# neu-vi/Superpoints_Registration

Measured on AMD Instinct MI355X. Metric: point-cloud pairs/sec (16 384 pts/cloud), higher is better.
Workload: dtype f32 (matrix products: range-scaled split-f16x2 MFMA, f32 accumulate; attention weights below 2^-5 of their row sum carried in one f16 plane); 1 GPU; synthetic 16384-pt pairs, full KPConv backbone + superpoint attn + Sinkhorn-SVD pose (3dmatch config, BASELINE configs[1]); streams_per_gpu=1, points_per_cloud=16384, generator=box, point_order=reference, upsample_indices=True, cross_step_overlap=True, streams_inside_a_forward=3: main path, pyramid searches, ResNet shortcut branches

## Files before the change

include/spr.h:

```cpp
#ifndef SPR_H_
#define SPR_H_

#include <stddef.h>
#include <stdint.h>

#ifdef __cplusplus
extern "C" {
#endif

#define SPR_VERSION 6

#define SPR_ACT_NONE 0
#define SPR_ACT_RELU 1
#define SPR_ACT_SIGMOID 2

#define SPR_ORDER_REFERENCE 0
#define SPR_ORDER_CANONICAL 1

#define SPR_SELECT_NEAREST 0
#define SPR_SELECT_INDEX 1

int spr_version(void);
const char* spr_last_error(void);

// ... 13 lines not shown

#define SPR_PREPARE_RANGE (-1)
#define SPR_PREPARE_PROBE (-2)
#define SPR_PREPARE_BAD_LAYOUT (-3)
size_t spr_prepare_scans_scratch_len(int n, int nb);
int spr_prepare_scans(const float* pts, int stride, const int* cu, int n, int nb, double voxel_size,
                      double crop_radius, int remove_ground, int* scratch, size_t scratch_len,
                      float* out_xyz, int* out_idx, int* out_cu, int* status, void* stream);

size_t spr_radius_neighbors_workspace_bytes(int nq, int ns, int nb);
int spr_radius_neighbors(const float* q_xyz, const int* q_cu, int nq,
                         const float* s_xyz, const int* s_cu, int ns, int nb,
                         float radius, int limit, int algo, int select, int* out_idx,
                         int* max_count, void* ws, size_t ws_bytes, void* stream);

size_t spr_radius_table_bytes(int ns, int nb);
size_t spr_radius_table_build_workspace_bytes(int ns, int nb);
size_t spr_radius_table_query_workspace_bytes(int nq);
int spr_radius_table_slots(void);
int spr_radius_table_build(const float* s_xyz, const int* s_cu, int ns, int nb, float radius,
                           void* table, size_t table_bytes, void* ws, size_t ws_bytes, void* stream);
int spr_radius_table_query(const float* q_xyz, const int* q_cu, int nq, int self, int ns, int nb,
                           float radius, int limit, int slot, const void* table, int* out_idx,
                           int* max_count, int algo, int select, void* ws, size_t ws_bytes, void* stream);

int spr_radius_table_count(const float* q_xyz, const int* q_cu, int nq, int self, int ns, int nb,
                           float radius, const void* table, int* counts, int* hist, int hist_n,
                           int* status, void* stream);

size_t spr_kdtree_replay_size(int ns, int nb);
int spr_kdtree_replay_build(const float* s_xyz, const int* s_cu, int ns, int nb, void* tree, size_t tree_bytes,
                            void* stream);
size_t spr_tie_order_workspace_size(int nq, int max_count, int depth);
int spr_tie_order(const float* q_xyz, const int* q_cu, int nq, const float* s_xyz, const int* s_cu, int ns, int nb,
                  float radius, const void* tree, int depth, int* nbr, int stride, int width, int max_count,
                  int* status, void* ws, size_t ws_bytes, void* stream);
int spr_tie_order_host(const float* q_xyz_host, const int* q_cu_host, int nq, const float* s_xyz_host,
                       const int* s_cu_host, int ns, int nb, float radius, int* nbr_host, int stride, int width,
                       int max_count, int* status_host);
int spr_std_sort_replay_host(const float* keys_host, int n, int* perm_host, int* heap_ranges_host);

size_t spr_gt_overlap_workspace_bytes(int ns, int nt, int nb);
int spr_gt_overlap(const float* src_xyz, const int* src_cu, int ns, const float* tgt_xyz, const int* tgt_cu,
                   int nt, const float* pose, int nb, double radius, int* src_corr, int* tgt_corr,
                   unsigned char* src_mask, unsigned char* tgt_mask, int* corr, int* corr_count, void* ws,
                   size_t ws_bytes, void* stream);

#define SPR_AUG_NONE 0
#define SPR_AUG_SMALL 1
#define SPR_AUG_LARGE 2
int spr_philox4x32_host(const uint32_t* ctr_host, const uint32_t* key_host, uint32_t* out_host);
int spr_augment_draw(uint64_t seed, const uint64_t* pair_key_host, int nb, int mode, unsigned char* perturb_src_host,
                     unsigned char* swap_host, float* perturb_host, const uint64_t* pair_key, const int* src_cu,
                     int ns, const int* tgt_cu, int nt, float* noise, unsigned int* keys, void* stream);
size_t spr_augment_workspace_bytes(int ns, int nt, int nb, int corr_stride);
int spr_augment_pairs(const float* src_xyz, const int* src_cu, int ns, const float* tgt_xyz, const int* tgt_cu,
                      int nt, const float* pose, int nb, const unsigned char* src_mask,
                      const unsigned char* tgt_mask, const int* corr, int corr_stride, const int* corr_off,
                      const int* corr_count, const float* perturb, const unsigned char* flags, int mode, float scale,
                      int max_pts, uint64_t seed, const uint64_t* pair_key, const float* noise,
                      const unsigned int* keys, float* out_src_xyz, float* out_tgt_xyz, int* out_src_cu,
                      int* out_tgt_cu, float* out_pose, unsigned char* out_src_mask, unsigned char* out_tgt_mask,
                      int* out_src_perm, int* out_tgt_perm, int* out_corr, int* out_corr_count, int* status, void* ws,
                      size_t ws_bytes, void* stream);

int spr_modelnet_draw(uint64_t seed, const uint64_t* pair_key_host, int nb, double rot_mag, double trans_mag,
                      double* dirs_host, float* transform_host, const uint64_t* pair_key, const int* cu, int n_total,
                      int k, unsigned int* rkeys, unsigned int* extra, float* noise, unsigned int* skeys, void* stream);
size_t spr_modelnet_pairs_workspace_size(int n_total, int nb, int k);
int spr_modelnet_pairs(const float* xyz, const int* cu, int n_total, int nb, int max_len_host, float p_src, float p_tgt,
                       double q_src, double q_tgt, int k, float scale, float clip, const float* transform,
                       const double* dirs, uint64_t seed, const uint64_t* pair_key, const unsigned int* rkeys,
                       const unsigned int* extra, const float* noise, const unsigned int* skeys, float* src_xyz,
                       float* tgt_xyz, float* pose, unsigned char* src_overlap, unsigned char* tgt_overlap,
                       int* src_index, int* tgt_index, int* corr, int* corr_count, int* status, void* ws,
                       size_t ws_bytes, void* stream);

int spr_estimate_normals(const float* xyz, const int* cu, int n, int nb, const int* nbr, int nbr_stride, int kmax,
                         const float* viewpoint, float* normals, float* curvature, void* stream);
int spr_feats_gather_rotate(const float* feats, int n_in, int c, const int* rows, int n_out, const int* cu_out, int nb,
                            const float* rot, const int* dir_cols_host, int n_dir, float* out, void* stream);

size_t spr_kpconv_workspace_bytes(int nq, int ns, int cin, int cout);
size_t spr_kpconv_plan_bytes(int nq);
int spr_kpconv_plan(const int* nbr, int nq, int ns, int nbr_stride, int kmax, int rows_sorted,
                    const int* order, void* plan, size_t plan_bytes, void* stream);
size_t spr_kpconv_wplanes_bytes(int cin, int cout);
int spr_kpconv_prep_weights(const float* weights, int n_kp, int cin, int cout, const float* w_range,
                            int w_range_n, void* wplanes, size_t wplanes_bytes, void* stream);
int spr_kpconv_fwd(const float* q_xyz, int nq, const float* s_xyz, int ns, const int* nbr,
                   int nbr_stride, int kmax, int rows_sorted, const float* x, int cin,
                   const float* weights, int cout, const float* kernel_points, int n_kp,
                   float kp_extent, float* out, int impl, const float* x_range, int x_range_n,
                   const float* w_range, int w_range_n, const void* plan, const void* wplanes,
                   void* ws, size_t ws_bytes, void* stream);

#define SPR_KP_CONSTANT 0
#define SPR_KP_LINEAR 1
#define SPR_KP_GAUSSIAN 2
#define SPR_KP_SUM 0
#define SPR_KP_CLOSEST 1
size_t spr_kpconv_modes_workspace_size(int nq, int ns, int cin, int cout);
int spr_kpconv_modes_fwd(const float* q_xyz, int nq, const float* s_xyz, int ns, const int* nbr, int nbr_stride,
                         int kmax, const float* x, int cin, const float* weights, int cout,
                         const float* kernel_points, int n_kp, float kp_extent, int influence, int aggregation,
                         float* out, int impl, const float* x_range, int x_range_n, const float* w_range,
                         int w_range_n, const void* wplanes, void* ws, size_t ws_bytes, void* stream);
size_t spr_kpconv_modes_weighted_features_workspace_size(int ns);
int spr_kpconv_modes_weighted_features(const float* q_xyz, int nq, const float* s_xyz, int ns, const int* nbr,
                                       int nbr_stride, int kmax, const float* x, int cin, const float* kernel_points,
                                       int n_kp, float kp_extent, int influence, int aggregation, float* wf,
                                       float* cnt, void* ws, size_t ws_bytes, void* stream);
int spr_kpconv_modes_bwd_dx(const float* q_xyz, int nq, const float* s_xyz, int ns, const int* nbr, int nbr_stride,
                            int kmax, int cin, const float* kernel_points, int n_kp, float kp_extent, int influence,
                            int aggregation, const float* dwf, const float* dwf_range, int dwf_range_n, float* dx,
                            void* ws, size_t ws_bytes, void* stream);

size_t spr_kpconv_deform_workspace_size(int nq, int ns, int cin, int cout);
int spr_kpconv_deform_fwd(const float* q_xyz, int nq, const float* s_xyz, int ns, const int* nbr, int nbr_stride,
                          int kmax, const float* x, int cin, const float* weights, int cout,
                          const float* kernel_points, int n_kp, float kp_extent, const float* offset_features,
                          int of_stride, int modulated, float* out, float* min_d2, int impl, const float* x_range,
                          int x_range_n, const float* w_range, int w_range_n, const void* wplanes, void* ws,
                          size_t ws_bytes, void* stream);
size_t spr_kpconv_deform_weighted_features_workspace_size(int ns);
int spr_kpconv_deform_weighted_features(const float* q_xyz, int nq, const float* s_xyz, int ns, const int* nbr,
                                        int nbr_stride, int kmax, const float* x, int cin, const float* kernel_points,
                                        int n_kp, float kp_extent, const float* offset_features, int of_stride,
                                        float* wf, float* cnt, void* ws, size_t ws_bytes, void* stream);
int spr_kpconv_deform_bwd_dx(const float* q_xyz, int nq, const float* s_xyz, int ns, const int* nbr, int nbr_stride,
                             int kmax, int cin, const float* kernel_points, int n_kp, float kp_extent,
                             const float* offset_features, int of_stride, int modulated, const float* dwfm,
                             const float* dwfm_range, int dwfm_range_n, float* dx, void* ws, size_t ws_bytes,
                             void* stream);
int spr_kpconv_deform_bwd_offsets(const float* q_xyz, int nq, const float* s_xyz, int ns, const int* nbr,
                                  int nbr_stride, int kmax, const float* x, int cin, const float* kernel_points,
                                  int n_kp, float kp_extent, const float* offset_features, int of_stride,
                                  int modulated, const float* dwfm, float* d_offset_features, void* stream);

size_t spr_deform_reg_workspace_size(int nq);
int spr_deform_reg(const float* q_xyz, int nq, const float* s_xyz, int ns, const int* nbr, int nbr_stride, int kmax,
                   const float* kernel_points, int n_kp, float kp_extent, const float* offset_features, int of_stride,
                   int modulated, float repulse_extent, float* out, float* d_offset_features, void* ws,
                   size_t ws_bytes, void* stream);

size_t spr_icp_pairs_workspace_size(int ns, int nt, int nb);
int spr_icp_pairs(const float* src_xyz, const int* src_cu, int ns, const float* tgt_xyz, const int* tgt_cu, int nt,
                  const double* pose_init, int nb, double max_dist, int max_iter, double rel_fitness, double rel_rmse,
                  float* pose, double* pose64, double* fitness, double* inlier_rmse, int* iterations, int* count,
                  int* corr, int* status, void* ws, size_t ws_bytes, void* stream);

int spr_kpconv_few_supported(int cin, int cout, int n_kp);

int spr_kpconv_stem_supported(int cin, int cout, int n_kp);
size_t spr_kpconv_stem_workspace_size(int nq, int ns, int nb, int max_len_host, int cout);
int spr_kpconv_stem(const float* q_xyz, int nq, const float* s_xyz, int ns, const int* nbr, int nbr_stride,
                    int kmax, int rows_sorted, const float* x, const float* weights, int cout,
                    const float* kernel_points, int n_kp, float kp_extent, const int* cu, int nb,
                    int max_len_host, float eps, float slope, float* out, float* out_range, int out_range_n,
                    float* mean_out, float* rstd_out, void* ws, size_t ws_bytes, void* stream);

size_t spr_instnorm_workspace_bytes(int max_len_host, int nb, int c);
int spr_instnorm(const float* x, const int* cu, int n, int nb, int max_len_host, int c,
                 float eps, int norm, const float* add, float slope, float* out,
                 float* out_range, int out_range_n, void* ws, size_t ws_bytes, void* stream);
int spr_instnorm_stats(const float* x, const int* cu, int n, int nb, int max_len_host, int c, float eps,
                       float* mean, float* rstd, void* ws, size_t ws_bytes, void* stream);

int spr_block_tail_tile_rows(int ka, int kb, int n_out);
size_t spr_block_tail_tiles_len(int n, int nb, int tile_rows);
int spr_block_tail_tiles(const int* cu, int n, int nb, int tile_rows, int* tiles, void* stream);
size_t spr_block_tail_workspace_bytes(int n, int nb, int kb, int n_out, int tile_rows);
int spr_block_tail(const float* xa, int ka, const float* wa, const float* xb, int kb, const float* wb,
                   const float* add, const int* cu, const int* tiles, int n, int nb, int n_out, float eps,
                   float slope, float* out, const float* xa_range, int xa_range_n, const float* wa_range,
                   int wa_range_n, const float* xb_range, int xb_range_n, const float* wb_range,
                   int wb_range_n, float* out_range, int out_range_n, const float* xa_mean,
                   const float* xa_rstd, float xa_slope, void* ws, size_t ws_bytes, void* stream);

int spr_maxpool_gather(const float* x, int ns, int c, const int* idx, int nq, int idx_stride, int k,
                       const int* order, float* out, float* out_range, int out_range_n, void* stream);
size_t spr_cell_order_workspace_bytes(int n);
int spr_cell_order(const float* xyz, const int* cu, int n, int nb, float cell, int* order, void* ws, size_t ws_bytes,
                   void* stream);

size_t spr_linear_workspace_bytes(void);
int spr_linear(const float* x, int m, int k, const float* w, int n, const float* bias,
               const float* residual, int act, float* out, const float* x_range,
               int x_range_n, const float* w_range, int w_range_n, float* out_range,
               int out_range_cap, int* out_range_n_host, void* ws, size_t ws_bytes, void* stream);
int spr_range_parts(void);
int spr_absmax(const float* x, long rows, int cols, long stride, float* parts, void* stream);
int spr_absmax_multi(const void* jobs_dev, int njobs, int parts_per_job, float* parts_out, void* stream);

int spr_set_gemm_mode(int mode);

int spr_layernorm_range_count(int m);
int spr_layernorm(const float* x, int m, int c, const float* gamma, const float* beta,
                  float eps, const float* pos, float* out_norm, float* out_pos,
                  float* range_norm, float* range_pos, void* stream);

int spr_posemb_sine(const float* xyz, int n, int d_model, float scale,
                    float temperature, float* out, void* stream);

int spr_posemb_mlp(const float* xyz, const float* const* params_host, int t, int d_model, float* pe, void* stream);
size_t spr_posemb_mlp_bwd_workspace_bytes(int t);
int spr_posemb_mlp_bwd(const float* xyz, const float* const* params_host, const float* dpe, int t, int d_model,
                       float* const* grads_host, void* ws, size_t ws_bytes, void* stream);

size_t spr_attn_workspace_bytes(int t, int nseg, int nhead, int head_dim);
int spr_attn_varlen_fwd(const float* q, int q_stride, const float* k, int k_stride, const float* v,
                        int v_stride, const int* cu, const int* kv_seg, int t, int nseg, int max_len_host,
                        int nhead, int head_dim, float scale, float* out, int o_stride, float* lse,
                        int* lse_written, void* ws, size_t ws_bytes, void* stream);

size_t spr_attn_inproj_workspace_bytes(int t, int nseg, int nhead, int head_dim);
int spr_attn_inproj_prepare(const float* w_in, int d, float* out, void* stream);
int spr_attn_inproj_varlen_fwd(const float* x_qk, const float* x_v, int t, const float* w_in,
                               const float* b_in, const int* cu, const int* kv_seg, int nseg,
                               int max_len_host, int nhead, int head_dim, float scale,
                               float* out, int o_stride, const float* xqk_range,
                               int xqk_range_n, const float* xv_range, int xv_range_n,
                               float* out_range, const float* w_prep, void* ws, size_t ws_bytes, void* stream);

size_t spr_attn_probs_workspace_bytes(int t, int nhead, int head_dim);
int spr_attn_probs(const float* q, int q_stride, const float* k, int k_stride, const int* cu,
                   const int* kv_seg, int t, int nseg, int max_len_host, int nhead, int head_dim,
                   float scale, int per_head, float* out, const long long* place, int max_rows_host,
                   int max_cols_host, void* ws, size_t ws_bytes, void* stream);

#define SPR_XENC_PTRS_PER_LAYER 18
size_t spr_xenc_prepared_bytes(int n_layers, int d_ff);
size_t spr_xenc_plan_bytes(void);
int spr_xenc_prepare(const void* const* layer_ptrs_host, const float* eps_host, int n_layers,
                     int d_model, int nhead, int d_ff, const float* final_g, const float* final_b,
                     float final_eps, float pos_bound, void* prepared, size_t prepared_bytes,
                     void* plan_host, size_t plan_bytes, void* stream);
size_t spr_xenc_workspace_bytes(int t, int nseg);
int spr_xenc_forward(const void* plan_host, const float* x, const float* pos, const int* cu,
                     const int* kv_self, const int* kv_cross, int t, int nseg, int max_len_host,
                     float* out, void* ws, size_t ws_bytes, void* stream);

size_t spr_attn_bwd_workspace_bytes(int t, int nseg, int nhead);
size_t spr_attn_bwd_min_workspace_bytes(int t, int nhead);
int spr_attn_varlen_bwd(const float* q, int q_stride, const float* k, int k_stride, const float* v,
                        int v_stride, const float* out, int o_stride, const float* dout, int do_stride,
                        const float* lse, const int* cu, const int* kv_seg, const int* q_seg, int t, int nseg,
                        int max_len_host, int nhead, int head_dim, float scale, float* dq, float* dk,
                        float* dv, void* ws, size_t ws_bytes, void* stream);

int spr_set_attn_mode(int mode);

size_t spr_match_workspace_bytes(const int* cu_host, int npairs);
int spr_match_dualsoftmax(const float* feat, int d, const int* cu,
                          const int* cu_host, int npairs, float* match_val,
                          float* match_val2, int* match_ind, void* ws, size_t ws_bytes,
                          void* stream);

int spr_pose_residuals(const float* pose, const float* a, const float* b, const int* pair_cu,
                       int npairs, int total_host, float* res, void* stream);
int spr_pose_scores(const float* poses, int nh, const float* a, const float* b, int n,
// ... 164 lines not shown
```

superpoints_registration_amd/_lib.py:

```python
import ctypes
import os
import subprocess

_HERE = os.path.dirname(os.path.abspath(__file__))
LIB_PATH = os.environ.get("SPR_HIP_LIB") or os.path.join(_HERE, "libspr_hip.so")

_vp = ctypes.c_void_p
_i = ctypes.c_int
_f = ctypes.c_float
_sz = ctypes.c_size_t
_l = ctypes.c_long
_u64 = ctypes.c_uint64
_d = ctypes.c_double

SIGNATURES = {
    "spr_version": (_i, []),
    "spr_last_error": (ctypes.c_char_p, []),
    "spr_grid_subsample_workspace_bytes": (_sz, [_i, _i]),
    "spr_grid_subsample": (_i, [_vp, _vp, _i, _i, _f, _i, _i, _vp, _vp, _vp, _vp, _sz, _vp]),
    "spr_grid_subsample_attrs_workspace_size": (_sz, [_i, _i, _i, _i]),
    "spr_grid_subsample_attrs": (_i, [_vp, _vp, _i, _i, _f, _i, _i, _vp, _i, _vp, _i, _vp, _vp, _vp, _vp, _vp, _vp, _sz,
                                      _vp]),
    "spr_voxel_downsample_workspace_bytes": (_sz, [_i]),
    "spr_voxel_downsample": (_i, [_vp, _i, ctypes.c_double, _vp, _vp, _vp, _sz, _vp]),
    "spr_prepare_scans_scratch_len": (_sz, [_i, _i]),
    "spr_prepare_scans": (_i, [_vp, _i, _vp, _i, _i, ctypes.c_double, ctypes.c_double, _i, _vp, _sz, _vp, _vp, _vp, _vp,
                               _vp]),
    "spr_radius_neighbors_workspace_bytes": (_sz, [_i, _i, _i]),
    "spr_radius_neighbors": (_i, [_vp, _vp, _i, _vp, _vp, _i, _i, _f, _i, _i, _i, _vp, _vp, _vp, _sz, _vp]),
    "spr_radius_table_bytes": (_sz, [_i, _i]),
    "spr_radius_table_build_workspace_bytes": (_sz, [_i, _i]),
    "spr_radius_table_query_workspace_bytes": (_sz, [_i]),
    "spr_radius_table_slots": (_i, []),
    "spr_radius_table_build": (_i, [_vp, _vp, _i, _i, _f, _vp, _sz, _vp, _sz, _vp]),
    "spr_radius_table_query": (_i, [_vp, _vp, _i, _i, _i, _i, _f, _i, _i, _vp, _vp, _vp, _i, _i, _vp, _sz, _vp]),
    "spr_radius_table_count": (_i, [_vp, _vp, _i, _i, _i, _i, _f, _vp, _vp, _vp, _i, _vp, _vp]),
    "spr_kdtree_replay_size": (_sz, [_i, _i]),
    "spr_kdtree_replay_build": (_i, [_vp, _vp, _i, _i, _vp, _sz, _vp]),
    "spr_tie_order_workspace_size": (_sz, [_i, _i, _i]),
    "spr_tie_order": (_i, [_vp, _vp, _i, _vp, _vp, _i, _i, _f, _vp, _i, _vp, _i, _i, _i, _vp, _vp, _sz, _vp]),
    "spr_tie_order_host": (_i, [_vp, _vp, _i, _vp, _vp, _i, _i, _f, _vp, _i, _i, _i, _vp]),
    "spr_std_sort_replay_host": (_i, [_vp, _i, _vp, _vp]),
    "spr_gt_overlap_workspace_bytes": (_sz, [_i, _i, _i]),
    "spr_gt_overlap": (_i, [_vp, _vp, _i, _vp, _vp, _i, _vp, _i, ctypes.c_double, _vp, _vp, _vp, _vp, _vp, _vp, _vp,
                            _sz, _vp]),
    "spr_icp_pairs_workspace_size": (_sz, [_i, _i, _i]),
    "spr_icp_pairs": (_i, [_vp, _vp, _i, _vp, _vp, _i, _vp, _i, _d, _i, _d, _d, _vp, _vp, _vp, _vp, _vp, _vp, _vp, _vp,
                           _vp, _sz, _vp]),
    "spr_philox4x32_host": (_i, [_vp, _vp, _vp]),
    "spr_augment_draw": (_i, [_u64, _vp, _i, _i, _vp, _vp, _vp, _vp, _vp, _i, _vp, _i, _vp, _vp, _vp]),
    "spr_augment_workspace_bytes": (_sz, [_i, _i, _i, _i]),
    "spr_augment_pairs": (_i, [_vp, _vp, _i, _vp, _vp, _i, _vp, _i, _vp, _vp, _vp, _i, _vp, _vp, _vp, _vp, _i, _f, _i,
                               _u64, _vp, _vp, _vp, _vp, _vp, _vp, _vp, _vp, _vp, _vp, _vp, _vp, _vp, _vp, _vp, _vp,
                               _sz, _vp]),
    "spr_modelnet_draw": (_i, [_u64, _vp, _i, _d, _d, _vp, _vp, _vp, _vp, _i, _i, _vp, _vp, _vp, _vp, _vp]),
    "spr_modelnet_pairs_workspace_size": (_sz, [_i, _i, _i]),
    "spr_modelnet_pairs": (_i, [_vp, _vp, _i, _i, _i, _f, _f, _d, _d, _i, _f, _f, _vp, _vp, _u64, _vp, _vp, _vp, _vp,
                                _vp, _vp, _vp, _vp, _vp, _vp, _vp, _vp, _vp, _vp, _vp, _vp, _sz, _vp]),
    "spr_estimate_normals": (_i, [_vp, _vp, _i, _i, _vp, _i, _i, _vp, _vp, _vp, _vp]),
    "spr_feats_gather_rotate": (_i, [_vp, _i, _i, _vp, _i, _vp, _i, _vp, _vp, _i, _vp, _vp]),
    "spr_kpconv_workspace_bytes": (_sz, [_i, _i, _i, _i]),
    "spr_kpconv_fwd": (_i, [_vp, _i, _vp, _i, _vp, _i, _i, _i, _vp, _i, _vp, _i, _vp, _i, _f, _vp, _i, _vp, _i, _vp,
                            _i, _vp, _vp, _vp, _sz, _vp]),
    "spr_kpconv_modes_workspace_size": (_sz, [_i, _i, _i, _i]),
    "spr_kpconv_modes_fwd": (_i, [_vp, _i, _vp, _i, _vp, _i, _i, _vp, _i, _vp, _i, _vp, _i, _f, _i, _i, _vp, _i, _vp,
                                  _i, _vp, _i, _vp, _vp, _sz, _vp]),
    "spr_kpconv_modes_weighted_features_workspace_size": (_sz, [_i]),
    "spr_kpconv_modes_weighted_features": (_i, [_vp, _i, _vp, _i, _vp, _i, _i, _vp, _i, _vp, _i, _f, _i, _i, _vp, _vp,
                                                _vp, _sz, _vp]),
    "spr_kpconv_modes_bwd_dx": (_i, [_vp, _i, _vp, _i, _vp, _i, _i, _i, _vp, _i, _f, _i, _i, _vp, _vp, _i, _vp, _vp,
                                     _sz, _vp]),
    "spr_kpconv_deform_workspace_size": (_sz, [_i, _i, _i, _i]),
    "spr_kpconv_deform_fwd": (_i, [_vp, _i, _vp, _i, _vp, _i, _i, _vp, _i, _vp, _i, _vp, _i, _f, _vp, _i, _i, _vp, _vp,
                                   _i, _vp, _i, _vp, _i, _vp, _vp, _sz, _vp]),
    "spr_kpconv_deform_weighted_features_workspace_size": (_sz, [_i]),
    "spr_kpconv_deform_weighted_features": (_i, [_vp, _i, _vp, _i, _vp, _i, _i, _vp, _i, _vp, _i, _f, _vp, _i, _vp,
                                                 _vp, _vp, _sz, _vp]),
    "spr_kpconv_deform_bwd_dx": (_i, [_vp, _i, _vp, _i, _vp, _i, _i, _i, _vp, _i, _f, _vp, _i, _i, _vp, _vp, _i, _vp,
                                      _vp, _sz, _vp]),
    "spr_kpconv_deform_bwd_offsets": (_i, [_vp, _i, _vp, _i, _vp, _i, _i, _vp, _i, _vp, _i, _f, _vp, _i, _i, _vp, _vp,
                                           _vp]),
    "spr_deform_reg_workspace_size": (_sz, [_i]),
    "spr_deform_reg": (_i, [_vp, _i, _vp, _i, _vp, _i, _i, _vp, _i, _f, _vp, _i, _i, _f, _vp, _vp, _vp, _sz, _vp]),
    "spr_kpconv_few_supported": (_i, [_i, _i, _i]),
    "spr_kpconv_stem_supported": (_i, [_i, _i, _i]),
    "spr_kpconv_stem_workspace_size": (_sz, [_i, _i, _i, _i, _i]),
    "spr_kpconv_stem": (_i, [_vp, _i, _vp, _i, _vp, _i, _i, _i, _vp, _vp, _i, _vp, _i, _f, _vp, _i, _i, _f, _f, _vp,
                             _vp, _i, _vp, _vp, _vp, _sz, _vp]),
    "spr_instnorm_workspace_bytes": (_sz, [_i, _i, _i]),
    "spr_instnorm": (_i, [_vp, _vp, _i, _i, _i, _i, _f, _i, _vp, _f, _vp, _vp, _i, _vp, _sz, _vp]),
    "spr_maxpool_gather": (_i, [_vp, _i, _i, _vp, _i, _i, _i, _vp, _vp, _vp, _i, _vp]),
    "spr_linear_workspace_bytes": (_sz, []),
    "spr_linear": (_i, [_vp, _i, _i, _vp, _i, _vp, _vp, _i, _vp, _vp, _i, _vp, _i, _vp, _i, _vp, _vp, _sz, _vp]),
    "spr_range_parts": (_i, []),
    "spr_absmax_multi": (_i, [_vp, _i, _i, _vp, _vp]),
    "spr_absmax": (_i, [_vp, _l, _i, _l, _vp, _vp]),
    "spr_kpconv_plan_bytes": (_sz, [_i]),
    "spr_kpconv_plan": (_i, [_vp, _i, _i, _i, _i, _i, _vp, _vp, _sz, _vp]),
    "spr_kpconv_wplanes_bytes": (_sz, [_i, _i]),
    "spr_kpconv_prep_weights": (_i, [_vp, _i, _i, _i, _vp, _i, _vp, _sz, _vp]),
    "spr_block_tail_tile_rows": (_i, [_i, _i, _i]),
    "spr_block_tail_tiles_len": (_sz, [_i, _i, _i]),
    "spr_block_tail_tiles": (_i, [_vp, _i, _i, _i, _vp, _vp]),
    "spr_block_tail_workspace_bytes": (_sz, [_i, _i, _i, _i, _i]),
    "spr_block_tail": (_i, [_vp, _i, _vp, _vp, _i, _vp, _vp, _vp, _vp, _i, _i, _i, _f, _f, _vp, _vp, _i, _vp, _i,
                            _vp, _i, _vp, _i, _vp, _i, _vp, _vp, _f, _vp, _sz, _vp]),
    "spr_instnorm_stats": (_i, [_vp, _vp, _i, _i, _i, _i, _f, _vp, _vp, _vp, _sz, _vp]),
    "spr_cell_order_workspace_bytes": (_sz, [_i]),
    "spr_cell_order": (_i, [_vp, _vp, _i, _i, _f, _vp, _vp, _sz, _vp]),
    "spr_layernorm_range_count": (_i, [_i]),
    "spr_attn_inproj_prepare": (_i, [_vp, _i, _vp, _vp]),
    "spr_set_gemm_mode": (_i, [_i]),
    "spr_layernorm": (_i, [_vp, _i, _i, _vp, _vp, _f, _vp, _vp, _vp, _vp, _vp, _vp]),
    "spr_posemb_sine": (_i, [_vp, _i, _i, _f, _f, _vp, _vp]),
    "spr_posemb_mlp": (_i, [_vp, _vp, _i, _i, _vp, _vp]),
    "spr_posemb_mlp_bwd_workspace_bytes": (_sz, [_i]),
    "spr_posemb_mlp_bwd": (_i, [_vp, _vp, _vp, _i, _i, _vp, _vp, _sz, _vp]),
    "spr_attn_workspace_bytes": (_sz, [_i, _i, _i, _i]),
    "spr_attn_varlen_fwd": (_i, [_vp, _i, _vp, _i, _vp, _i, _vp, _vp, _i, _i, _i, _i, _i, _f, _vp, _i, _vp, _vp, _vp,
                                 _sz, _vp]),
    "spr_attn_probs_workspace_bytes": (_sz, [_i, _i, _i]),
    "spr_attn_probs": (_i, [_vp, _i, _vp, _i, _vp, _vp, _i, _i, _i, _i, _i, _f, _i, _vp, _vp, _i, _i, _vp, _sz,
                            _vp]),
    "spr_attn_bwd_workspace_bytes": (_sz, [_i, _i, _i]),
    "spr_attn_bwd_min_workspace_bytes": (_sz, [_i, _i]),
    "spr_attn_varlen_bwd": (_i, [_vp, _i, _vp, _i, _vp, _i, _vp, _i, _vp, _i, _vp, _vp, _vp, _vp, _i, _i, _i, _i, _i,
                                 _f, _vp, _vp, _vp, _vp, _sz, _vp]),
    "spr_attn_inproj_workspace_bytes": (_sz, [_i, _i, _i, _i]),
    "spr_attn_inproj_varlen_fwd": (_i, [_vp, _vp, _i, _vp, _vp, _vp, _vp, _i, _i, _i, _i, _f, _vp, _i, _vp, _i, _vp,
                                        _i, _vp, _vp, _vp, _sz, _vp]),
    "spr_set_attn_mode": (_i, [_i]),
    "spr_xenc_prepared_bytes": (_sz, [_i, _i]),
    "spr_xenc_plan_bytes": (_sz, []),
    "spr_xenc_prepare": (_i, [_vp, _vp, _i, _i, _i, _i, _vp, _vp, _f, _f, _vp, _sz, _vp, _sz, _vp]),
    "spr_xenc_workspace_bytes": (_sz, [_i, _i]),
    "spr_xenc_forward": (_i, [_vp, _vp, _vp, _vp, _vp, _vp, _i, _i, _i, _vp, _vp, _sz, _vp]),
    "spr_match_workspace_bytes": (_sz, [_vp, _i]),
    "spr_match_dualsoftmax": (_i, [_vp, _i, _vp, _vp, _i, _vp, _vp, _vp, _vp, _sz, _vp]),
    "spr_pose_residuals": (_i, [_vp, _vp, _vp, _vp, _i, _i, _vp, _vp]),
    "spr_pose_scores": (_i, [_vp, _i, _vp, _vp, _i, _vp, _vp]),
    "spr_weighted_procrustes": (_i, [_vp, _vp, _vp, _vp, _i, _vp, _vp]),
    "spr_refine_pairs_workspace_bytes": (_sz, [_i, _i]),
    "spr_refine_pairs": (_i, [_vp, _vp, _vp, _vp, _vp, _vp, _i, _i, _vp, _vp, _i, _f, _f, _i, _vp, _i, _vp, _vp, _vp, _vp,
                              _vp, _vp, _vp, _sz, _vp]),
    "spr_ransac_draw": (_i, [_u64, _vp, _vp, _i, _i, _i, _vp]),
    "spr_ransac_pairs": (_i, [_vp, _vp, _vp, _vp, _i, _i, _i, _u64, _vp, _vp, _vp, _vp, _vp, _vp, _vp, _vp]),
    "spr_sinkhorn_workspace_bytes": (_sz, [_vp, _i]),
    "spr_match_sinkhorn": (_i, [_vp, _i, _vp, _vp, _vp, _i, _vp, _vp, _i, _vp, _vp, _vp, _vp, _vp, _vp, _sz, _vp]),
    "spr_sinkhorn_correspondences": (_i, [_vp, _i, _vp, _vp, _vp, _i, _vp, _vp, _i, _i, _vp, _vp, _vp,
                                          _sz, _vp]),
    "spr_loss_workspace_bytes": (_sz, [_i, _i, _i]),
    "spr_overlap_pool": (_i, [_vp, _i, _vp, _i, _i, _i, _vp, _vp]),
    "spr_bce_logits_mean": (_i, [_vp, _vp, _i, _vp, _vp, _sz, _vp]),
    "spr_infonce_pair": (_i, [_vp, _i, _vp, _i, _i, _vp, _vp, _vp, _vp, _f, _f, _vp, _vp, _sz, _vp]),
    "spr_transform_l1_pair": (_i, [_vp, _vp, _vp, _i, _vp, _vp, _sz, _vp]),
    "spr_sum_scaled": (_i, [_vp, _i, _f, _vp, _vp]),
    "spr_gather_rows": (_i, [_vp, _i, _i, _vp, _i, _vp, _vp]),
    "spr_upsample_unary_supported": (_i, [_i, _i, _i]),
    "spr_upsample_unary_workspace_size": (_sz, []),
    "spr_upsample_unary": (_i, [_vp, _i, _i, _vp, _i, _i, _vp, _i, _vp, _i, _vp, _vp, _i, _vp, _i, _vp, _i, _vp, _i,
                                _vp, _vp, _sz, _vp]),
    "spr_pair_gather": (_i, [_vp, _i, _i, _vp, _i, _vp, _vp, _i, _vp, _i, _vp, _vp]),
    "spr_pair_gather_bwd": (_i, [_vp, _i, _i, _vp, _i, _vp, _vp, _i, _vp, _i, _vp, _vp]),
    "spr_overlap_pool_pairs": (_i, [_vp, _i, _vp, _i, _i, _i, _vp, _vp, _i, _vp, _i, _vp, _vp, _i, _vp, _vp]),
    "spr_bgemm": (_i, [_vp, _vp, _vp, _vp, _i, _i, _i, _l, _l, _l, _l, _l, _l, _f, _f, _vp]),
    "spr_tn_product_split_workspace_bytes": (_sz, []),
    "spr_tn_product_split": (_i, [_vp, _vp, _l, _i, _i, _i, _vp, _i, _vp, _i, _vp, _vp, _sz, _vp]),
    "spr_tn_product_f64_workspace_bytes": (_sz, [_l, _i, _i]),
    "spr_tn_product_f64": (_i, [_vp, _vp, _l, _i, _i, _vp, _vp, _sz, _vp]),
    "spr_reduce_parts": (_i, [_vp, _i, _l, _f, _vp, _i, _vp]),
    "spr_act_bwd": (_i, [_vp, _vp, _i, _l, _vp, _vp]),
    "spr_colsum_workspace_bytes": (_sz, [_i]),
    "spr_colsum": (_i, [_vp, _l, _i, _vp, _vp, _sz, _vp]),
    "spr_layernorm_bwd_workspace_bytes": (_sz, [_i]),
    "spr_layernorm_bwd": (_i, [_vp, _i, _i, _vp, _f, _vp, _vp, _vp, _vp, _vp, _vp, _sz, _vp]),
    "spr_instnorm_bwd_workspace_bytes": (_sz, [_i, _i, _i]),
    "spr_instnorm_bwd": (_i, [_vp, _vp, _vp, _vp, _i, _i, _i, _i, _f, _i, _f, _vp, _vp, _vp, _sz, _vp]),
    "spr_scatter_workspace_bytes": (_sz, [_l, _i]),
    "spr_maxpool_bwd": (_i, [_vp, _i, _i, _vp, _i, _i, _i, _vp, _vp, _vp, _sz, _vp]),
    "spr_scatter_rows_add": (_i, [_vp, _vp, _i, _i, _i, _vp, _vp, _sz, _vp]),
    "spr_kpconv_weighted_features_workspace_bytes": (_sz, [_i]),
    "spr_kpconv_weighted_features": (_i, [_vp, _i, _vp, _i, _vp, _i, _i, _vp, _i, _vp, _i, _f, _vp, _vp, _vp, _sz,
                                          _vp]),
    "spr_kpconv_bwd_dx": (_i, [_vp, _i, _vp, _i, _vp, _i, _i, _i, _vp, _i, _f, _vp, _vp, _i, _vp, _vp, _sz, _vp]),
    "spr_softmax_rows": (_i, [_vp, _vp, _i, _i, _vp]),
    "spr_softmax_bwd_rows": (_i, [_vp, _vp, _vp, _i, _i, _vp]),
    "spr_bce_logits_mean_bwd": (_i, [_vp, _vp, _i, _vp, _vp, _vp]),
    "spr_infonce_pair_dlogits": (_i, [_vp, _i, _vp, _i, _i, _vp, _vp, _vp, _vp, _f, _f, _vp, _vp, _vp, _vp, _vp, _sz,
                                      _vp]),
# ... 46 lines not shown
```

superpoints_registration_amd/csrc/block_tail.hip:

```cpp
#include "spr_common.h"
#include "split_mma.h"

namespace spr {
int gemm_mode();
namespace {

constexpr int kTailThreads = 512;
constexpr int kTailWaves = 8;

struct TailArgs {
  const float* xa;
  const float* xb;
  const float* wa;
  const float* wb;
  const float* add;
  const int* cu;
  const int* tile_cu;
  const int4* tile_desc;
  int nb, n, n_total;
  const float* xa_parts;
  const float* xb_parts;
  const float* wa_parts;
  const float* wb_parts;
  int xa_np, xb_np, wa_np, wb_np;
// ... 304 lines not shown
  }
  const int len = cu[cloud + 1] - cu[cloud];
  const double n = len > 0 ? (double)len : 1.0;
  const double m = s / n;
  double var = ss / n - m * m;
  if (var < 0.0) var = 0.0;
  float* o = stats + ((size_t)cloud * nbr + br) * 2 * n_total + col;
  o[0] = (float)m;
  o[n_total] = (float)(1.0 / sqrt(var + (double)eps));
}

__global__ __launch_bounds__(1024) void k_tile_cu(const int* __restrict__ cu, int nb, int tr, int* __restrict__ tile_cu) {
  __shared__ int sh[1024];
  int carry = 0;
  for (int base = 0; base < nb; base += 1024) {
    const int c = base + threadIdx.x;
    int v = c < nb ? (cu[c + 1] - cu[c] + tr - 1) / tr : 0;
    sh[threadIdx.x] = v;
    __syncthreads();
    for (int o = 1; o < 1024; o <<= 1) {
      const int add = threadIdx.x >= o ? sh[threadIdx.x - o] : 0;
      __syncthreads();
      sh[threadIdx.x] += add;
      __syncthreads();
    }
    if (c < nb) tile_cu[c + 1] = carry + sh[threadIdx.x];
    carry += sh[1023];
    __syncthreads();
  }
  if (threadIdx.x == 0) tile_cu[0] = 0;
}

__global__ void k_tile_desc(const int* __restrict__ cu, const int* __restrict__ tile_cu, int tr, int4* __restrict__ desc) {
  const int c = blockIdx.x;
  const int t0 = tile_cu[c], nt = tile_cu[c + 1] - t0, r0 = cu[c], len = cu[c + 1] - r0;
  for (int i = threadIdx.x; i < nt; i += blockDim.x) desc[t0 + i] = make_int4(r0 + i * tr, min(tr, len - i * tr), c, 0);
}

struct TailShape {
  int nc, tr;
};
TailShape tail_shape(int ka, int kb, int n_total) {
  if (ka == 32 && kb == 64 && n_total == 128) return {128, 64};
  if (ka == 32 && kb == 0 && n_total == 128) return {128, 64};
  if (ka == 64 && kb == 128 && n_total == 256) return {256, 64};
  if (ka == 64 && kb == 0 && n_total == 256) return {256, 64};
  if (ka == 128 && kb == 256 && n_total == 512) return {128, 32};
  if (ka == 128 && kb == 0 && n_total == 512) return {256, 64};
  return {0, 0};
}

template <int KA, int KB, int NC, int TR>
int launch_tail(const TailArgs& a, float eps, hipStream_t stream) {
  constexpr int KS = (KA + KB) / 32, NBR = KB > 0 ? 2 : 1;
  constexpr int lds = 4 * (TR / 16) * KS * 1024 + 2 * NBR * 2 * NC * (int)sizeof(float);
  const void* k1 = (const void*)k_block_tail<KA, KB, NC, TR, 1>;
  const void* k2 = (const void*)k_block_tail<KA, KB, NC, TR, 2>;
  if (int rc = ensure_dyn_lds(k1, lds)) return rc;
  if (int rc = ensure_dyn_lds(k2, lds)) return rc;
  static int per_cu[2] = {0, 0};
  if (per_cu[0] == 0) {
    int n1 = 0, n2 = 0;
    if (hipOccupancyMaxActiveBlocksPerMultiprocessor(&n1, k1, kTailThreads, lds) != hipSuccess || n1 < 1) n1 = 1;
    if (hipOccupancyMaxActiveBlocksPerMultiprocessor(&n2, k2, kTailThreads, lds) != hipSuccess || n2 < 1) n2 = 1;
    per_cu[1] = n2 > 2 ? 2 : n2;
    per_cu[0] = n1 > 2 ? 2 : n1;
  }
  const int ncg = a.n_total / NC;
  const int max_tiles = cdiv(a.n, TR) + a.nb;
  auto grid_x = [&](int occ) {
    int g = device_cu_count() * occ / ncg;
    if (g > max_tiles) g = max_tiles;
    return g < 1 ? 1 : g;
  };
  hipLaunchKernelGGL((k_block_tail<KA, KB, NC, TR, 1>), dim3(grid_x(per_cu[0]), ncg), dim3(kTailThreads), lds, stream, a);
  hipLaunchKernelGGL(k_tail_final, dim3(cdiv((long)a.nb * NBR * a.n_total, 256)), dim3(256), 0, stream, a.part, a.cu,
                     a.tile_cu, a.nb, NBR, a.n_total, eps, a.stats);
  hipLaunchKernelGGL((k_block_tail<KA, KB, NC, TR, 2>), dim3(grid_x(per_cu[1]), ncg), dim3(kTailThreads), lds, stream, a);
  SPR_LAUNCH_CHECK();
  return 0;
}

}
}

using namespace spr;

extern "C" int spr_block_tail_tile_rows(int ka, int kb, int n_out) { return tail_shape(ka, kb, n_out).tr; }

static size_t tiles_desc_offset(int nb) { return align_up((size_t)(nb > 0 ? nb : 0) + 1, 4); }
extern "C" size_t spr_block_tail_tiles_len(int n, int nb, int tile_rows) {
  return tiles_desc_offset(nb) + 4 * ((size_t)cdiv(n > 0 ? n : 1, tile_rows > 0 ? tile_rows : 64) + (size_t)(nb > 0 ? nb : 1));
}

extern "C" int spr_block_tail_tiles(const int* cu, int n, int nb, int tile_rows, int* tiles, void* stream_) {
  hipStream_t stream = (hipStream_t)stream_;
  SPR_REQUIRE(cu != nullptr && tiles != nullptr && n >= 1 && nb >= 1 && tile_rows >= 16 && ((uintptr_t)tiles & 15) == 0,
              "block_tail_tiles: bad arguments");
  hipLaunchKernelGGL(k_tile_cu, dim3(1), dim3(1024), 0, stream, cu, nb, tile_rows, tiles);
  hipLaunchKernelGGL(k_tile_desc, dim3(nb), dim3(256), 0, stream, cu, tiles, tile_rows,
                     reinterpret_cast<int4*>(tiles + tiles_desc_offset(nb)));
  SPR_LAUNCH_CHECK();
  return 0;
}

namespace {
struct TailWs {
  double* part;
  float* stats;
  float* mp[4];
};
TailWs tail_layout(Workspace& w, int n, int nb, int kb, int n_out, int tile_rows) {
  const size_t nbr = kb > 0 ? 2 : 1, B = (size_t)(nb > 0 ? nb : 1), no = (size_t)(n_out > 0 ? n_out : 0);
  const size_t tiles = (size_t)cdiv(n > 0 ? n : 1, tile_rows > 0 ? tile_rows : 64) + B;
  TailWs l;
  l.part = w.take<double>(tiles * nbr * 2 * no);
  l.stats = w.take<float>(B * nbr * 2 * no);
  for (float*& p : l.mp) p = w.take<float>(kAmaxParts);
  return l;
}
}

extern "C" size_t spr_block_tail_workspace_bytes(int n, int nb, int kb, int n_out, int tile_rows) {
  return measure(tail_layout, n, nb, kb, n_out, tile_rows);
}

extern "C" int spr_block_tail(const float* xa, int ka, const float* wa, const float* xb, int kb, const float* wb,
                              const float* add, const int* cu, const int* tiles, int n, int nb, int n_out, float eps,
                              float slope, float* out, const float* xa_range, int xa_range_n, const float* wa_range,
                              int wa_range_n, const float* xb_range, int xb_range_n, const float* wb_range,
                              int wb_range_n, float* out_range, int out_range_n, const float* xa_mean,
                              const float* xa_rstd, float xa_slope, void* ws, size_t ws_bytes, void* stream_) {
  hipStream_t stream = (hipStream_t)stream_;
  SPR_REQUIRE(spr::gemm_mode() == 1, "block_tail: only in the split-fp16 product mode (spr_set_gemm_mode(1))");
  const TailShape sh = tail_shape(ka, kb, n_out);
  SPR_REQUIRE(sh.tr > 0, "block_tail: unsupported shape ka=%d kb=%d n_out=%d (spr_block_tail_tile_rows)", ka, kb, n_out);
  SPR_REQUIRE(xa && wa && cu && tiles && out && n > 0 && nb >= 1, "block_tail: null operand or empty input");
  SPR_REQUIRE((kb > 0) == (xb != nullptr) && (kb > 0) == (wb != nullptr), "block_tail: xb / wb must come with kb > 0");
  SPR_REQUIRE(!(kb > 0 && add != nullptr), "block_tail: either a projected shortcut (xb, wb) or a plain one (add)");
  SPR_REQUIRE(out_range == nullptr || (out_range_n >= 1 && (out_range_n & (out_range_n - 1)) == 0),
              "block_tail: out_range_n must be a power of two");
  Workspace w(ws, ws_bytes);
  const TailWs l = tail_layout(w, n, nb, kb, n_out, sh.tr);
  SPR_REQUIRE(ws != nullptr && w.ok(), "block_tail: workspace too small");
  TailArgs a;
  a.part = l.part;
  a.stats = l.stats;
  float* const* mp = l.mp;
  a.xa = xa; a.xb = xb; a.wa = wa; a.wb = wb; a.add = add; a.cu = cu; a.tile_cu = tiles;
  a.tile_desc = reinterpret_cast<const int4*>(tiles + tiles_desc_offset(nb));
  a.nb = nb; a.n = n; a.n_total = n_out; a.slope = slope; a.out = out; a.out_range = out_range; a.nslots = out_range_n;
  a.xa_mean = xa_mean; a.xa_rstd = xa_rstd; a.xa_slope = xa_slope;
  SPR_REQUIRE((xa_mean == nullptr) == (xa_rstd == nullptr), "block_tail: xa_mean and xa_rstd come together");
  SPR_REQUIRE(xa_mean == nullptr || xa_range != nullptr,
              "block_tail: a normalised-on-load xa needs the bound of the NORMALISED values as xa_range");
  auto range = [&](const float* x, long rows, int cols, const float* given, int given_n, float* scratch,
                   const float*& parts, int& np) -> int {
    if (given != nullptr) {
      SPR_REQUIRE(given_n >= 1, "block_tail: a range needs a count");
      parts = given;
      np = given_n;
      return 0;
    }
    parts = scratch;
    np = kAmaxParts;
    return launch_absmax(x, rows, cols, cols, scratch, stream);
  };
  if (int rc = range(xa, n, ka, xa_range, xa_range_n, mp[0], a.xa_parts, a.xa_np)) return rc;
  if (int rc = range(wa, n_out, ka, wa_range, wa_range_n, mp[1], a.wa_parts, a.wa_np)) return rc;
  a.xb_parts = a.wb_parts = nullptr;
  a.xb_np = a.wb_np = 0;
  if (kb > 0) {
    if (int rc = range(xb, n, kb, xb_range, xb_range_n, mp[2], a.xb_parts, a.xb_np)) return rc;
// ... 15 lines not shown
```

superpoints_registration_amd/csrc/kpconv.hip:

```cpp
#include "lds_dma.h"
#include "spr_common.h"
#include "split_mma.h"

namespace spr {
namespace {

constexpr int kKP = 15;

__global__ __launch_bounds__(256) void k_rowflag(const float* __restrict__ x, const float* __restrict__ s_xyz,
                                                 int ns, int cin, unsigned char* __restrict__ flag,
                                                 float4* __restrict__ sxf, int* __restrict__ tile_ctr) {
  const int wid = (blockIdx.x * blockDim.x + threadIdx.x) >> 6;
  const int lane = threadIdx.x & 63;
  const int c4 = cin >> 2;
  if (blockIdx.x == 0 && threadIdx.x == 0) {
    sxf[ns] = make_float4(-1.0e17f, -1.0e17f, -1.0e17f, __int_as_float(0));
    tile_ctr[0] = 0;
  }
  if ((cin & 3) == 0 && c4 <= 64 && (c4 & (c4 - 1)) == 0) {
    constexpr int kRfSteps = 4;
    const int rpl = 64 / c4;
    const int sub = lane / c4, chunk = lane % c4;
    const int row0 = wid * rpl * kRfSteps + sub;
    float4 v[kRfSteps];
#pragma unroll
    for (int r = 0; r < kRfSteps; ++r) {
      const int row = row0 + r * rpl;
      v[r] = make_float4(0.f, 0.f, 0.f, 0.f);
      if (row < ns) v[r] = reinterpret_cast<const float4*>(x + (size_t)row * cin)[chunk];
    }
#pragma unroll
    for (int r = 0; r < kRfSteps; ++r) {
      const int row = row0 + r * rpl;
      float c[4] = {v[r].x, v[r].y, v[r].z, v[r].w};
#pragma unroll
      for (int e = 0; e < 4; ++e) {
        float t = c[e];
        if (c4 == 64) {
          const int b = lane & 15;
          const float a0 = __shfl(t, b, 64), a1 = __shfl(t, b | 16, 64), a2 = __shfl(t, b | 32, 64),
                      a3 = __shfl(t, b | 48, 64);
          t = ((a0 + a1) + a2) + a3;
        } else if (c4 == 32) {
          t += __shfl_xor(t, 16, 64);
        }
        for (int o = (c4 < 16 ? c4 : 16) >> 1; o > 0; o >>= 1) t += __shfl_xor(t, o, 64);
        c[e] = t;
      }
      const float t = (c[0] + c[2]) + (c[1] + c[3]);
      if (chunk == 0 && row < ns) {
        const int f = t > 0.f ? 1 : 0;
        flag[row] = (unsigned char)f;
        sxf[row] = make_float4(s_xyz[3 * (size_t)row], s_xyz[3 * (size_t)row + 1],
                               s_xyz[3 * (size_t)row + 2], __int_as_float(f));
      }
    }
    return;
  }
  const int row = wid;
  if (row >= ns) return;
  float s = 0.f;
  for (int c = lane; c < cin; c += 64) s += x[(size_t)row * cin + c];
  s = wave_sum(s);
  if (lane == 0) {
    const int f = s > 0.f ? 1 : 0;
    flag[row] = (unsigned char)f;
    sxf[row] = make_float4(s_xyz[3 * (size_t)row], s_xyz[3 * (size_t)row + 1],
                           s_xyz[3 * (size_t)row + 2], __int_as_float(f));
  }
}

__global__ void k_kpconv_simple(const float* __restrict__ q_xyz, int nq,
                                const float* __restrict__ s_xyz, int ns,
                                const int* __restrict__ nbr, int nbr_stride, int kmax,
                                const float* __restrict__ x, int cin,
                                const float* __restrict__ W, int cout,
                                const float* __restrict__ kpts, int n_kp, float inv_extent,
                                const unsigned char* __restrict__ flag,
                                float* __restrict__ out) {
  const long gid = (long)blockIdx.x * blockDim.x + threadIdx.x;
  if (gid >= (long)nq * cout) return;
  const int n = (int)(gid / cout), o = (int)(gid % cout);
  const float qx = q_xyz[3 * (size_t)n], qy = q_xyz[3 * (size_t)n + 1], qz = q_xyz[3 * (size_t)n + 2];
  float acc = 0.f;
  int cnt = 0;
  for (int k = 0; k < kmax; ++k) {
    const int idx = nbr[(size_t)n * nbr_stride + k];
    if (idx < 0 || idx >= ns) continue;
    cnt += flag[idx];
    const float rx = s_xyz[3 * (size_t)idx] - qx, ry = s_xyz[3 * (size_t)idx + 1] - qy,
                rz = s_xyz[3 * (size_t)idx + 2] - qz;
    for (int p = 0; p < n_kp; ++p) {
      const float dx = rx - kpts[3 * p], dy = ry - kpts[3 * p + 1], dz = rz - kpts[3 * p + 2];
      const float w = fmaxf(0.f, 1.f - sqrtf(dx * dx + dy * dy + dz * dz) * inv_extent);
      if (w > 0.f) {
        float d = 0.f;
        for (int c = 0; c < cin; ++c)
          d += x[(size_t)idx * cin + c] * W[((size_t)p * cin + c) * cout + o];
        acc += w * d;
      }
    }
  }
  out[(size_t)n * cout + o] = acc / (float)max(cnt, 1);
}

__global__ __launch_bounds__(256) void k_records_cin1(const float* __restrict__ x, const float* __restrict__ s_xyz,
                                                      int ns, float4* __restrict__ sxf) {
  const int i = blockIdx.x * blockDim.x + threadIdx.x;
  if (i < ns) sxf[i] = make_float4(s_xyz[3 * (size_t)i], s_xyz[3 * (size_t)i + 1], s_xyz[3 * (size_t)i + 2], x[i]);
}

constexpr int kCin1Chunk = 64;
constexpr int kCin1RowStride = kCin1Chunk + 1;
constexpr int kCin1Batch = 8;
constexpr int kCin1LdsInts = 4 * 16 * kCin1RowStride + 32;

template <int B>
__device__ __forceinline__ void cin1_gather(const float* __restrict__ q_xyz, int nq, int ns,
                                            const int* __restrict__ nbr, int nbr_stride, int kmax, int rows_sorted,
                                            const float4* __restrict__ sxf, const float* __restrict__ kpts, int n_kp,
                                            float inv_extent, int* __restrict__ lrows, float (&wf)[4]) {
  static_assert(B >= 1 && B <= 32, "the last batch's reads past the last staged row stay inside the slack");
  const int lane = threadIdx.x & 63, wave = threadIdx.x >> 6;
  const int qv = lane & 15, g = lane >> 4;
  const int q0 = blockIdx.x * 64 + wave * 16;
  const int n = min(q0 + qv, nq - 1);
  const float qx = q_xyz[3 * (size_t)n], qy = q_xyz[3 * (size_t)n + 1], qz = q_xyz[3 * (size_t)n + 2];
  float kx[4], ky[4], kz[4];
  bool kok[4];
#pragma unroll
  for (int s = 0; s < 4; ++s) {
    const int p = 4 * s + g;
    kok[s] = p < n_kp;
    kx[s] = kok[s] ? kpts[3 * p] : 0.f;
    ky[s] = kok[s] ? kpts[3 * p + 1] : 0.f;
    kz[s] = kok[s] ? kpts[3 * p + 2] : 0.f;
  }
#pragma unroll
  for (int s = 0; s < 4; ++s) wf[s] = 0.f;
  int cnt = 0;
  int* lrow = lrows + wave * 16 * kCin1RowStride;
  bool done = q0 >= nq;
  for (int c0 = 0; c0 < kmax; c0 += kCin1Chunk) {
    const int kc = min(kCin1Chunk, kmax - c0);
    if (c0 > 0) __syncthreads();
    {
      int v[4][kCin1Chunk / 16];
#pragma unroll
      for (int i = 0; i < 4; ++i) {
        const int* src = nbr + (size_t)min(q0 + g + 4 * i, nq - 1) * nbr_stride + c0;
#pragma unroll
        for (int j = 0; j < kCin1Chunk / 16; ++j) {
// ... 1032 lines not shown

    f32x4 acc2 = {0.f, 0.f, 0.f, 0.f};
    {
      const _Float16* ah_row = wfh + p16 * SH + 8 * j4;
      const _Float16* al_row = wfl + p16 * SH + 8 * j4;
#pragma unroll
      for (int k = 0; k < KSW; ++k) {
        const int ks = min(ks0 + k, KS - 1);
        const f16x8 ah = *reinterpret_cast<const f16x8*>(ah_row + 32 * ks);
        const f16x8 al = *reinterpret_cast<const f16x8*>(al_row + 32 * ks);
        acc2 = mma3_16(ah, al, bh[k], bl[k], acc2);
      }
    }
    if (sp > 0) {
#pragma unroll
      for (int r = 0; r < 4; ++r) red[((ng * (SPLIT - 1) + sp - 1) * 4 + r) * 64 + lane] = acc2[r];
    }
    KP_STAMP(6);
    asm volatile("s_waitcnt lgkmcnt(0)" ::: "memory");
    __builtin_amdgcn_s_barrier();
    KP_STAMP(7);
    if (sp == 0) {
#pragma unroll
      for (int s2 = 1; s2 < SPLIT; ++s2)
#pragma unroll
        for (int r = 0; r < 4; ++r) acc2[r] += red[((ng * (SPLIT - 1) + s2 - 1) * 4 + r) * 64 + lane];
#pragma unroll
      for (int r = 0; r < 4; ++r) {
        const int ql = acc_row16(r, j4);
        pend_n[r] = lqid[par * kRingTQ + ql];
        const float inv = unscale / (float)max(lcnt[par * kRingTQ + ql], 1);
        pend_v[r] = acc2[r] * inv;
      }
    }
    KP_STAMP(8);
    d_cur = d_nxt;
    d_nxt = d_nn;
    tile = tile_nxt;
    tile_nxt = tile_nn;
    tile_nn = __builtin_amdgcn_readfirstlane(ltile[1 + par]);
  }
  if (sp == 0) flush_pending();
  wait_vm<0>();
#ifdef SPR_KP_RING_PROF
  if (blockIdx.x == 0) {
    asm volatile("s_waitcnt lgkmcnt(0)" ::: "memory");
    for (int k = lane; k < kTraceN; k += 64) g_kp_trace[wave * kTraceN + k] = k < trace_n ? trace_lds[wave * kTraceN + k] : 0ull;
  }
#endif
}

template <int CC, int COUT, int NS>
int launch_ring(const float* q_xyz, int nq, int ns, const int* nbr, int nbr_stride, int kmax, const float* x,
                const _Float16* Wh, const _Float16* Wl, const float* kpts, float inv_extent, const float4* sxf,
                const int4* desc, const int* pad_word, const float* x_parts, const float* w_parts, int n_xparts,
                int n_wparts, int* tile_ctr, float* out, hipStream_t stream) {
  typedef RingShape<CC, COUT, NS> S;
  const int idxw = kmax <= 64 ? 64 : 128;
#ifdef SPR_KP_RING_PROF
  const size_t lds = S::lds_bytes(idxw) + 8 * kTraceN * 8;
#else
  const size_t lds = S::lds_bytes(idxw);
#endif
  auto kern = k_kpconv_ring<CC, COUT, NS>;
  ProfScope prof(stream, CC * 100000 + COUT, nq);
  if (lds > 64 * 1024)
    if (int rc = ensure_dyn_lds((const void*)kern, 160 * 1024)) return rc;
  const int ntiles = cdiv(nq, kRingTQ);
  const int n_cu = device_cu_count();
  int per_cu = (int)((160 * 1024) / lds);
  per_cu = per_cu < 1 ? 1 : (per_cu > S::MINW / 2 ? S::MINW / 2 : per_cu);
  const int grid = ntiles < n_cu * per_cu ? ntiles : n_cu * per_cu;
  hipLaunchKernelGGL(kern, dim3(grid), dim3(512), lds, stream, q_xyz, ns, nbr, nbr_stride, kmax, x, Wh, Wl, kpts,
                     inv_extent, sxf, desc, ntiles, pad_word, idxw, x_parts, w_parts, n_xparts, n_wparts, tile_ctr, out);
  SPR_LAUNCH_CHECK();
  return 0;
}

}

void launch_rowflag(const float* x, const float* s_xyz, int ns, int cin, unsigned char* flag, float4* sxf,
                    int* tile_ctr, hipStream_t stream) {
  const int c4 = cin >> 2;
  const bool wide = (cin & 3) == 0 && c4 <= 64 && (c4 & (c4 - 1)) == 0;
  const long waves = wide ? cdiv(ns, (64 / c4) * 4) : (long)ns;
  hipLaunchKernelGGL(k_rowflag, dim3(cdiv(waves * 64, 256)), dim3(256), 0, stream, x, s_xyz, ns, cin, flag, sxf, tile_ctr);
}
}

using namespace spr;

#ifdef SPR_KP_RING_PROF
extern "C" int spr_debug_kp_trace(unsigned long long* out, int n) {
  if (hipDeviceSynchronize() != hipSuccess) return 1;
  if (hipMemcpyFromSymbol(out, HIP_SYMBOL(g_kp_trace), sizeof(unsigned long long) * n) != hipSuccess) return 1;
  return 0;
}
#endif

struct KpPlan {
  int4* desc;
  int* pad_word;
};
static KpPlan plan_view(Workspace& w, int nq) {
  KpPlan p;
  p.desc = w.take<int4>((size_t)cdiv(nq > 0 ? nq : 1, kRingTQ) * 8);
  p.pad_word = w.take<int>(64);
  return p;
}
struct KpWPlanes {
  _Float16 *hi, *lo;
};
static KpWPlanes wplanes_view(Workspace& w, int cin, int cout) {
  const size_t n = (size_t)32 * (size_t)(cin > 0 ? cin : 0) * (size_t)(cout > 0 ? cout : 0);
  KpWPlanes p;
  p.hi = w.take<_Float16>(n);
  p.lo = w.take<_Float16>(n);
  return p;
}
struct KpWs {
  unsigned char* flag;
  float4* sxf;
  KpWPlanes wplanes;
  float *x_parts, *w_parts;
  KpPlan plan;
  int* tile_ctr;
  float4* few_rec;
};
static inline bool few_cin(int cin) { return cin >= 2 && cin <= 8; }
static KpWs kpconv_layout(Workspace& w, int nq, int ns, int cin, int cout) {
  const size_t n = (size_t)(ns > 0 ? ns : 1);
  KpWs l;
  l.flag = w.take<unsigned char>(n);
  l.sxf = w.take<float4>(n + 1);
  l.wplanes = wplanes_view(w, cin, cout);
  l.x_parts = w.take<float>(kAmaxParts);
  l.w_parts = w.take<float>(kAmaxParts);
  l.plan = plan_view(w, nq);
  l.tile_ctr = w.take<int>(64);
  l.few_rec = w.take<float4>(cin >= 2 ? n * (cin <= 4 ? 2 : 3) : 0);
  return l;
}
static inline int w_chunk(int cin) { return cin % 64 == 0 ? 64 : 32; }
static inline bool ring_shape(int cin, int cout) {
  return (cin == 32 || cin == 64) && cin * cout <= 4096 && cout % 32 == 0 && 8 % (cout / 16) == 0;
}

extern "C" size_t spr_kpconv_plan_bytes(int nq) {
  return measure(plan_view, nq);
}

static int launch_plan(const int* nbr, int nq, int ns, int nbr_stride, int kmax, int rows_sorted, const int* order,
                       const KpPlan& p, hipStream_t stream) {
  const int ntiles = cdiv(nq, kRingTQ);
  hipLaunchKernelGGL(k_kp_tiles, dim3(cdiv((long)ntiles * 64, 256)), dim3(256), 0, stream, nbr, nq, ns, nbr_stride,
                     kmax, rows_sorted, order, ntiles, p.desc, p.pad_word);
  SPR_LAUNCH_CHECK();
  return 0;
}

extern "C" int spr_kpconv_plan(const int* nbr, int nq, int ns, int nbr_stride, int kmax, int rows_sorted,
                               const int* order, void* plan, size_t plan_bytes, void* stream_) {
  hipStream_t stream = (hipStream_t)stream_;
  SPR_REQUIRE(nq > 0 && ns > 0 && kmax >= 1 && kmax <= nbr_stride, "kpconv plan: bad sizes");
  Workspace w(plan, plan_bytes);
  const KpPlan p = plan_view(w, nq);
  SPR_REQUIRE(plan != nullptr && w.ok(), "kpconv plan: buffer too small");
  return launch_plan(nbr, nq, ns, nbr_stride, kmax, rows_sorted, order, p, stream);
}

extern "C" size_t spr_kpconv_wplanes_bytes(int cin, int cout) {
  return measure(wplanes_view, cin, cout);
}

extern "C" int spr_kpconv_prep_weights(const float* weights, int n_kp, int cin, int cout, const float* w_range,
                                       int w_range_n, void* wplanes, size_t bytes, void* stream_) {
  hipStream_t stream = (hipStream_t)stream_;
  SPR_REQUIRE(n_kp == kKP && cin % 32 == 0 && cout % 32 == 0 && cout <= 256,
              "kpconv weight planes exist for the MFMA shapes only (15 kernel points, channels in multiples of 32)");
  SPR_REQUIRE(w_range != nullptr && w_range_n >= 1, "kpconv weight planes: the weight range is required");
  Workspace w(wplanes, bytes);
  const auto [wh, wl] = wplanes_view(w, cin, cout);
  SPR_REQUIRE(wplanes != nullptr && w.ok(), "kpconv weight planes: buffer too small");
  hipLaunchKernelGGL(k_w_prep, dim3(cdiv((long)n_kp * cin * cout, 256)), dim3(256), 0, stream, weights, cin, cout,
                     w_chunk(cin), w_range, w_range_n, wh, wl);
  SPR_LAUNCH_CHECK();
  return 0;
}

extern "C" size_t spr_kpconv_workspace_bytes(int nq, int ns, int cin, int cout) {
  return measure(kpconv_layout, nq, ns, cin, cout);
}

namespace {
struct StemWs {
  float4* sxf;
  float* S;
  double* part;
  float *mean, *rstd;
};
StemWs stem_layout(Workspace& w, int nq, int ns, int nb, int max_len, int cout) {
  const size_t Q = (size_t)(nq > 0 ? nq : 1), N = (size_t)(ns > 0 ? ns : 1), B = (size_t)(nb > 0 ? nb : 1),
               C = (size_t)(cout > 0 ? cout : 1);
  StemWs l{};
  l.sxf = w.take<float4>(N);
  l.S = w.take<float>(Q * 16);
  l.part = w.take<double>(B * instnorm_nsplit(max_len) * 2 * C);
  l.mean = w.take<float>(B * C);
  l.rstd = w.take<float>(B * C);
  return l;
}
}

extern "C" int spr_kpconv_few_supported(int cin, int cout, int n_kp) {
  return few_cin(cin) && cout >= 1 && n_kp >= 1 && n_kp <= 16;
}

extern "C" int spr_kpconv_stem_supported(int cin, int cout, int n_kp) {
  return cin == 1 && cout >= 16 && cout % 16 == 0 && n_kp >= 1 && n_kp <= 16;
}

extern "C" size_t spr_kpconv_stem_workspace_size(int nq, int ns, int nb, int max_len, int cout) {
  return measure(stem_layout, nq, ns, nb, max_len, cout);
}

extern "C" int spr_kpconv_stem(const float* q_xyz, int nq, const float* s_xyz, int ns, const int* nbr, int nbr_stride,
                               int kmax, int rows_sorted, const float* x, const float* weights, int cout,
                               const float* kernel_points, int n_kp, float kp_extent, const int* cu, int nb,
                               int max_len_host, float eps, float slope, float* out, float* out_range,
                               int out_range_n, float* mean_out, float* rstd_out, void* ws, size_t ws_bytes,
                               void* stream_) {
  hipStream_t stream = (hipStream_t)stream_;
  SPR_REQUIRE(nq > 0 && ns > 0 && nb >= 1, "kpconv_stem: empty input");
  SPR_REQUIRE(kmax >= 1 && kmax <= nbr_stride, "kpconv_stem: bad kmax=%d stride=%d", kmax, nbr_stride);
  SPR_REQUIRE(spr_kpconv_stem_supported(1, cout, n_kp), "kpconv_stem: no kernel for cout=%d, %d kernel points", cout,
              n_kp);
  SPR_REQUIRE(kp_extent > 0.f, "kpconv_stem: KP_extent must be > 0");
  SPR_REQUIRE(max_len_host >= 1 && max_len_host <= nq, "kpconv_stem: bad max_len_host=%d", max_len_host);
  SPR_REQUIRE(out_range == nullptr || (out_range_n >= 1 && (out_range_n & (out_range_n - 1)) == 0),
              "kpconv_stem: out_range_n must be a power of two");
  SPR_REQUIRE(instnorm_slice_rows() == kStemSliceRows, "kpconv_stem: statistics slices differ from the InstanceNorm's");
  Workspace w(ws, ws_bytes);
  const StemWs l = stem_layout(w, nq, ns, nb, max_len_host, cout);
  SPR_REQUIRE(ws != nullptr && w.ok(), "kpconv_stem: workspace too small");
  const int nsplit = instnorm_nsplit(max_len_host);
  float* mean = mean_out != nullptr ? mean_out : l.mean;
  float* rstd = rstd_out != nullptr ? rstd_out : l.rstd;
  hipLaunchKernelGGL(k_records_cin1, dim3(cdiv(ns, 256)), dim3(256), 0, stream, x, s_xyz, ns, l.sxf);
  {
    ProfScope prof(stream, 100000 + cout, nq);
    hipLaunchKernelGGL(k_stem_sums, dim3(cdiv(nq, 64)), dim3(256), 0, stream, q_xyz, nq, ns, nbr, nbr_stride, kmax,
                       rows_sorted, l.sxf, kernel_points, n_kp, 1.0f / kp_extent, l.S);
  }
  hipLaunchKernelGGL(k_stem_stats, dim3(nb, nsplit), dim3(256), 0, stream, l.S, cu, weights, cout, n_kp, nsplit,
                     l.part);
  launch_in_final(l.part, cu, nb, cout, nsplit, eps, mean, rstd, stream);
  hipLaunchKernelGGL(k_stem_apply, dim3(cdiv(nq, 64)), dim3(256), 0, stream, l.S, nq, cu, nb, weights, cout, n_kp,
                     mean, rstd, slope, out, out_range, out_range_n);
  SPR_LAUNCH_CHECK();
  return 0;
}

extern "C" int spr_kpconv_fwd(const float* q_xyz, int nq, const float* s_xyz, int ns,
                              const int* nbr, int nbr_stride, int kmax, int rows_sorted,
                              const float* x, int cin, const float* weights, int cout,
                              const float* kernel_points, int n_kp, float kp_extent,
                              float* out, int impl, const float* x_range, int x_range_n, const float* w_range,
                              int w_range_n, const void* plan, const void* wplanes, void* ws, size_t ws_bytes,
                              void* stream_) {
  hipStream_t stream = (hipStream_t)stream_;
  SPR_REQUIRE((x_range == nullptr || x_range_n >= 1) && (w_range == nullptr || w_range_n >= 1),
              "kpconv: a range needs a count");
  SPR_REQUIRE(nq > 0 && ns > 0, "kpconv: empty input");
  SPR_REQUIRE(kmax >= 1 && kmax <= nbr_stride, "kpconv: bad kmax=%d stride=%d", kmax, nbr_stride);
  SPR_REQUIRE(cin >= 1 && cout >= 1 && n_kp >= 1 && n_kp <= 32, "kpconv: bad dims");
  SPR_REQUIRE(kp_extent > 0.f, "kpconv: KP_extent must be > 0");
  Workspace w(ws, ws_bytes);
  const auto [flag, sxf, own_wplanes, x_parts, w_parts, own_plan, tile_ctr, few_rec] = kpconv_layout(w, nq, ns, cin, cout);
  SPR_REQUIRE(ws != nullptr && w.ok(), "kpconv: workspace too small");
  SPR_REQUIRE(wplanes == nullptr || w_range != nullptr, "kpconv: prepared weight planes come with the range they were scaled by");
  Workspace given_w(const_cast<void*>(wplanes), SIZE_MAX), given_p(const_cast<void*>(plan), SIZE_MAX);
  const auto [wh, wl] = wplanes != nullptr ? wplanes_view(given_w, cin, cout) : own_wplanes;
  const float inv_extent = 1.0f / kp_extent;

  if (cin == 1 && (impl == 0 || impl == 2) && n_kp <= 16) {
    hipLaunchKernelGGL(k_records_cin1, dim3(cdiv(ns, 256)), dim3(256), 0, stream, x, s_xyz, ns, sxf);
    ProfScope prof(stream, cin * 100000 + cout, nq);
    hipLaunchKernelGGL(k_kpconv_cin1, dim3(cdiv(nq, 64)), dim3(256), 0, stream, q_xyz, nq, s_xyz, ns, nbr,
                       nbr_stride, kmax, rows_sorted, sxf, weights, cout, kernel_points, n_kp, inv_extent, out);
    SPR_LAUNCH_CHECK();
    return 0;
  }

  if ((impl == 0 || impl == 2) && spr_kpconv_few_supported(cin, cout, n_kp)) {
    switch (cin) {
#define SPR_FEW_CASE(C)                                                                                              \
  case C: {                                                                                                          \
    hipLaunchKernelGGL(k_records_few<C>, dim3(cdiv(ns, 256)), dim3(256), 0, stream, x, s_xyz, ns, few_rec);          \
    ProfScope prof(stream, cin * 100000 + cout, nq);                                                                 \
    hipLaunchKernelGGL(k_kpconv_few<C>, dim3(cdiv(nq, 64)), dim3(256), 0, stream, q_xyz, nq, ns, nbr, nbr_stride,    \
                       kmax, rows_sorted, few_rec, weights, cout, kernel_points, n_kp, inv_extent, out);             \
  } break;
      SPR_FEW_CASE(2) SPR_FEW_CASE(3) SPR_FEW_CASE(4) SPR_FEW_CASE(5) SPR_FEW_CASE(6) SPR_FEW_CASE(7) SPR_FEW_CASE(8)
#undef SPR_FEW_CASE
    }
    SPR_LAUNCH_CHECK();
    return 0;
  }

  launch_rowflag(x, s_xyz, ns, cin, flag, sxf, tile_ctr, stream);
  SPR_LAUNCH_CHECK();

  const bool tile_fits = cin % 64 == 0 ? mfma_lds_bytes(64, kTile64TQ, kTileWaves, kmax) <= kMfmaLdsMax
                                       : mfma_lds_bytes(32, kTile32TQ, kTileWaves, kmax) <= kMfmaLdsMax;
  if ((impl == 0 || impl == 2) && n_kp == kKP && cin % 32 == 0 && cout % 32 == 0 && cout <= 256 && tile_fits) {
    const int ktot = n_kp * cin;
    const float* xp = x_range != nullptr ? x_range : x_parts;
    const float* wp = w_range != nullptr ? w_range : w_parts;
    const int n_xp = x_range != nullptr ? x_range_n : kAmaxParts, n_wp = w_range != nullptr ? w_range_n : kAmaxParts;
    if (x_range == nullptr && w_range == nullptr) {
      if (int rc = launch_absmax2(x, ns, cin, cin, x_parts, weights, ktot, cout, cout, w_parts, stream)) return rc;
    } else if (x_range == nullptr) {
      if (int rc = launch_absmax(x, ns, cin, cin, x_parts, stream)) return rc;
    } else if (w_range == nullptr) {
      if (int rc = launch_absmax(weights, ktot, cout, cout, w_parts, stream)) return rc;
    }
    if (wplanes == nullptr)
      hipLaunchKernelGGL(k_w_prep, dim3(cdiv((long)ktot * cout, 256)), dim3(256), 0, stream, weights, cin, cout,
                         w_chunk(cin), wp, n_wp, wh, wl);
    const bool ring_ok = impl == 0 && ring_shape(cin, cout) && kmax <= 128 && (size_t)ns * cin * 4 < (1ull << 32) &&
                         (size_t)nq * nbr_stride * 4 < (1ull << 32);
    if (ring_ok) {
      if (plan == nullptr)
        if (int rc = launch_plan(nbr, nq, ns, nbr_stride, kmax, rows_sorted, nullptr, own_plan, stream)) return rc;
      const auto [desc, pad_word] = plan != nullptr ? plan_view(given_p, nq) : own_plan;
#define SPR_RING_ARGS                                                                                       \
  q_xyz, nq, ns, nbr, nbr_stride, kmax, x, wh, wl, kernel_points, inv_extent, sxf, desc, pad_word, xp, wp, \
      n_xp, n_wp, tile_ctr, out, stream
      if (cin == 64 && cout == 64) return launch_ring<64, 64, 4>(SPR_RING_ARGS);
      if (cin == 64 && cout == 32) return launch_ring<64, 32, 4>(SPR_RING_ARGS);
      if (cin == 32 && cout == 32) return launch_ring<32, 32, 3>(SPR_RING_ARGS);
      if (cin == 32 && cout == 64) return launch_ring<32, 64, 8>(SPR_RING_ARGS);
      if (cin == 32 && cout == 128) return launch_ring<32, 128, 8>(SPR_RING_ARGS);
#undef SPR_RING_ARGS
    }
#define SPR_KP_ARGS                                                                         \
  q_xyz, nq, s_xyz, ns, nbr, nbr_stride, kmax, rows_sorted, x, cin, wh, wl, cout,           \
      kernel_points, inv_extent, sxf, xp, wp, n_xp, n_wp, out, stream
    if (cin % 64 == 0) {
      if (cout == 64) return launch_mfma<64, kTile64TQ, 1, kTileWaves, 2>(SPR_KP_ARGS);
      if (cout == 128) return launch_mfma<64, kTile64TQ, 2, kTileWaves, 2>(SPR_KP_ARGS);
      if (cout == 256) return launch_mfma<64, kTile64TQ, 4, kTileWaves, 2>(SPR_KP_ARGS);
    } else {
      if (cout == 32) return launch_mfma<32, kTile32TQ, 1, kTileWaves, 1>(SPR_KP_ARGS);
      if (cout == 64) return launch_mfma<32, kTile32TQ, 2, kTileWaves, 1>(SPR_KP_ARGS);
      if (cout == 128) return launch_mfma<32, kTile32TQ, 4, kTileWaves, 1>(SPR_KP_ARGS);
    }
#undef SPR_KP_ARGS
  }
  const long total = (long)nq * cout;
  hipLaunchKernelGGL(k_kpconv_simple, dim3(cdiv(total, 256)), dim3(256), 0, stream, q_xyz, nq,
                     s_xyz, ns, nbr, nbr_stride, kmax, x, cin, weights, cout, kernel_points, n_kp,
                     inv_extent, flag, out);
  SPR_LAUNCH_CHECK();
  return 0;
}
```

superpoints_registration_amd/csrc/linear.hip:

```cpp
#include <atomic>

#include "attn_planes.h"
#include "lds_dma.h"
#include "spr_common.h"
#include "split_mma.h"

namespace spr {
namespace {

constexpr int BK = 32;
static_assert(BK == kPlaneK, "the split kernels stage split_mma.h's slabs");
constexpr int LDSK = BK + 1;

template <int ACT, bool RES>
__device__ __forceinline__ float store_tile(const f32x16& acc, int row0, int col, int M, int N,
                                            float bv, const float* __restrict__ residual,
                                            float* __restrict__ out, int lh, float unscale = 1.0f,
                                            const float* __restrict__ epi = nullptr) {
  if (col >= N) return 0.f;
  float vmax = 0.f;
  float res[16];
  if (RES) {
#pragma unroll
    for (int r = 0; r < 16; ++r) {
// ... 37 lines not shown
  f32x16 acc;
#pragma unroll
  for (int i = 0; i < 16; ++i) acc[i] = 0.f;

  f32x4 ra[A_PT], rb[B_PT];
  auto load_slab = [&](int k0) {
#pragma unroll
    for (int i = 0; i < A_PT; ++i) {
      const int f = tid + i * NT;
      if (f < A_F4) {
        const int r = f / (BK / 4), c4 = f % (BK / 4);
        const float* p = X + (size_t)min(m0 + r, M - 1) * K + k0 + c4 * 4;
        asm volatile("global_load_dwordx4 %0, %1, off" : "=v"(ra[i]) : "v"(p));
      }
    }
#pragma unroll
    for (int i = 0; i < B_PT; ++i) {
      const int f = tid + i * NT;
      if (f < B_F4) {
        const int r = f / (BK / 4), c4 = f % (BK / 4);
        const float* p = Wt + (size_t)min(n0 + r, N - 1) * K + k0 + c4 * 4;
        asm volatile("global_load_dwordx4 %0, %1, off" : "=v"(rb[i]) : "v"(p));
      }
    }
  };
  auto store_slab = [&]() {
    wait_vm<0>();
    __builtin_amdgcn_sched_barrier(0);
#pragma unroll
    for (int i = 0; i < A_PT; ++i) {
      const int f = tid + i * NT;
      if (f < A_F4) {
        const int r = f / (BK / 4), c4 = f % (BK / 4);
        const bool in = m0 + r < M;
        float* d = As + r * LDSK + c4 * 4;
        d[0] = in ? ra[i][0] : 0.f;
        d[1] = in ? ra[i][1] : 0.f;
        d[2] = in ? ra[i][2] : 0.f;
        d[3] = in ? ra[i][3] : 0.f;
      }
    }
#pragma unroll
    for (int i = 0; i < B_PT; ++i) {
      const int f = tid + i * NT;
      if (f < B_F4) {
        const int r = f / (BK / 4), c4 = f % (BK / 4);
        const bool in = n0 + r < N;
        float* d = Bs + r * LDSK + c4 * 4;
        d[0] = in ? rb[i][0] : 0.f;
        d[1] = in ? rb[i][1] : 0.f;
        d[2] = in ? rb[i][2] : 0.f;
        d[3] = in ? rb[i][3] : 0.f;
      }
    }
  };

  load_slab(0);
  for (int k0 = 0; k0 < K; k0 += BK) {
    store_slab();
    __syncthreads();
    if (k0 + BK < K) load_slab(k0 + BK);
    __builtin_amdgcn_sched_barrier(0);
    const float* ap = As + (wm * 32 + l31) * LDSK + lh;
    const float* bp = Bs + (wn * 32 + l31) * LDSK + lh;
    float fa[BK / 2], fb[BK / 2];
#pragma unroll
    for (int s = 0; s < BK / 2; ++s) {
      fa[s] = ap[2 * s];
      fb[s] = bp[2 * s];
    }
    __builtin_amdgcn_sched_barrier(0);
#pragma unroll
    for (int s = 0; s < BK / 2; ++s)
      acc = __builtin_amdgcn_mfma_f32_32x32x2f32(fa[s], fb[s], acc, 0, 0, 0);
    __builtin_amdgcn_sched_barrier(0);
    __syncthreads();
  }
  wait_vm<0>();
  const int col = n0 + wn * 32 + l31;
  const float bv = (bias && col < N) ? bias[col] : 0.f;
  store_tile<ACT, RES>(acc, m0 + wm * 32, col, M, N, bv, residual, out, lh);
}

template <int BM, int BN, int WM, int WN, int ACT, bool RES, bool PLANES = false>
__global__ __launch_bounds__(WM* WN * 64) void k_gemm_nt_h3(
    const float* __restrict__ Xp, int Mp, int K, const float* __restrict__ Wp, int Np,
    const float* __restrict__ bias, const float* __restrict__ residual,
    float* __restrict__ outp, AttnPlanes pl, int f0, const float* __restrict__ a_parts, int n_aparts,
    const float* __restrict__ w_parts, float* __restrict__ out_parts,
    const GemmGroup* __restrict__ groups, int n_wparts) {
  constexpr int NT = WM * WN * 64;
  const float* __restrict__ X = Xp;
  const float* __restrict__ Wt = Wp;
  float* __restrict__ out = outp;
  int M = Mp, N = Np, bid = blockIdx.x, nblk = gridDim.x;
  if (groups != nullptr) {
    int g = 0, beg = 0;
    while (bid >= groups[g].tile_end) beg = groups[g++].tile_end;
    X += groups[g].a_off;
    Wt += groups[g].b_off;
    out += groups[g].c_off;
    M = groups[g].m;
    N = groups[g].n;
    nblk = groups[g].tile_end - beg;
    bid -= beg;
  }
  constexpr int TM = BM / (WM * 32), TN = BN / (WN * 32);
  extern __shared__ __align__(16) unsigned char gemm_smem[];
  _Float16* Ah = reinterpret_cast<_Float16*>(gemm_smem);
  _Float16* Al = Ah + BM * kPlaneStride;
  _Float16* Bh = Al + BM * kPlaneStride;
  _Float16* Bl = Bh + BN * kPlaneStride;
  const int tid = threadIdx.x, wave = tid >> 6, lane = tid & 63;
  const int wm = wave / WN, wn = wave % WN;
  const int gx = (N + BN - 1) / BN;
  const int lid = groups != nullptr ? bid : xcd_swizzle(bid, nblk);
  const int m0 = (lid / gx) * BM, n0 = (lid % gx) * BN;
  const int l31 = lane & 31, lh = lane >> 5;

  float sa, sb, unscale;
  {
    float* shf = reinterpret_cast<float*>(gemm_smem);
    const int ka = pow2_exp_for(block_absmax(a_parts, shf, n_aparts));
    const int kb = pow2_exp_for(block_absmax(w_parts, shf, n_wparts));
    __syncthreads();
    sa = pow2f(ka);
    sb = pow2f(kb);
    unscale = pow2f(-ka - kb);
  }

  f32x16 acc[TM][TN];
#pragma unroll
  for (int i = 0; i < TM; ++i)
#pragma unroll
    for (int j = 0; j < TN; ++j)
#pragma unroll
      for (int r = 0; r < 16; ++r) acc[i][j][r] = 0.f;

  f32x4 ra[BM * BK / 4 / NT], rb[BN * BK / 4 / NT];
  auto load_slab = [&](int k0) {
    slab_load<BM, NT>(ra, X, M, K, tid, m0, k0);
    slab_load<BN, NT>(rb, Wt, N, K, tid, n0, k0);
  };
  auto store_slab = [&]() {
    wait_vm<0>();
    __builtin_amdgcn_sched_barrier(0);
    slab_store<BM, NT>(ra, sa, Ah, Al, tid);
    slab_store<BN, NT>(rb, sb, Bh, Bl, tid);
  };

  load_slab(0);
  for (int k0 = 0; k0 < K; k0 += BK) {
    store_slab();
    __syncthreads();
    if (k0 + BK < K) load_slab(k0 + BK);
    __builtin_amdgcn_sched_barrier(0);
#pragma unroll
    for (int s = 0; s < BK / 16; ++s) {
      const int ko = 16 * s + 8 * lh;
      f16x8 ah[TM], al[TM], bh[TN], bl[TN];
#pragma unroll
      for (int i = 0; i < TM; ++i) frag_ld40(Ah, Al, (wm * TM + i) * 32 + l31, ko, ah[i], al[i]);
#pragma unroll
      for (int j = 0; j < TN; ++j) frag_ld40(Bh, Bl, (wn * TN + j) * 32 + l31, ko, bh[j], bl[j]);
#pragma unroll
      for (int i = 0; i < TM; ++i)
#pragma unroll
        for (int j = 0; j < TN; ++j) {
          if (PLANES) acc[i][j] = mma3_32<true>(bh[j], bl[j], ah[i], al[i], acc[i][j]);
          else acc[i][j] = mma3_32(ah[i], al[i], bh[j], bl[j], acc[i][j]);
        }
    }
    __builtin_amdgcn_sched_barrier(0);
    __syncthreads();
  }
  wait_vm<0>();
  if (PLANES) {
#pragma unroll
    for (int i = 0; i < TM; ++i) {
      const int tok = m0 + (wm * TM + i) * 32 + l31;
      if (tok >= M) continue;
      const int which = (f0 + n0) >> 8;
      const float pmul = pl.scales[which];
      int vcol = 0;
      if (which == 2) {
        const int sg = find_segment(pl.cu, pl.nseg, tok);
        vcol = attn_vperm(attn_vstart_of(pl.cu[sg], sg) + tok - pl.cu[sg]);
      }
#pragma unroll
      for (int j = 0; j < TN; ++j) {
        const int fl = n0 + (wn * TN + j) * 32;
        const int fg = (f0 + fl) & 255;
        if (which == 2) {
#pragma unroll
          for (int r = 0; r < 16; r += 2) {
            const int d = acc_row32(r, lh);
            const float a = acc[i][j][r] * unscale + bias[fl + d];
            const float b = acc[i][j][r + 1] * unscale + bias[fl + d + 1];
            unsigned int hu, lu;
            split_pk_s(a, b, pmul, hu, lu);
            const f16x2 hh = __builtin_bit_cast(f16x2, hu), ll = __builtin_bit_cast(f16x2, lu);
            const size_t o = attn_v_off(fg + d, (size_t)vcol, 256);
            pl.vth[o] = hh[0];
            pl.vth[o + 16] = hh[1];
            pl.vtl[o] = ll[0];
            pl.vtl[o + 16] = ll[1];
          }
        } else {
          _Float16* ph = which == 0 ? pl.qh : pl.kh;
          _Float16* pw = which == 0 ? pl.ql : pl.kl;
          const size_t row = ((size_t)(fg >> 5) * pl.t_total + tok) * 32;
#pragma unroll
          for (int g = 0; g < 4; ++g) {
            const int d0 = 8 * g + 4 * lh;
            f32x4 v;
#pragma unroll
            for (int e = 0; e < 4; ++e) v[e] = acc[i][j][4 * g + e] * unscale + bias[fl + d0 + e];
            split_store4(v, pmul, ph + row + d0, pw + row + d0);
          }
        }
      }
    }
    return;
  }
  float omax = 0.f;
#pragma unroll
  for (int j = 0; j < TN; ++j) {
    const int col = n0 + (wn * TN + j) * 32 + l31;
    const float bv = (ACT < kEpiScale && bias && col < N) ? bias[col] : 0.f;
#pragma unroll
    for (int i = 0; i < TM; ++i)
      omax = fmaxf(omax, store_tile<ACT, RES>(acc[i][j], m0 + (wm * TM + i) * 32, col, M, N, bv, residual, out, lh,
                                              unscale, ACT >= kEpiScale ? bias : nullptr));
  }
  if (out_parts != nullptr) {
    float* shf = reinterpret_cast<float*>(gemm_smem);
    omax = wave_max(omax);
    __syncthreads();
    if (lane == 0) shf[wave] = omax;
    __syncthreads();
    if (tid == 0) {
      float t = shf[0];
      for (int w_ = 1; w_ < WM * WN; ++w_) t = fmaxf(t, shf[w_]);
      out_parts[blockIdx.x] = t;
    }
  }
}

template <int ACT>
__global__ __launch_bounds__(512) void k_gemm_nt_h3p(
    const float* __restrict__ X, int M, const float* __restrict__ Wt, int N,
    const float* __restrict__ bias, float* __restrict__ out,
    const float* __restrict__ a_parts, int n_aparts, const float* __restrict__ w_parts, int n_wparts,
    float* __restrict__ out_parts, int ntiles) {
  constexpr int K = 256, NSLAB = K / BK;
  constexpr int BM = 128, BN = 256, WN = 4, NT = 512, TM = 2, TN = 2;
  constexpr int QPS = 16 / NSLAB;
  extern __shared__ __align__(16) unsigned char gemm_smem[];
  _Float16* Ah = reinterpret_cast<_Float16*>(gemm_smem);
  _Float16* Al = Ah + BM * kPlaneStride;
  _Float16* Bh = Al + BM * kPlaneStride;
  _Float16* Bl = Bh + BN * kPlaneStride;
  const int tid = threadIdx.x, wave = tid >> 6, lane = tid & 63;
  const int wm = wave / WN, wn = wave % WN;
  const int l31 = lane & 31, lh = lane >> 5;
  const int gx = (N + BN - 1) / BN;

  float sa, sb, unscale;
  {
    float* shf = reinterpret_cast<float*>(gemm_smem);
    const int ka = pow2_exp_for(block_absmax(a_parts, shf, n_aparts));
    const int kb = pow2_exp_for(block_absmax(w_parts, shf, n_wparts));
    __syncthreads();
    sa = pow2f(ka);
    sb = pow2f(kb);
    unscale = pow2f(-ka - kb);
  }

  f32x16 acc[TM][TN], prev[TM][TN];
  f32x4 ra[BM * BK / 4 / NT], rb[BN * BK / 4 / NT];
  auto load_slab = [&](int m0, int n0, int k0) {
    slab_load<BM, NT>(ra, X, M, K, tid, m0, k0);
    slab_load<BN, NT>(rb, Wt, N, K, tid, n0, k0);
  };
  auto store_slab = [&]() {
    slab_store<BM, NT>(ra, sa, Ah, Al, tid);
    slab_store<BN, NT>(rb, sb, Bh, Bl, tid);
  };

  bool have_prev = false;
  int pm0 = 0, pn0 = 0, ptile = 0;
  float pbias[TN] = {0.f, 0.f};
  float pmax = 0.f;
  auto emit = [&](auto qtag) {
    constexpr int Q = decltype(qtag)::value;
    constexpr int b = Q >> 2, g = Q & 3, bi = b >> 1, bj = b & 1;
    const int row0 = pm0 + (wm * TM + bi) * 32 + 8 * g + 4 * lh;
    const int col = pn0 + (wn * TN + bj) * 32 + l31;
    if (col < N) {
      float* p = out + (size_t)row0 * N + col;
#pragma unroll
      for (int e = 0; e < 4; ++e) {
        float y = prev[bi][bj][4 * g + e] * unscale + pbias[bj];
        if (ACT == SPR_ACT_RELU) y = fmaxf(y, 0.f);
        if (ACT == SPR_ACT_SIGMOID) y = 1.f / (1.f + expf(-y));
        if (row0 + e < M) {
          asm volatile("global_store_dword %0, %1, off" ::"v"(p + (size_t)e * N), "v"(y) : "memory");
          pmax = fmaxf(pmax, fabsf(y));
        }
      }
    }
  };
  auto publish_prev_max = [&]() {
    if (out_parts == nullptr) return;
    float* shf = reinterpret_cast<float*>(gemm_smem);
    const float t_ = wave_max(pmax);
// ... 246 lines not shown
    if (threadIdx.x == 0) {
      const int slot = blockIdx.x & (kLnRangeSlots - 1);
      if (range_norm)
        atomicMax(reinterpret_cast<unsigned int*>(range_norm) + slot,
                  __float_as_uint(fmaxf(fmaxf(shr[0], shr[1]), fmaxf(shr[2], shr[3]))));
      if (range_pos)
        atomicMax(reinterpret_cast<unsigned int*>(range_pos) + slot,
                  __float_as_uint(fmaxf(fmaxf(shr[4], shr[5]), fmaxf(shr[6], shr[7]))));
    }
  }
}

constexpr int kPosembTokens = 16;
constexpr int kPosembMaxFreq = 1024;

__global__ __launch_bounds__(256) void k_posemb(const float* __restrict__ xyz, int n, int d_model, int npf,
                                                float scale, float temperature, float* __restrict__ out) {
  __shared__ float dim_t[kPosembMaxFreq];
  for (int f = threadIdx.x; f < npf / 2; f += 256) dim_t[f] = powf(temperature, (float)(2 * f) / (float)npf);
  __syncthreads();
  const int slots = (d_model + 1) >> 1;
  const bool vec = (d_model & 1) == 0;
  const int row0 = blockIdx.x * kPosembTokens;
  const int rows = min(kPosembTokens, n - row0);
  const int dr = 256 / slots, ds = 256 % slots;
  int r = (int)threadIdx.x / slots, s = (int)threadIdx.x % slots;
  while (r < rows) {
    const int row = row0 + r, ch = 2 * s;
    float v0 = 0.f, v1 = 0.f;
    if (ch < 3 * npf) {
      const int axis = (ch >= npf ? 1 : 0) + (ch >= 2 * npf ? 1 : 0), i = ch - axis * npf;
      const float a = (xyz[3 * (size_t)row + axis] * scale) / dim_t[i >> 1];
      v0 = sinf(a);
      v1 = cosf(a);
    }
    float* o = out + (size_t)row * d_model + ch;
    if (vec) {
      *reinterpret_cast<float2*>(o) = make_float2(v0, v1);
    } else {
      o[0] = v0;
      if (ch + 1 < d_model) o[1] = v1;
    }
    s += ds;
    r += dr;
    if (s >= slots) {
      s -= slots;
      ++r;
    }
  }
}

}
}

using namespace spr;

namespace {
template <int ACT, bool RES>
int launch_gemm(const float* x, int m, int k, const float* w, int n, const float* bias,
                const float* residual, float* out, const float* a_parts, int n_aparts, const float* w_parts,
                int n_wparts, float* out_parts, int out_cap, int* out_n, hipStream_t stream) {
  if (out_n) *out_n = 0;
  if (spr::g_gemm_mode.load(std::memory_order_relaxed) == 1) {
    SPR_REQUIRE(a_parts != nullptr && w_parts != nullptr, "linear: split-fp16 mode needs the absmax partials");
    auto lds = [](int bm, int bn) { return (size_t)(bm + bn) * spr::kPlaneStride * 2 * sizeof(_Float16); };
    if (!RES && ACT <= SPR_ACT_SIGMOID && n >= 256 && k == 256 && m >= 1024 && m < 32768) {
      auto kern = spr::k_gemm_nt_h3p<ACT>;
      if (int rc = ensure_dyn_lds((const void*)kern, (int)lds(128, 256))) return rc;
      const int ntiles = cdiv(n, 256) * cdiv(m, 128);
      int grid = device_cu_count();
      grid = grid < ntiles ? grid : ntiles;
      if (grid >= 8) grid &= ~7;
      float* op = (out_parts && ntiles <= out_cap) ? out_parts : nullptr;
      if (op && out_n) *out_n = ntiles;
      hipLaunchKernelGGL(kern, dim3(grid), dim3(512), lds(128, 256), stream, x, m, w, n, bias, out,
                         a_parts, n_aparts, w_parts, n_wparts, op, ntiles);
    } else if (n >= 256 && m >= 256 && cdiv(n, 256) * cdiv(m, 256) >= 128) {
      auto kern = spr::k_gemm_nt_h3<256, 256, 4, 2, ACT, RES>;
      if (int rc = ensure_dyn_lds((const void*)kern, (int)lds(256, 256))) return rc;
      const int grid = cdiv(n, 256) * cdiv(m, 256);
      float* op = (out_parts && grid <= out_cap) ? out_parts : nullptr;
      if (op && out_n) *out_n = grid;
      hipLaunchKernelGGL(kern, dim3(grid), dim3(512), lds(256, 256), stream, x, m, k,
                         w, n, bias, residual, out, spr::AttnPlanes(), 0, a_parts, n_aparts, w_parts, op, (const spr::GemmGroup*)nullptr, n_wparts);
    } else if (n > 32) {
      const int grid = cdiv(n, 64) * cdiv(m, 128);
      float* op = (out_parts && grid <= out_cap) ? out_parts : nullptr;
      if (op && out_n) *out_n = grid;
      hipLaunchKernelGGL((spr::k_gemm_nt_h3<128, 64, 4, 1, ACT, RES>), dim3(grid),
                         dim3(256), lds(128, 64), stream, x, m, k, w, n, bias, residual, out, spr::AttnPlanes(), 0,
                         a_parts, n_aparts, w_parts, op, (const spr::GemmGroup*)nullptr, n_wparts);
    } else {
      hipLaunchKernelGGL((spr::k_gemm_nt_h3<128, 32, 4, 1, ACT, RES>), dim3(cdiv(n, 32) * cdiv(m, 128)),
                         dim3(256), lds(128, 32), stream, x, m, k, w, n, bias, residual, out, spr::AttnPlanes(), 0,
                         a_parts, n_aparts, w_parts, (float*)nullptr, (const spr::GemmGroup*)nullptr, n_wparts);
    }
  } else if (n % 64 == 0) {
    hipLaunchKernelGGL((spr::k_gemm_nt<2, 2, ACT, RES>), dim3((n / 64) * cdiv(m, 64)), dim3(256), 0, stream,
                       x, m, k, w, n, bias, residual, out);
  } else {
    hipLaunchKernelGGL((spr::k_gemm_nt<4, 1, ACT, RES>), dim3(cdiv(n, 32) * cdiv(m, 128)), dim3(256), 0,
                       stream, x, m, k, w, n, bias, residual, out);
  }
  SPR_LAUNCH_CHECK();
  return 0;
}
}

int spr::gemm_mode() { return spr::g_gemm_mode.load(std::memory_order_relaxed); }

int spr::launch_inproj_planes(const float* x, int m, int k, const float* w, int n, const float* bias, int f0,
                              const AttnPlanes& planes, const float* a_parts, int n_aparts, const float* w_parts,
                              hipStream_t stream) {
  SPR_REQUIRE(n % 256 == 0 && f0 % 256 == 0 && k % BK == 0 && m >= 1 && bias != nullptr,
              "in-projection planes: bad shape (m=%d k=%d n=%d)", m, k, n);
  SPR_REQUIRE(a_parts && w_parts && planes.scales, "in-projection planes: missing scale inputs");
  auto kern = spr::k_gemm_nt_h3<256, 256, 4, 2, SPR_ACT_NONE, false, true>;
  const size_t lds = (size_t)(256 + 256) * spr::kPlaneStride * 2 * sizeof(_Float16);
  if (int rc = ensure_dyn_lds((const void*)kern, (int)lds)) return rc;
  hipLaunchKernelGGL(kern, dim3(cdiv(n, 256) * cdiv(m, 256)), dim3(512), lds, stream, x, m, k, w, n, bias,
                     (const float*)nullptr, (float*)nullptr, planes, f0, a_parts, n_aparts, w_parts, (float*)nullptr,
                     (const spr::GemmGroup*)nullptr, kAmaxParts);
  SPR_LAUNCH_CHECK();
  return 0;
}

int spr::launch_linear_ranged(const float* x, int m, int k, const float* w, int n, const float* bias,
                              float* out, const float* a_parts, const float* w_parts, hipStream_t stream) {
  return launch_gemm<SPR_ACT_NONE, false>(x, m, k, w, n, bias, nullptr, out, a_parts, kAmaxParts, w_parts, kAmaxParts,
                                          nullptr, 0, nullptr, stream);
}

void spr::gemm_group_tile(int max_n, int* bm, int* bn) {
  if (max_n >= 256) { *bm = 256; *bn = 256; }
  else if (max_n > 32) { *bm = 128; *bn = 64; }
  else { *bm = 128; *bn = 32; }
}

namespace {
template <int ACT>
int launch_grouped_act(const float* a, int k, const float* b, float* c, const spr::GemmGroup* groups_dev,
                       int total_tiles, int max_n, const float* a_parts, const float* w_parts, const float* epi,
                       hipStream_t stream) {
  auto lds = [](int bm, int bn) { return (size_t)(bm + bn) * spr::kPlaneStride * 2 * sizeof(_Float16); };
  int bm, bn;
  spr::gemm_group_tile(max_n, &bm, &bn);
  if (bn == 256) {
    auto kern = spr::k_gemm_nt_h3<256, 256, 4, 2, ACT, false>;
    if (int rc = ensure_dyn_lds((const void*)kern, (int)lds(256, 256))) return rc;
    hipLaunchKernelGGL(kern, dim3(total_tiles), dim3(512), lds(256, 256), stream, a, 0, k, b, 0, epi,
                       (const float*)nullptr, c, spr::AttnPlanes(), 0, a_parts, kAmaxParts, w_parts,
                       (float*)nullptr, groups_dev, kAmaxParts);
  } else if (bn == 64) {
    hipLaunchKernelGGL((spr::k_gemm_nt_h3<128, 64, 4, 1, ACT, false>), dim3(total_tiles), dim3(256),
                       lds(128, 64), stream, a, 0, k, b, 0, epi, (const float*)nullptr, c, spr::AttnPlanes(), 0,
                       a_parts, kAmaxParts, w_parts, (float*)nullptr, groups_dev, kAmaxParts);
  } else {
    hipLaunchKernelGGL((spr::k_gemm_nt_h3<128, 32, 4, 1, ACT, false>), dim3(total_tiles), dim3(256),
                       lds(128, 32), stream, a, 0, k, b, 0, epi, (const float*)nullptr, c, spr::AttnPlanes(), 0,
                       a_parts, kAmaxParts, w_parts, (float*)nullptr, groups_dev, kAmaxParts);
  }
  SPR_LAUNCH_CHECK();
  return 0;
}
}

int spr::launch_gemm_grouped(const float* a, int k, const float* b, float* c, const GemmGroup* groups_dev,
                             int total_tiles, int max_n, const float* a_parts, const float* w_parts,
                             int epi_mode, const float* epi, hipStream_t stream) {
  SPR_REQUIRE(spr::gemm_mode() == 1 && a_parts && w_parts && groups_dev && total_tiles >= 1 && k % BK == 0,
              "grouped gemm: bad arguments");
  SPR_REQUIRE(epi_mode == 0 || epi != nullptr, "grouped gemm: epilogue parameters missing");
  switch (epi_mode) {
    case 0: return launch_grouped_act<SPR_ACT_NONE>(a, k, b, c, groups_dev, total_tiles, max_n, a_parts, w_parts,
                                                    nullptr, stream);
    case kEpiScale: return launch_grouped_act<kEpiScale>(a, k, b, c, groups_dev, total_tiles, max_n, a_parts,
                                                         w_parts, epi, stream);
  }
  SPR_REQUIRE(false, "grouped gemm: unknown epilogue %d", epi_mode);
  return 1;
}

namespace {
struct LinearWs {
  float *ap, *wp;
};
LinearWs linear_layout(Workspace& w) {
  LinearWs l;
  l.ap = w.take<float>(kAmaxParts);
  l.wp = w.take<float>(kAmaxParts);
  return l;
}
}

extern "C" size_t spr_linear_workspace_bytes(void) {
  return measure(linear_layout);
}

extern "C" int spr_linear(const float* x, int m, int k, const float* w, int n, const float* bias,
                          const float* residual, int act, float* out, const float* x_range, int x_range_n,
                          const float* w_range, int w_range_n, float* out_range, int out_range_cap,
                          int* out_range_n_host, void* ws, size_t ws_bytes, void* stream_) {
  hipStream_t stream = (hipStream_t)stream_;
  if (out_range_n_host) *out_range_n_host = 0;
  SPR_REQUIRE(m > 0 && k > 0 && n > 0, "linear: bad sizes m=%d k=%d n=%d", m, k, n);
  SPR_REQUIRE(act >= 0 && act <= 2, "linear: unknown activation %d", act);
  SPR_REQUIRE(x_range == nullptr || x_range_n >= 1, "linear: x_range needs a count");
  SPR_REQUIRE(w_range == nullptr || w_range_n >= 1, "linear: w_range needs a count");
  if (n < 16 || k % BK != 0) {
    SPR_REQUIRE(n <= 64 || k % BK == 0, "linear: k must be a multiple of %d for n > 64 (k=%d n=%d)", BK, k, n);
    const long waves = (long)m * n;
    hipLaunchKernelGGL(k_gemv_rows, dim3(cdiv(waves * 64, 256)), dim3(256), 0, stream, x, m, k, w, n,
                       bias, residual, act, out);
    SPR_LAUNCH_CHECK();
    return 0;
  }
  const float *a_parts = nullptr, *w_parts = nullptr;
  int n_ap = kAmaxParts, n_wp = kAmaxParts;
  if (spr::gemm_mode() == 1) {
    Workspace wk(ws, ws_bytes);
    const auto [ap, wp] = linear_layout(wk);
    SPR_REQUIRE(ws != nullptr && wk.ok(),
                "linear: workspace too small (%zu bytes given, spr_linear_workspace_bytes() needed)", ws_bytes);
    a_parts = x_range != nullptr ? x_range : ap;
    w_parts = w_range != nullptr ? w_range : wp;
    if (x_range != nullptr) n_ap = x_range_n;
    if (w_range != nullptr) n_wp = w_range_n;
    if (x_range == nullptr && w_range == nullptr) {
      if (int rc = launch_absmax2(x, m, k, k, ap, w, n, k, k, wp, stream)) return rc;
    } else if (x_range == nullptr) {
      if (int rc = launch_absmax(x, m, k, k, ap, stream)) return rc;
    } else if (w_range == nullptr) {
      if (int rc = launch_absmax(w, n, k, k, wp, stream)) return rc;
    }
  }
  const bool res = residual != nullptr;
#define SPR_LG(A, R) launch_gemm<A, R>(x, m, k, w, n, bias, residual, out, a_parts, n_ap, w_parts, n_wp, out_range, \
                                       out_range_cap, out_range_n_host, stream)
  switch (act * 2 + (res ? 1 : 0)) {
    case 0: return SPR_LG(SPR_ACT_NONE, false);
    case 1: return SPR_LG(SPR_ACT_NONE, true);
    case 2: return SPR_LG(SPR_ACT_RELU, false);
    case 3: return SPR_LG(SPR_ACT_RELU, true);
// ... 49 lines not shown
```

superpoints_registration_amd/csrc/norm_pool.hip:

```cpp
#include "spr_common.h"

namespace spr {
namespace {

constexpr int kSliceRows = 512;
int in_nsplit(int max_len) {
  int s = cdiv(max_len > 0 ? max_len : 1, kSliceRows);
  return s < 1 ? 1 : s;
}

__global__ __launch_bounds__(256) void k_in_stats(const float* __restrict__ x,
                                                  const int* __restrict__ cu, int c, int nsplit,
                                                  double* __restrict__ part ) {
  const int cloud = blockIdx.x, split = blockIdx.y, cb = blockIdx.z * 64;
  const int beg = cu[cloud], end = cu[cloud + 1];
  const int r0 = beg + split * kSliceRows;
  const int r1 = min(r0 + kSliceRows, end);
  const int cw = min(c - cb, 64);
  const int cw4 = cw >> 2;
  const int rl = 256 / cw4;
  const int tc = threadIdx.x % cw4, tr = threadIdx.x / cw4;
  __shared__ double sh[8][256];
  double s[4] = {0, 0, 0, 0}, ss[4] = {0, 0, 0, 0};
  if (tr < rl) {
    const float* base = x + cb + 4 * tc;
    int r = r0 + tr;
    for (; r + 3 * rl < r1; r += 4 * rl) {
      float4 v[4];
#pragma unroll
      for (int u = 0; u < 4; ++u)
        v[u] = *reinterpret_cast<const float4*>(base + (size_t)(r + u * rl) * c);
#pragma unroll
      for (int u = 0; u < 4; ++u) {
        const double a = v[u].x, b = v[u].y, cc = v[u].z, d = v[u].w;
        s[0] += a; ss[0] += a * a;
        s[1] += b; ss[1] += b * b;
        s[2] += cc; ss[2] += cc * cc;
        s[3] += d; ss[3] += d * d;
      }
    }
    for (; r < r1; r += rl) {
      const float4 v = *reinterpret_cast<const float4*>(base + (size_t)r * c);
      const double a = v.x, b = v.y, cc = v.z, d = v.w;
      s[0] += a; ss[0] += a * a;
      s[1] += b; ss[1] += b * b;
      s[2] += cc; ss[2] += cc * cc;
      s[3] += d; ss[3] += d * d;
    }
  }
#pragma unroll
  for (int k = 0; k < 4; ++k) {
    sh[k][threadIdx.x] = s[k];
    sh[4 + k][threadIdx.x] = ss[k];
  }
  __syncthreads();
  if (tr == 0) {
    double* p = part + (((size_t)cloud * nsplit + split) * 2) * c;
#pragma unroll
    for (int k = 0; k < 4; ++k) {
      double a = s[k], b = ss[k];
      for (int q = 1; q < rl; ++q) {
        a += sh[k][q * cw4 + tc];
        b += sh[4 + k][q * cw4 + tc];
      }
      p[cb + 4 * tc + k] = a;
      p[c + cb + 4 * tc + k] = b;
    }
  }
}

__global__ void k_in_final(const double* __restrict__ part, const int* __restrict__ cu, int nb,
                           int c, int nsplit, float eps, float* __restrict__ mean,
                           float* __restrict__ rstd) {
  const int i = blockIdx.x * blockDim.x + threadIdx.x;
  if (i >= nb * c) return;
  const int cloud = i / c, ch = i % c;
  double s = 0.0, ss = 0.0;
  for (int k = 0; k < nsplit; ++k) {
    const double* p = part + (((size_t)cloud * nsplit + k) * 2) * c;
    s += p[ch];
    ss += p[c + ch];
  }
  const int len = cu[cloud + 1] - cu[cloud];
  const double n = len > 0 ? (double)len : 1.0;
  const double m = s / n;
  double var = ss / n - m * m;
  if (var < 0.0) var = 0.0;
  mean[i] = (float)m;
  rstd[i] = (float)(1.0 / sqrt(var + (double)eps));
}

constexpr int kInApplyUnroll = 4;
__global__ __launch_bounds__(256) void k_in_apply(const float* __restrict__ x, const int* __restrict__ cu, int n,
                                                  int nb, int c, int norm, const float* __restrict__ mean,
                                                  const float* __restrict__ rstd, const float* __restrict__ add,
                                                  float slope, float* __restrict__ out,
                                                  float* __restrict__ out_range, int nslots) {
  const int c4 = c >> 2;
  const long total = (long)n * c4;
  const long stride = (long)gridDim.x * blockDim.x;
  const long g0 = (long)blockIdx.x * blockDim.x + threadIdx.x;
  float4 v[kInApplyUnroll], a[kInApplyUnroll];
#pragma unroll
  for (int u = 0; u < kInApplyUnroll; ++u) {
    const long gid = g0 + u * stride;
    if (gid < total) {
      v[u] = reinterpret_cast<const float4*>(x)[gid];
      if (add) a[u] = reinterpret_cast<const float4*>(add)[gid];
    }
  }
  float mx = 0.f;
#pragma unroll
  for (int u = 0; u < kInApplyUnroll; ++u) {
    const long gid = g0 + u * stride;
    if (gid >= total) continue;
    float4 w = v[u];
    if (norm) {
      const int row = (int)(gid / c4), q = (int)(gid % c4);
      const int cloud = find_segment(cu, nb, row);
      const float4 m = reinterpret_cast<const float4*>(mean + (size_t)cloud * c)[q];
      const float4 r = reinterpret_cast<const float4*>(rstd + (size_t)cloud * c)[q];
      w.x = (w.x - m.x) * r.x;
      w.y = (w.y - m.y) * r.y;
      w.z = (w.z - m.z) * r.z;
      w.w = (w.w - m.w) * r.w;
    }
    if (add) {
      w.x += a[u].x;
      w.y += a[u].y;
      w.z += a[u].z;
      w.w += a[u].w;
    }
    w.x = w.x >= 0.f ? w.x : w.x * slope;
    w.y = w.y >= 0.f ? w.y : w.y * slope;
    w.z = w.z >= 0.f ? w.z : w.z * slope;
    w.w = w.w >= 0.f ? w.w : w.w * slope;
    reinterpret_cast<float4*>(out)[gid] = w;
    mx = fmaxf(mx, fmaxf(fmaxf(fabsf(w.x), fabsf(w.y)), fmaxf(fabsf(w.z), fabsf(w.w))));
  }
  if (out_range != nullptr) publish_range(mx, out_range, nslots);
}

__global__ __launch_bounds__(256) void k_in_bwd_stats(const float* __restrict__ x, const float* __restrict__ out,
                                                      const float* __restrict__ dout, const int* __restrict__ cu,
                                                      int c, int nsplit, float slope,
                                                      const float* __restrict__ mean, const float* __restrict__ rstd,
                                                      double* __restrict__ part ) {
  const int cloud = blockIdx.x, split = blockIdx.y, cb = blockIdx.z * 64;
  const int beg = cu[cloud], end = cu[cloud + 1];
  const int r0 = beg + split * kSliceRows;
  const int r1 = min(r0 + kSliceRows, end);
  const int cw = min(c - cb, 64);
  const int cw4 = cw >> 2;
  const int rl = 256 / cw4;
  const int tc = threadIdx.x % cw4, tr = threadIdx.x / cw4;
  __shared__ double sh[8][256];
  double s1[4] = {0, 0, 0, 0}, s2[4] = {0, 0, 0, 0};
  if (tr < rl) {
    const int col = cb + 4 * tc;
    const float4 mu = *reinterpret_cast<const float4*>(mean + (size_t)cloud * c + col);
    const float4 rs = *reinterpret_cast<const float4*>(rstd + (size_t)cloud * c + col);
    for (int r = r0 + tr; r < r1; r += rl) {
      const size_t o = (size_t)r * c + col;
      const float4 xv = *reinterpret_cast<const float4*>(x + o);
      const float4 ov = *reinterpret_cast<const float4*>(out + o);
      const float4 dv = *reinterpret_cast<const float4*>(dout + o);
      const float g0 = dv.x * (ov.x > 0.f ? 1.f : slope), g1 = dv.y * (ov.y > 0.f ? 1.f : slope);
      const float g2 = dv.z * (ov.z > 0.f ? 1.f : slope), g3 = dv.w * (ov.w > 0.f ? 1.f : slope);
      s1[0] += (double)g0; s2[0] += (double)g0 * (double)((xv.x - mu.x) * rs.x);
      s1[1] += (double)g1; s2[1] += (double)g1 * (double)((xv.y - mu.y) * rs.y);
      s1[2] += (double)g2; s2[2] += (double)g2 * (double)((xv.z - mu.z) * rs.z);
      s1[3] += (double)g3; s2[3] += (double)g3 * (double)((xv.w - mu.w) * rs.w);
    }
  }
#pragma unroll
  for (int k = 0; k < 4; ++k) {
    sh[k][threadIdx.x] = s1[k];
    sh[4 + k][threadIdx.x] = s2[k];
  }
  __syncthreads();
  if (tr == 0) {
    double* p = part + (((size_t)cloud * nsplit + split) * 2) * c;
#pragma unroll
    for (int k = 0; k < 4; ++k) {
      double a = s1[k], b = s2[k];
      for (int q = 1; q < rl; ++q) {
        a += sh[k][q * cw4 + tc];
        b += sh[4 + k][q * cw4 + tc];
      }
      p[cb + 4 * tc + k] = a;
      p[c + cb + 4 * tc + k] = b;
    }
  }
}

__global__ void k_in_bwd_final(const double* __restrict__ part, const int* __restrict__ cu, int nb, int c,
                               int nsplit, double* __restrict__ m1, double* __restrict__ m2) {
  const int i = blockIdx.x * blockDim.x + threadIdx.x;
  if (i >= nb * c) return;
  const int cloud = i / c, ch = i % c;
  double s1 = 0.0, s2 = 0.0;
  for (int k = 0; k < nsplit; ++k) {
    const double* p = part + (((size_t)cloud * nsplit + k) * 2) * c;
    s1 += p[ch];
    s2 += p[c + ch];
  }
  const int len = cu[cloud + 1] - cu[cloud];
  const double n = len > 0 ? (double)len : 1.0;
  m1[i] = s1 / n;
  m2[i] = s2 / n;
}

__global__ void k_in_bwd_apply(const float* __restrict__ x, const float* __restrict__ out,
                               const float* __restrict__ dout, const int* __restrict__ cu, int n, int nb, int c,
                               int norm, float slope, const float* __restrict__ mean,
                               const float* __restrict__ rstd, const double* __restrict__ m1,
                               const double* __restrict__ m2, float* __restrict__ dx, float* __restrict__ dadd) {
  const long gid = (long)blockIdx.x * blockDim.x + threadIdx.x;
  if (gid >= (long)n * c) return;
  const int row = (int)(gid / c), ch = (int)(gid % c);
  const float g = dout[gid] * (out[gid] > 0.f ? 1.f : slope);
// ... 75 lines not shown
    float4 v = make_float4(0.f, 0.f, 0.f, 0.f);
    if (id >= 0 && id < ns) v = reinterpret_cast<const float4*>(x + (size_t)id * c)[q];
    m.x = fmaxf(m.x, v.x);
    m.y = fmaxf(m.y, v.y);
    m.z = fmaxf(m.z, v.z);
    m.w = fmaxf(m.w, v.w);
  }
  reinterpret_cast<float4*>(out)[gid] = m;
  mx = fmaxf(fmaxf(fabsf(m.x), fabsf(m.y)), fmaxf(fabsf(m.z), fabsf(m.w)));
  }
  if (out_range != nullptr) publish_range(mx, out_range, nslots);
}

__global__ void k_gather_rows(const float* __restrict__ x, int n_src, int c,
                              const int* __restrict__ idx, int n, float* __restrict__ out) {
  const long gid = (long)blockIdx.x * blockDim.x + threadIdx.x;
  if (gid >= (long)n * c) return;
  const int row = (int)(gid / c), ch = (int)(gid % c);
  const int id = idx[row];
  out[gid] = (id >= 0 && id < n_src) ? x[(size_t)id * c + ch] : 0.f;
}

}

int instnorm_slice_rows() { return kSliceRows; }
int instnorm_nsplit(int max_len) { return in_nsplit(max_len); }
void launch_in_final(const double* part, const int* cu, int nb, int c, int nsplit, float eps, float* mean,
                     float* rstd, hipStream_t stream) {
  hipLaunchKernelGGL(k_in_final, dim3(cdiv((long)nb * c, 256)), dim3(256), 0, stream, part, cu, nb, c, nsplit, eps,
                     mean, rstd);
}
}

using namespace spr;

namespace {
struct InstnormWs {
  double* part;
  float *mean, *rstd;
  double *m1, *m2;
};
InstnormWs instnorm_layout(Workspace& w, int max_len, int nb, int c, bool backward) {
  const size_t B = (size_t)(nb > 0 ? nb : 1), C = (size_t)(c > 0 ? c : 1);
  InstnormWs l{};
  l.part = w.take<double>(B * in_nsplit(max_len) * 2 * C);
  l.mean = w.take<float>(B * C);
  l.rstd = w.take<float>(B * C);
  if (backward) {
    l.m1 = w.take<double>(B * C);
    l.m2 = w.take<double>(B * C);
  }
  return l;
}
}

extern "C" size_t spr_instnorm_workspace_bytes(int max_len, int nb, int c) {
  return measure(instnorm_layout, max_len, nb, c, false);
}

extern "C" int spr_instnorm(const float* x, const int* cu, int n, int nb, int max_len_host, int c,
                            float eps, int norm, const float* add, float slope, float* out, float* out_range,
                            int out_range_n, void* ws, size_t ws_bytes, void* stream_) {
  hipStream_t stream = (hipStream_t)stream_;
  SPR_REQUIRE(out_range == nullptr || (out_range_n >= 1 && (out_range_n & (out_range_n - 1)) == 0),
              "instnorm: out_range_n must be a power of two");
  SPR_REQUIRE(n > 0 && nb >= 1 && c >= 4 && c % 4 == 0, "instnorm: need n>0 and c %% 4 == 0 (c=%d)", c);
  float* mean = nullptr;
  float* rstd = nullptr;
  if (norm) {
    SPR_REQUIRE(max_len_host >= 1 && max_len_host <= n, "instnorm: bad max_len_host=%d", max_len_host);
    Workspace w(ws, ws_bytes);
    const InstnormWs l = instnorm_layout(w, max_len_host, nb, c, false);
    SPR_REQUIRE(ws != nullptr && w.ok(), "instnorm: workspace too small");
    const int nsplit = in_nsplit(max_len_host);
    double* part = l.part;
    mean = l.mean;
    rstd = l.rstd;
    hipLaunchKernelGGL(k_in_stats, dim3(nb, nsplit, cdiv(c, 64)), dim3(256), 0, stream, x, cu, c, nsplit, part);
    hipLaunchKernelGGL(k_in_final, dim3(cdiv((long)nb * c, 256)), dim3(256), 0, stream, part, cu,
                       nb, c, nsplit, eps, mean, rstd);
    SPR_LAUNCH_CHECK();
  }
  const long total = (long)n * (c / 4);
  hipLaunchKernelGGL(k_in_apply, dim3(cdiv(total, 256 * kInApplyUnroll)), dim3(256), 0, stream, x, cu, n, nb, c,
                     norm, mean, rstd, add, slope, out, out_range, out_range_n);
  SPR_LAUNCH_CHECK();
  return 0;
}

extern "C" int spr_instnorm_stats(const float* x, const int* cu, int n, int nb, int max_len_host, int c, float eps,
                                  float* mean, float* rstd, void* ws, size_t ws_bytes, void* stream_) {
  hipStream_t stream = (hipStream_t)stream_;
  SPR_REQUIRE(x && cu && mean && rstd && n > 0 && nb >= 1 && c >= 4 && c % 4 == 0, "instnorm_stats: bad arguments (c=%d)", c);
  SPR_REQUIRE(max_len_host >= 1 && max_len_host <= n, "instnorm_stats: bad max_len_host=%d", max_len_host);
  Workspace w(ws, ws_bytes);
  double* part = instnorm_layout(w, max_len_host, nb, c, false).part;
  SPR_REQUIRE(ws != nullptr && w.ok(), "instnorm_stats: workspace too small");
  const int nsplit = in_nsplit(max_len_host);
  hipLaunchKernelGGL(k_in_stats, dim3(nb, nsplit, cdiv(c, 64)), dim3(256), 0, stream, x, cu, c, nsplit, part);
  hipLaunchKernelGGL(k_in_final, dim3(cdiv((long)nb * c, 256)), dim3(256), 0, stream, part, cu, nb, c, nsplit, eps, mean,
                     rstd);
  SPR_LAUNCH_CHECK();
  return 0;
}

extern "C" size_t spr_instnorm_bwd_workspace_bytes(int max_len, int nb, int c) {
  return measure(instnorm_layout, max_len, nb, c, true);
}

extern "C" int spr_instnorm_bwd(const float* x, const float* out, const float* dout, const int* cu, int n, int nb,
                                int max_len_host, int c, float eps, int norm, float slope, float* dx, float* dadd,
                                void* ws, size_t ws_bytes, void* stream_) {
  hipStream_t stream = (hipStream_t)stream_;
  SPR_REQUIRE(n > 0 && nb >= 1 && c >= 4 && c % 4 == 0, "instnorm_bwd: need n>0 and c %% 4 == 0 (c=%d)", c);
  SPR_REQUIRE(x && out && dout && dx, "instnorm_bwd: null operand");
  float *mean = nullptr, *rstd = nullptr;
  double *m1 = nullptr, *m2 = nullptr;
  if (norm) {
    SPR_REQUIRE(max_len_host >= 1 && max_len_host <= n, "instnorm_bwd: bad max_len_host=%d", max_len_host);
    Workspace w(ws, ws_bytes);
    const InstnormWs l = instnorm_layout(w, max_len_host, nb, c, true);
    SPR_REQUIRE(ws != nullptr && w.ok(), "instnorm_bwd: workspace too small");
    const int nsplit = in_nsplit(max_len_host);
    double* part = l.part;
    mean = l.mean; rstd = l.rstd; m1 = l.m1; m2 = l.m2;
    hipLaunchKernelGGL(k_in_stats, dim3(nb, nsplit, cdiv(c, 64)), dim3(256), 0, stream, x, cu, c, nsplit, part);
    hipLaunchKernelGGL(k_in_final, dim3(cdiv((long)nb * c, 256)), dim3(256), 0, stream, part, cu, nb, c, nsplit,
                       eps, mean, rstd);
    hipLaunchKernelGGL(k_in_bwd_stats, dim3(nb, nsplit, cdiv(c, 64)), dim3(256), 0, stream, x, out, dout, cu, c, nsplit, slope,
                       mean, rstd, part);
    hipLaunchKernelGGL(k_in_bwd_final, dim3(cdiv((long)nb * c, 256)), dim3(256), 0, stream, part, cu, nb, c, nsplit,
                       m1, m2);
    SPR_LAUNCH_CHECK();
  }
  if (c % 4 == 0 && (((uintptr_t)x | (uintptr_t)out | (uintptr_t)dout | (uintptr_t)dx | (uintptr_t)dadd) & 15) == 0)
    hipLaunchKernelGGL(k_in_bwd_apply4, dim3(cdiv((long)n * (c / 4), 256)), dim3(256), 0, stream, x, out, dout, cu, n, nb,
                       c, norm, slope, mean, rstd, m1, m2, dx, dadd);
  else
    hipLaunchKernelGGL(k_in_bwd_apply, dim3(cdiv((long)n * c, 256)), dim3(256), 0, stream, x, out, dout, cu, n, nb, c,
                       norm, slope, mean, rstd, m1, m2, dx, dadd);
  SPR_LAUNCH_CHECK();
  return 0;
}

extern "C" int spr_maxpool_gather(const float* x, int ns, int c, const int* idx, int nq, int idx_stride, int k,
                                  const int* order, float* out, float* out_range, int out_range_n, void* stream_) {
  hipStream_t stream = (hipStream_t)stream_;
  SPR_REQUIRE(out_range == nullptr || (out_range_n >= 1 && (out_range_n & (out_range_n - 1)) == 0),
              "maxpool: out_range_n must be a power of two");
  SPR_REQUIRE(nq > 0 && ns > 0 && c % 4 == 0 && k >= 1 && k <= idx_stride, "maxpool: bad arguments");
  const long total = (long)nq * (c / 4);
  const long nblk = order != nullptr ? align_up((size_t)cdiv(total, 256), 8) : cdiv(total, 256);
  hipLaunchKernelGGL(k_maxpool, dim3((unsigned)nblk), dim3(256), 0, stream, x, ns, c, idx, nq, idx_stride, k, out,
                     out_range, out_range_n, order);
  SPR_LAUNCH_CHECK();
  return 0;
}

extern "C" int spr_gather_rows(const float* x, int n_src, int c, const int* idx, int n, float* out,
                               void* stream_) {
  hipStream_t stream = (hipStream_t)stream_;
  SPR_REQUIRE(n > 0 && c >= 1, "gather_rows: bad arguments");
  const long total = (long)n * c;
  hipLaunchKernelGGL(k_gather_rows, dim3(cdiv(total, 256)), dim3(256), 0, stream, x, n_src, c, idx,
                     n, out);
  SPR_LAUNCH_CHECK();
  return 0;
}
// ... 1 lines not shown
```

superpoints_registration_amd/csrc/spr_common.h:

```cpp
#pragma once
#include <hip/hip_runtime.h>

#include <cstdarg>
#include <cstdio>
#include <cstdint>
#include <cstring>

#include "../../include/spr.h"

namespace spr {

constexpr int kWave = 64;

void set_error(const char* fmt, ...);

#define SPR_HIP_CHECK(expr)                                                   \
  do {                                                                        \
    hipError_t _e = (expr);                                                   \
    if (_e != hipSuccess) {                                                   \
      ::spr::set_error("%s failed: %s (%s:%d)", #expr, hipGetErrorString(_e), \
                       __FILE__, __LINE__);                                   \
      return 1;                                                               \
    }                                                                         \
  } while (0)
// ... 8 lines not shown
    }                                                                       \
  } while (0)

#define SPR_REQUIRE(cond, ...)        \
  do {                                \
    if (!(cond)) {                    \
      ::spr::set_error(__VA_ARGS__);  \
      return 2;                       \
    }                                 \
  } while (0)

static inline size_t align_up(size_t x, size_t a) { return (x + a - 1) / a * a; }
static inline int cdiv(long a, long b) { return (int)((a + b - 1) / b); }

struct Workspace {
  char* base;
  size_t size;
  size_t off;
  bool failed;
  Workspace() : base(nullptr), size(SIZE_MAX), off(0), failed(false) {}
  Workspace(void* p, size_t n) : base((char*)p), size(n), off(0), failed(false) {}
  bool ok() const { return !failed; }
  size_t used() const { return failed ? SIZE_MAX : off; }
  template <typename T>
  T* take(size_t count) {
    if (count > (SIZE_MAX - 255) / sizeof(T)) {
      failed = true;
      return nullptr;
    }
    size_t bytes = align_up(count * sizeof(T), 256);
    if (bytes > size - off) {
      failed = true;
      return nullptr;
    }
    T* r = base ? (T*)(base + off) : nullptr;
    off += bytes;
    return r;
  }
};
template <typename Layout, typename... Args>
size_t measure(Layout layout, Args... args) {
  Workspace w;
  layout(w, args...);
  return w.used();
}

bool prof_enabled();
void prof_push(hipEvent_t beg, hipEvent_t end, int code, int n);
struct ProfScope {
  hipStream_t stream;
  bool on;
  hipEvent_t beg, end;
  int code, n;
  ProfScope(hipStream_t s, int code_, int n_) : stream(s), on(prof_enabled()), code(code_), n(n_) {
    if (!on) return;
    if (hipEventCreate(&beg) != hipSuccess || hipEventCreate(&end) != hipSuccess) {
      on = false;
      return;
    }
    (void)hipEventRecord(beg, stream);
  }
  ~ProfScope() {
    if (!on) return;
    (void)hipEventRecord(end, stream);
    prof_push(beg, end, code, n);
  }
};

int ensure_dyn_lds(const void* kernel, int bytes);
int device_cu_count();

int launch_absmax(const float* x, long rows, int cols, long stride, float* parts, hipStream_t stream);
int launch_absmax2(const float* x0, long rows0, int cols0, long stride0, float* parts0, const float* x1,
                   long rows1, int cols1, long stride1, float* parts1, hipStream_t stream);

void launch_rowflag(const float* x, const float* s_xyz, int ns, int cin, unsigned char* flag, float4* sxf,
                    int* tile_ctr, hipStream_t stream);

int instnorm_slice_rows();
int instnorm_nsplit(int max_len);
void launch_in_final(const double* part, const int* cu, int nb, int c, int nsplit, float eps, float* mean,
                     float* rstd, hipStream_t stream);

#ifdef __HIPCC__
typedef float f32x2 __attribute__((ext_vector_type(2)));
typedef float f32x4 __attribute__((ext_vector_type(4)));
typedef float f32x16 __attribute__((ext_vector_type(16)));
typedef _Float16 f16x2 __attribute__((ext_vector_type(2)));

__device__ __forceinline__ int find_segment(const int* __restrict__ cu, int nseg,
                                            int i) {
  int lo = 0, hi = nseg;
  while (hi - lo > 1) {
    int mid = (lo + hi) >> 1;
    if (cu[mid] <= i)
      lo = mid;
    else
      hi = mid;
  }
  return lo;
}

__device__ __forceinline__ int xcd_swizzle(int b, int nwg) {
  const int q = nwg >> 3, r = nwg & 7;
  const int xcd = b & 7, idx = b >> 3;
  const int base = (xcd < r) ? xcd * (q + 1) : r * (q + 1) + (xcd - r) * q;
  return base + idx;
}

__device__ __forceinline__ void split_pk(float a, float b, unsigned int& hi_u, unsigned int& lo_u) {
  const f16x2 hi = {(_Float16)a, (_Float16)b};
  hi_u = __builtin_bit_cast(unsigned int, hi);
  asm("v_fma_mixlo_f16 %0, %1, -1.0, %2 op_sel_hi:[1,0,0]\n\t"
      "v_fma_mixhi_f16 %0, %1, -1.0, %3 op_sel:[1,0,0] op_sel_hi:[1,0,0]"
      : "=&v"(lo_u)
      : "v"(hi_u), "v"(a), "v"(b));
}

__device__ __forceinline__ void split_pk_s(float a, float b, float s, unsigned int& hi_u,
                                           unsigned int& lo_u) {
  asm("v_fma_mixlo_f16 %0, %1, %3, 0 op_sel_hi:[0,0,0]\n\t"
      "v_fma_mixhi_f16 %0, %2, %3, 0 op_sel_hi:[0,0,0]"
      : "=&v"(hi_u)
      : "v"(a), "v"(b), "v"(s));
  asm("v_fma_mixlo_f16 %0, %2, %4, -%1 op_sel_hi:[0,0,1]\n\t"
      "v_fma_mixhi_f16 %0, %3, %4, -%1 op_sel:[0,0,1] op_sel_hi:[0,0,1]"
      : "=&v"(lo_u)
      : "v"(hi_u), "v"(a), "v"(b), "v"(s));
}

__device__ __forceinline__ void split_pk_s_hi(float a, float b, float s, unsigned int& hi_u) {
  asm("v_fma_mixlo_f16 %0, %1, %3, 0 op_sel_hi:[0,0,0]\n\t"
      "v_fma_mixhi_f16 %0, %2, %3, 0 op_sel_hi:[0,0,0]"
      : "=&v"(hi_u)
      : "v"(a), "v"(b), "v"(s));
}
__device__ __forceinline__ void split_pk_s_lo(float a, float b, float s, unsigned int hi_u, unsigned int& lo_u) {
  asm("v_fma_mixlo_f16 %0, %2, %4, -%1 op_sel_hi:[0,0,1]\n\t"
      "v_fma_mixhi_f16 %0, %3, %4, -%1 op_sel:[0,0,1] op_sel_hi:[0,0,1]"
      : "=&v"(lo_u)
      : "v"(hi_u), "v"(a), "v"(b), "v"(s));
}

__host__ __device__ __forceinline__ int pow2_exp_for(float amax) {
  if (!(amax > 0.f) || !(amax < 3.0e38f)) return 0;
  unsigned int u;
#ifdef __HIP_DEVICE_COMPILE__
  u = __float_as_uint(amax);
#else
  memcpy(&u, &amax, 4);
#endif
  const int e = (int)((u >> 23) & 0xff) - 127;
  int k = 14 - e;
  if (k > 60) k = 60;
  if (k < -60) k = -60;
  return k;
}
__host__ __device__ __forceinline__ float pow2f(int k) {
  const unsigned int u = (unsigned int)(127 + k) << 23;
  float f;
#ifdef __HIP_DEVICE_COMPILE__
  f = __uint_as_float(u);
#else
  memcpy(&f, &u, 4);
#endif
  return f;
// ... 57 lines not shown
```

superpoints_registration_amd/kpconv_blocks.py:

```python
import math

import torch
import torch.nn as nn
from torch.nn.init import kaiming_uniform_
from torch.nn.parameter import Parameter

from . import _concurrency, kpconv_modes, ops, stem
from .kernel_points import load_kernels


def _cu_of(batch, layer_ind):
    cache = batch.setdefault('_cu', {})
    cu = cache.get(layer_ind)
    if cu is None:
        cu = ops.lengths_to_cu(batch['stack_lengths'][layer_ind],
                               batch['points'][layer_ind].device)
        cache[layer_ind] = cu
    return cu


def _maxlen_of(batch, layer_ind):
    lens = batch.get('_lens_host')
    return max(lens[layer_ind]) if lens is not None else None


def _idx_of(batch, key, layer_ind):
    cache = batch.setdefault('_i32', {})
    t = cache.get((key, layer_ind))
    if t is None:
        t = batch[key][layer_ind].to(torch.int32)
        cache[(key, layer_ind)] = t
    return t


def gather(x, idx, method=2):
    if idx.dim() == 1:
        return ops.gather_rows(x, idx.to(torch.int32))
    flat = ops.gather_rows(x, idx.reshape(-1).to(torch.int32))
    return flat.view(*idx.shape, x.shape[1])


def _pool_order_of(batch, level):
    po = batch.get('pool_order') if isinstance(batch, dict) else None
    return po[level] if po is not None and level < len(po) else None


def max_pool(x, inds, order=None):
    return ops.maxpool(x, inds, order)


def closest_pool(x, inds):
    return ops.gather_rows(x, inds[:, 0].contiguous().to(torch.int32))


class KPConv(nn.Module):

    def __init__(self, kernel_size, p_dim, in_channels, out_channels, KP_extent, radius,
                 fixed_kernel_points='center', KP_influence='linear', aggregation_mode='sum',
                 deformable=False, modulated=False):
        super().__init__()
        if deformable or modulated:
            raise NotImplementedError("deformable / modulated KPConv is outside the hot-path scope")
        kpconv_modes.mode_codes(KP_influence, aggregation_mode)
        self.K = kernel_size
        self.p_dim = p_dim
        self.in_channels = in_channels
        self.out_channels = out_channels
        self.radius = radius
        self.KP_extent = KP_extent
        self.fixed_kernel_points = fixed_kernel_points
        self.KP_influence = KP_influence
        self.aggregation_mode = aggregation_mode
        self.deformable = deformable
        self.modulated = modulated
        self.rows_sorted = False
        self.impl = 0

        self.weights = Parameter(torch.zeros((self.K, in_channels, out_channels), dtype=torch.float32),
                                 requires_grad=True)
        self.reset_parameters()
        self.kernel_points = self.init_KP()

    def reset_parameters(self):
        kaiming_uniform_(self.weights, a=math.sqrt(5))

    def init_KP(self):
        K_points_numpy = load_kernels(self.radius, self.K, dimension=self.p_dim,
                                      fixed=self.fixed_kernel_points)
        return Parameter(torch.tensor(K_points_numpy, dtype=torch.float32), requires_grad=False)

    def forward(self, q_pts, s_pts, neighb_inds, x):
        if kpconv_modes.is_default_mode(self.KP_influence, self.aggregation_mode):
            return ops.kpconv(q_pts, s_pts, neighb_inds, x, self.weights,
                              self.kernel_points.detach(), self.KP_extent,
                              rows_sorted=self.rows_sorted, impl=self.impl)
        return kpconv_modes.kpconv(q_pts, s_pts, neighb_inds, x, self.weights, self.kernel_points.detach(),
                                   self.KP_extent, self.KP_influence, self.aggregation_mode)

    def __repr__(self):
        return 'KPConv(radius: {:.2f}, extent: {:.2f}, in_feat: {:d}, out_feat: {:d})'.format(
            self.radius, self.KP_extent, self.in_channels, self.out_channels)


DEFORMABLE_SIMPLE = ('simple_deformable', 'simple_deformable_strided')
DEFORMABLE_RESNET = ('resnetb_deformable', 'resnetb_deformable_strided')


def deformable_enabled(config) -> bool:
    return bool(getattr(config, 'deformable_kpconv', False))


def _block_kpconv(block_name, config, in_dim, out_dim, extent, radius):
    kw = dict(fixed_kernel_points=config.fixed_kernel_points, KP_influence=config.KP_influence,
              aggregation_mode=config.aggregation_mode)
    optin = deformable_enabled(config)
    if optin and 'deform' in block_name:
        from . import deformable
        return deformable.KPConvDeformable(config.num_kernel_points, config.in_points_dim, in_dim, out_dim, extent,
                                           radius, deformable=True, modulated=config.modulated, **kw)
    return KPConv(config.num_kernel_points, config.in_points_dim, in_dim, out_dim, extent, radius,
                  deformable='deform' in block_name, modulated=False if optin else config.modulated, **kw)


def block_decider(block_name, radius, in_dim, out_dim, layer_ind, config):
    if block_name in DEFORMABLE_SIMPLE and deformable_enabled(config):
        return SimpleBlock(block_name, in_dim, out_dim, radius, layer_ind, config)
    elif block_name in DEFORMABLE_RESNET and deformable_enabled(config):
        return ResnetBottleneckBlock(block_name, in_dim, out_dim, radius, layer_ind, config)
    elif block_name == 'unary':
        return UnaryBlock(in_dim, out_dim, config.use_batch_norm, config.batch_norm_momentum)
    elif block_name in ['simple', 'simple_strided']:
        return SimpleBlock(block_name, in_dim, out_dim, radius, layer_ind, config)
    elif block_name in ['resnetb', 'resnetb_strided']:
        return ResnetBottleneckBlock(block_name, in_dim, out_dim, radius, layer_ind, config)
    elif block_name == 'nearest_upsample':
        return NearestUpsampleBlock(layer_ind)
    else:
        raise ValueError('Unknown / unsupported block name in the architecture definition : ' + block_name)


class BatchNormBlock(nn.Module):

    def __init__(self, in_dim, use_bn, bn_momentum):
        super().__init__()
        self.bn_momentum = bn_momentum
        self.use_bn = use_bn
        self.in_dim = in_dim
        self.eps = 1e-5
        if not self.use_bn:
            self.bias = Parameter(torch.zeros(in_dim, dtype=torch.float32), requires_grad=True)

    def forward(self, x, stack_lengths, cu=None, add=None, slope=1.0, max_len=None):
        if cu is None:
            cu = ops.lengths_to_cu(stack_lengths, x.device)
        if self.use_bn:
            return ops.instnorm(x, cu, eps=self.eps, norm=True, add=add, slope=slope, max_len=max_len)
        y = x + self.bias
        return ops.instnorm(y, cu, norm=False, add=add, slope=slope, max_len=max_len)

    def __repr__(self):
        return 'BatchNormBlock(in_feat: {:d}, momentum: {:.3f}, only_bias: {:s})'.format(
            self.in_dim, self.bn_momentum, str(not self.use_bn))


class UnaryBlock(nn.Module):

    def __init__(self, in_dim, out_dim, use_bn, bn_momentum, no_relu=False):
        super().__init__()
        self.bn_momentum = bn_momentum
        self.use_bn = use_bn
        self.no_relu = no_relu
        self.in_dim = in_dim
        self.out_dim = out_dim
        self.mlp = nn.Linear(in_dim, out_dim, bias=False)
        self.batch_norm = BatchNormBlock(out_dim, self.use_bn, self.bn_momentum)
        if not no_relu:
            self.leaky_relu = nn.LeakyReLU(0.1)

# ... 34 lines not shown
        if 'strided' in self.block_name:
            q_pts, s_pts = batch['points'][li + 1], batch['points'][li]
            neighb_inds = _idx_of(batch, 'pools', li)
            stack_lengths, cu, ml = batch['stack_lengths'][li + 1], _cu_of(batch, li + 1), _maxlen_of(batch, li + 1)
        else:
            q_pts = s_pts = batch['points'][li]
            neighb_inds = _idx_of(batch, 'neighbors', li)
            stack_lengths, cu, ml = batch['stack_lengths'][li], _cu_of(batch, li), _maxlen_of(batch, li)
        self.KPConv.rows_sorted = bool(batch.get('_rows_sorted', False))
        if self.stem_route(x):
            return stem.kpconv_stem(q_pts, s_pts, neighb_inds, x, self.KPConv.weights,
                                    self.KPConv.kernel_points.detach(), self.KPConv.KP_extent, cu,
                                    eps=self.batch_norm.eps, slope=0.1, rows_sorted=self.KPConv.rows_sorted,
                                    max_len=ml)
        x = self.KPConv(q_pts, s_pts, neighb_inds, x)
        return self.batch_norm(x, stack_lengths, cu=cu, slope=0.1, max_len=ml)


class ResnetBottleneckBlock(nn.Module):

    def __init__(self, block_name, in_dim, out_dim, radius, layer_ind, config):
        super().__init__()
        current_extent = radius * config.KP_extent / config.conv_radius
        self.bn_momentum = config.batch_norm_momentum
        self.use_bn = config.use_batch_norm
        self.block_name = block_name
        self.layer_ind = layer_ind
        self.in_dim = in_dim
        self.out_dim = out_dim
        if in_dim != out_dim // 4:
            self.unary1 = UnaryBlock(in_dim, out_dim // 4, self.use_bn, self.bn_momentum)
        else:
            self.unary1 = nn.Identity()
        self.KPConv = _block_kpconv(block_name, config, out_dim // 4, out_dim // 4, current_extent, radius)
        self.batch_norm_conv = BatchNormBlock(out_dim // 4, self.use_bn, self.bn_momentum)
        self.unary2 = UnaryBlock(out_dim // 4, out_dim, self.use_bn, self.bn_momentum, no_relu=True)
        if in_dim != out_dim:
            self.unary_shortcut = UnaryBlock(in_dim, out_dim, self.use_bn, self.bn_momentum,
                                             no_relu=True)
        else:
            self.unary_shortcut = nn.Identity()
        self.leaky_relu = nn.LeakyReLU(0.1)

    def forward(self, features, batch):
        li = self.layer_ind
        stack_lengths_pre, cu_pre, ml_pre = batch['stack_lengths'][li], _cu_of(batch, li), _maxlen_of(batch, li)
        if 'strided' in self.block_name:
            q_pts, s_pts = batch['points'][li + 1], batch['points'][li]
            neighb_inds = _idx_of(batch, 'pools', li)
            stack_lengths_post, cu_post, ml_post = (batch['stack_lengths'][li + 1], _cu_of(batch, li + 1),
                                                    _maxlen_of(batch, li + 1))
        else:
            q_pts = s_pts = batch['points'][li]
            neighb_inds = _idx_of(batch, 'neighbors', li)
            stack_lengths_post, cu_post, ml_post = batch['stack_lengths'][li], _cu_of(batch, li), ml_pre

        strided = 'strided' in self.block_name
        projected = isinstance(self.unary_shortcut, UnaryBlock)
        mid = self.unary2.in_dim
        fused = (features.is_cuda and not torch.is_grad_enabled() and self.use_bn
                 and ops.block_tail_tile_rows(mid, self.in_dim if projected else 0, self.out_dim) > 0)

        def shortcut_branch():
            sc = max_pool(features, neighb_inds, _pool_order_of(batch, li)) if strided else features
            if projected and not fused:
                sc = self.unary_shortcut(sc, stack_lengths_post, cu=cu_post, max_len=ml_post)
            return sc

        has_work = strided or (projected and not fused)
        fork = (has_work and features.is_cuda and not torch.is_grad_enabled()
                and _concurrency.active(features.device))
        if fork:
            main = torch.cuda.current_stream(features.device)
            branch = _concurrency.aux_stream(main, features.device, 'shortcut')
            ready = torch.cuda.Event()
            ready.record(main)
            branch.wait_event(ready)
            with torch.cuda.stream(branch):
                shortcut = shortcut_branch()
                joined = torch.cuda.Event()
                joined.record(branch)
            features.record_stream(branch)

        x = self.unary1(features, stack_lengths_pre, cu=cu_pre, max_len=ml_pre) \
            if isinstance(self.unary1, UnaryBlock) else features
        self.KPConv.rows_sorted = bool(batch.get('_rows_sorted', False))
        x = self.KPConv(q_pts, s_pts, neighb_inds, x)
        fold = fused and self.use_bn
        conv_stats = None
        if fold:
            conv_stats = ops.instnorm_stats(x, cu_post, eps=self.batch_norm_conv.eps, max_len=ml_post)
        else:
            x = self.batch_norm_conv(x, stack_lengths_post, cu=cu_post, slope=0.1, max_len=ml_post)

        if fork:
            main.wait_event(joined)
            shortcut.record_stream(main)
        else:
            shortcut = shortcut_branch()
        if fused:
            if projected:
                return ops.block_tail(x, self.unary2.mlp.weight, cu_post, xb=shortcut,
                                      wb=self.unary_shortcut.mlp.weight, eps=self.unary2.batch_norm.eps, slope=0.1,
                                      xa_stats=conv_stats, xa_slope=0.1, xa_max_len=ml_post)
            return ops.block_tail(x, self.unary2.mlp.weight, cu_post, add=shortcut,
                                  eps=self.unary2.batch_norm.eps, slope=0.1,
                                  xa_stats=conv_stats, xa_slope=0.1, xa_max_len=ml_post)
        return self.unary2(x, stack_lengths_post, cu=cu_post, add=shortcut, final_slope=0.1,
                           max_len=ml_post)


class NearestUpsampleBlock(nn.Module):

    def __init__(self, layer_ind):
        super().__init__()
        self.layer_ind = layer_ind

    def forward(self, x, batch):
        return closest_pool(x, _idx_of(batch, 'upsamples', self.layer_ind - 1))

    def __repr__(self):
        return 'NearestUpsampleBlock(layer: {:d} -> {:d})'.format(self.layer_ind, self.layer_ind - 1)
```

superpoints_registration_amd/ops.py:

```python
import ctypes
import math
import threading
from typing import Optional, Sequence, Tuple

import numpy as np
import torch

from . import _lib

ACT_NONE, ACT_RELU, ACT_SIGMOID = 0, 1, 2
ORDER_REFERENCE, ORDER_CANONICAL = 0, 1
SELECT_NEAREST, SELECT_INDEX = 0, 1


def _stream(t: torch.Tensor):
    return ctypes.c_void_p(torch.cuda.current_stream(t.device).cuda_stream)


def _ptr(t: Optional[torch.Tensor]):
    return None if t is None else ctypes.c_void_p(t.data_ptr())


def _dev(t: torch.Tensor, name: str, dtype=None) -> torch.Tensor:
    if not isinstance(t, torch.Tensor) or not t.is_cuda:
# ... 435 lines not shown
    def __init__(self, supports: torch.Tensor, s_cu: torch.Tensor, radius: float):
        self.supports = _dev(supports, "supports", torch.float32)
        self.s_cu = _dev(s_cu, "s_cu", torch.int32)
        self.radius = float(radius)
        self.ns, self.nb = self.supports.shape[0], self.s_cu.numel() - 1
        L = _lib.lib()
        self.blob = torch.empty((L.spr_radius_table_bytes(self.ns, self.nb),), dtype=torch.uint8, device=supports.device)
        ws = _workspace(L.spr_radius_table_build_workspace_bytes(self.ns, self.nb), supports.device)
        _lib.check(L.spr_radius_table_build(_ptr(self.supports), _ptr(self.s_cu), self.ns, self.nb, self.radius,
                                            _ptr(self.blob), self.blob.numel(), _ptr(ws), ws.numel(),
                                            _stream(self.supports)), "spr_radius_table_build")
        self._slot = 0
        self._slots = L.spr_radius_table_slots()
        self._built = (_ident(self.supports), _ident(self.s_cu))

    def matches(self, supports: torch.Tensor, s_cu: torch.Tensor, radius: float) -> bool:
        return ((_ident(supports), _ident(s_cu)) == self._built
                and (_ident(self.supports), _ident(self.s_cu)) == self._built
                and supports.shape[0] == self.ns and float(radius) == self.radius and self._slot < self._slots)

    def query(self, queries: torch.Tensor, q_cu: torch.Tensor, limit: int,
              dense: Optional[bool] = None, select: int = SELECT_NEAREST) -> Tuple[torch.Tensor, int]:
        queries = _dev(queries, "queries", torch.float32)
        q_cu = _dev(q_cu, "q_cu", torch.int32)
        nq = queries.shape[0]
        self_search = int(queries.data_ptr() == self.supports.data_ptr() and nq == self.ns
                          and q_cu.data_ptr() == self.s_cu.data_ptr())
        L = _lib.lib()
        ws = _workspace(L.spr_radius_table_query_workspace_bytes(nq), queries.device)
        out = torch.empty((nq, limit), dtype=torch.int32, device=queries.device)
        mc = torch.empty((1,), dtype=torch.int32, device=queries.device)
        slot, self._slot = self._slot, self._slot + 1
        _lib.check(L.spr_radius_table_query(_ptr(queries), _ptr(q_cu), nq, self_search, self.ns, self.nb, self.radius,
                                            int(limit), slot, _ptr(self.blob), _ptr(out), _ptr(mc),
                                            -1 if dense is None else int(bool(dense)), int(select), _ptr(ws),
                                            ws.numel(), _stream(queries)), "spr_radius_table_query")
        m = int(mc.item())
        if m == -2:
            return radius_neighbors(queries, self.supports, q_cu, self.s_cu, self.radius, limit, True, algo=1,
                                    select=select)
        if m < 0:
            raise RuntimeError("spr_radius_neighbors: cloud extent / radius exceeds 8191 cells per axis")
        if select == SELECT_INDEX:
            return out, m
        if m < 1:
            raise RuntimeError("Error")
        return out[:, :min(m, limit)], m

    def count(self, queries: torch.Tensor, q_cu: torch.Tensor, hist_n: Optional[int] = None, *,
              counts: bool = True, hist: Optional[torch.Tensor] = None):
        queries = _dev(queries, "queries", torch.float32)
        q_cu = _dev(q_cu, "q_cu", torch.int32)
        nq = queries.shape[0]
        self_search = int(queries.data_ptr() == self.supports.data_ptr() and nq == self.ns
                          and q_cu.data_ptr() == self.s_cu.data_ptr())
        if hist is not None:
            if (not hist.is_cuda or hist.dtype != torch.int32 or not hist.is_contiguous()
                    or hist.dim() != 2 or hist.shape[0] != self.nb or hist_n not in (None, hist.shape[1])):
                raise ValueError("RadiusTable.count: hist must be a contiguous int32 [nb, hist_n] device tensor")
            hist_n = hist.shape[1]
        elif hist_n is not None:
            hist = torch.zeros((self.nb * max(int(hist_n), 1),), dtype=torch.int32,
                               device=queries.device).view(self.nb, -1)
        out = torch.empty((nq,), dtype=torch.int32, device=queries.device) if counts else None
        st = torch.empty((1,), dtype=torch.int32, device=queries.device)
        _lib.check(_lib.lib().spr_radius_table_count(_ptr(queries), _ptr(q_cu), nq, self_search, self.ns, self.nb,
                                                     self.radius, _ptr(self.blob), _ptr(out), _ptr(hist),
                                                     0 if hist_n is None else int(hist_n), _ptr(st),
                                                     _stream(queries)), "spr_radius_table_count")
        s = int(st.item())
        if s == -2:
            raise RuntimeError("spr_radius_table_count: the clouds' bounding boxes need more cells at this radius than "
                               "the table holds (64 per support point + 2^20); voxelise or split the cloud")
        if s < 0:
            raise RuntimeError("spr_radius_table_count: cloud extent / radius exceeds 8191 cells per axis")
        return out, hist


def _wants_grad(*tensors) -> bool:
    return torch.is_grad_enabled() and any(isinstance(t, torch.Tensor) and t.requires_grad for t in tensors)


def kpconv(q_pts, s_pts, nbr, x, weights, kernel_points, kp_extent: float, rows_sorted: bool = False,
           impl: int = 0) -> torch.Tensor:
    if _wants_grad(x, weights):
        from .autograd import KPConvFn
        return KPConvFn.apply(_dev(q_pts, "q_pts", torch.float32), _dev(s_pts, "s_pts", torch.float32), nbr,
                              _dev(x, "x", torch.float32), weights, kernel_points, float(kp_extent),
                              bool(rows_sorted), int(impl))
    return kpconv_raw(q_pts, s_pts, nbr, x, weights, kernel_points, kp_extent, rows_sorted, impl)


def kpconv_raw(q_pts, s_pts, nbr, x, weights, kernel_points, kp_extent: float, rows_sorted: bool = False,
               impl: int = 0, order: Optional[torch.Tensor] = None) -> torch.Tensor:
    q_pts = _dev(q_pts, "q_pts", torch.float32)
    s_pts = _dev(s_pts, "s_pts", torch.float32)
    x = _dev(x, "x", torch.float32)
    weights = _dev(weights, "weights", torch.float32)
    kernel_points = _dev(kernel_points, "kernel_points", torch.float32)
    if not nbr.is_cuda:
        raise RuntimeError("neighb_inds must be on the device")
    if nbr.dtype != torch.int32:
        nbr = nbr.to(torch.int32)
    stride = nbr.stride(0) if nbr.stride(1) == 1 and nbr.shape[1] > 0 else None
    if stride is None:
        nbr = nbr.contiguous()
        stride = nbr.shape[1]
    nq, ns, kmax = q_pts.shape[0], s_pts.shape[0], nbr.shape[1]
    n_kp, cin, cout = weights.shape
    assert x.shape == (ns, cin), (x.shape, ns, cin)
    L = _lib.lib()
    ws = _workspace(L.spr_kpconv_workspace_bytes(nq, ns, cin, cout), x.device)
    out = torch.empty((nq, cout), dtype=torch.float32, device=x.device)
    xr, xr_n = _get_range(x)
    wr, wr_n = _static_range(weights)
    plan = wplanes = None
    if impl == 0 and n_kp == 15 and cin % 32 == 0 and cout % 32 == 0 and cout <= 256:
        if cin in (32, 64) and cin * cout <= 4096 and kmax <= 128:
            plan = _kpconv_plan(nbr, nq, ns, int(stride), kmax, bool(rows_sorted), order)
        if wr is not None:
            wplanes = _kpconv_wplanes(weights, wr, wr_n)
    _lib.check(L.spr_kpconv_fwd(_ptr(q_pts), nq, _ptr(s_pts), ns, _ptr(nbr), int(stride), kmax,
                                int(bool(rows_sorted)), _ptr(x), cin, _ptr(weights), cout,
                                _ptr(kernel_points), n_kp, float(kp_extent), _ptr(out), int(impl),
                                _ptr(xr), int(xr_n), _ptr(wr), int(wr_n), _ptr(plan), _ptr(wplanes),
                                _ptr(ws), ws.numel(), _stream(x)), "spr_kpconv_fwd")
    return out


def _kpconv_plan(nbr: torch.Tensor, nq: int, ns: int, stride: int, kmax: int, rows_sorted: bool,
                 order: Optional[torch.Tensor] = None) -> torch.Tensor:
    if order is not None:
        order = _dev(order, "order", torch.int32)
        assert order.shape == (nq,)

    def build():
        L = _lib.lib()
        nbytes = L.spr_kpconv_plan_bytes(nq)
        plan = torch.empty((nbytes,), dtype=torch.uint8, device=nbr.device)
        _lib.check(L.spr_kpconv_plan(_ptr(nbr), nq, ns, stride, kmax, int(rows_sorted), _ptr(order), _ptr(plan),
                                     nbytes, _stream(nbr)), "spr_kpconv_plan")
        return plan, plan
    return _derived(nbr, '_spr_kp_plan', (nq, ns, stride, kmax, rows_sorted, None if order is None else _ident(order)),
                    build)


def kpconv_plan_prefetch(nbr: torch.Tensor, ns: int, rows_sorted: bool = True) -> None:
    if nbr is None or not nbr.is_cuda or nbr.dtype != torch.int32 or nbr.dim() != 2 or nbr.shape[1] < 1:
        return
    if nbr.stride(1) != 1 or nbr.shape[1] > 128 or nbr.shape[0] < 1:
        return
    _kpconv_plan(nbr, nbr.shape[0], int(ns), int(nbr.stride(0)), nbr.shape[1], bool(rows_sorted))


def _kpconv_wplanes(weights: torch.Tensor, wr: torch.Tensor, wr_n: int) -> torch.Tensor:
    def build():
        L = _lib.lib()
        n_kp, cin, cout = weights.shape
        nbytes = L.spr_kpconv_wplanes_bytes(cin, cout)
        planes = torch.empty((nbytes,), dtype=torch.uint8, device=weights.device)
        _lib.check(L.spr_kpconv_prep_weights(_ptr(weights), n_kp, cin, cout, _ptr(wr), int(wr_n), _ptr(planes),
                                             nbytes, _stream(weights)), "spr_kpconv_prep_weights")
        return planes, planes
    return _derived(weights, '_spr_kp_wplanes', wr.data_ptr(), build)


def instnorm(x, cu, eps: float = 1e-5, norm: bool = True, add=None, slope: float = 1.0,
             out=None, max_len: Optional[int] = None) -> torch.Tensor:
    if _wants_grad(x, add):
        from .autograd import InstNormFn
        return InstNormFn.apply(_dev(x, "x", torch.float32), _dev(cu, "cu", torch.int32), float(eps), bool(norm),
                                None if add is None else _dev(add, "add", torch.float32), float(slope), max_len)
    return instnorm_raw(x, cu, eps, norm, add, slope, out, max_len)


def instnorm_raw(x, cu, eps: float = 1e-5, norm: bool = True, add=None, slope: float = 1.0,
                 out=None, max_len: Optional[int] = None) -> torch.Tensor:
    x = _dev(x, "x", torch.float32)
    cu = _dev(cu, "cu", torch.int32)
    n, c = x.shape
    nb = cu.numel() - 1
    if add is not None:
        add = _dev(add, "add", torch.float32)
        assert add.shape == x.shape
    if out is None:
        out = torch.empty_like(x)
    L = _lib.lib()
    max_len = n if max_len is None else max(1, min(int(max_len), n))
    ws = _workspace(L.spr_instnorm_workspace_bytes(max_len, nb, c), x.device)
    cnt = _STREAM_SLOTS
    rng = _zero_slots(cnt, x.device)
    _lib.check(L.spr_instnorm(_ptr(x), _ptr(cu), n, nb, max_len, c, float(eps), int(bool(norm)), _ptr(add),
                              float(slope), _ptr(out), _ptr(rng), cnt, _ptr(ws), ws.numel(), _stream(x)),
               "spr_instnorm")
    _set_range(out, rng, cnt)
    return out


def block_tail_tile_rows(ka: int, kb: int, n_out: int) -> int:
    if _modes["gemm"] != 1:
        return 0
    return int(_lib.lib().spr_block_tail_tile_rows(int(ka), int(kb), int(n_out)))


def _tail_tiles(cu: torch.Tensor, n: int, tr: int) -> torch.Tensor:
    def build():
        L = _lib.lib()
        t = torch.empty((L.spr_block_tail_tiles_len(n, cu.numel() - 1, tr),), dtype=torch.int32, device=cu.device)
        _lib.check(L.spr_block_tail_tiles(_ptr(cu), n, cu.numel() - 1, tr, _ptr(t), _stream(cu)), "spr_block_tail_tiles")
        return t, t
    return _derived(cu, f'_spr_tail_tiles_{tr}', (n, tr), build)


def instnorm_stats(x, cu, eps: float = 1e-5, max_len: Optional[int] = None):
    x = _dev(x, "x", torch.float32)
    cu = _dev(cu, "cu", torch.int32)
    n, c = x.shape
    nb = cu.numel() - 1
    L = _lib.lib()
    max_len = n if max_len is None else max(1, min(int(max_len), n))
    ws = _workspace(L.spr_instnorm_workspace_bytes(max_len, nb, c), x.device)
    st = torch.empty((2, nb, c), dtype=torch.float32, device=x.device)
    _lib.check(L.spr_instnorm_stats(_ptr(x), _ptr(cu), n, nb, max_len, c, float(eps), _ptr(st[0]), _ptr(st[1]),
                                    _ptr(ws), ws.numel(), _stream(x)), "spr_instnorm_stats")
    return st[0], st[1]


_NORM_BOUNDS = {}


def _norm_bound(max_len: int, device) -> torch.Tensor:
    key = (int(max_len), str(device))
    t = _NORM_BOUNDS.get(key)
    if t is None:
        t = torch.full((1,), float(max(1, int(max_len))) ** 0.5, dtype=torch.float32, device=device)
        _NORM_BOUNDS[key] = t
    return t


def block_tail(xa, wa, cu, xb=None, wb=None, add=None, eps: float = 1e-5, slope: float = 0.1,
               xa_stats=None, xa_slope: float = 0.1, xa_max_len: Optional[int] = None) -> torch.Tensor:
    xa = _dev(xa, "xa", torch.float32)
    wa = _dev(wa, "wa", torch.float32)
    cu = _dev(cu, "cu", torch.int32)
    n, ka = xa.shape
    n_out = wa.shape[0]
    assert wa.shape[1] == ka
    kb = 0
    if xb is not None:
        xb = _dev(xb, "xb", torch.float32)
        wb = _dev(wb, "wb", torch.float32)
        kb = xb.shape[1]
        assert xb.shape[0] == n and wb.shape == (n_out, kb) and add is None
    if add is not None:
        add = _dev(add, "add", torch.float32)
        assert add.shape == (n, n_out)
    nb = cu.numel() - 1
    L = _lib.lib()
    tr = L.spr_block_tail_tile_rows(ka, kb, n_out)
    if tr <= 0:
        raise RuntimeError(f"block_tail: no kernel for ka={ka} kb={kb} n_out={n_out}")
    tiles = _tail_tiles(cu, n, tr)
    out = torch.empty((n, n_out), dtype=torch.float32, device=xa.device)
    ws = _workspace(L.spr_block_tail_workspace_bytes(n, nb, kb, n_out, tr), xa.device)
    if xa_stats is not None:
        xar, xar_n = _norm_bound(n if xa_max_len is None else xa_max_len, xa.device), 1
    else:
        xar, xar_n = _get_range(xa)
    war, war_n = _static_range(wa)
    xbr, xbr_n, wbr, wbr_n = None, 0, None, 0
    if kb > 0:
        xbr, xbr_n = _get_range(xb)
        wbr, wbr_n = _static_range(wb)
    cnt = _STREAM_SLOTS
    rng = _zero_slots(cnt, xa.device)
    mean = rstd = None
    if xa_stats is not None:
        mean, rstd = xa_stats
        assert mean.shape == (nb, ka) and rstd.shape == (nb, ka) and mean.is_contiguous() and rstd.is_contiguous()
    _lib.check(L.spr_block_tail(_ptr(xa), ka, _ptr(wa), _ptr(xb), kb, _ptr(wb), _ptr(add), _ptr(cu), _ptr(tiles),
                                n, nb, n_out, float(eps), float(slope), _ptr(out), _ptr(xar), int(xar_n),
                                _ptr(war), int(war_n), _ptr(xbr), int(xbr_n), _ptr(wbr), int(wbr_n),
                                _ptr(rng), cnt, _ptr(mean), _ptr(rstd), float(xa_slope), _ptr(ws), ws.numel(),
                                _stream(xa)), "spr_block_tail")
    _set_range(out, rng, cnt)
    return out


def cell_order(points: torch.Tensor, cu: torch.Tensor, cell: float) -> torch.Tensor:
    points = _dev(points, "points", torch.float32)
    cu = _dev(cu, "cu", torch.int32)
    n, nb = points.shape[0], cu.numel() - 1
    L = _lib.lib()
    out = torch.empty((n,), dtype=torch.int32, device=points.device)
    ws = _workspace(L.spr_cell_order_workspace_bytes(n), points.device)
    _lib.check(L.spr_cell_order(_ptr(points), _ptr(cu), n, nb, float(cell), _ptr(out), _ptr(ws), ws.numel(),
                                _stream(points)), "spr_cell_order")
    return out


def maxpool(x, idx, order=None) -> torch.Tensor:
    if _wants_grad(x):
        from .autograd import MaxPoolFn
        return MaxPoolFn.apply(_dev(x, "x", torch.float32), idx)
    return maxpool_raw(x, idx, order)


def maxpool_raw(x, idx, order=None) -> torch.Tensor:
    x = _dev(x, "x", torch.float32)
    if idx.dtype != torch.int32:
        idx = idx.to(torch.int32)
    stride = idx.stride(0) if idx.stride(1) == 1 else None
    if stride is None:
        idx = idx.contiguous()
        stride = idx.shape[1]
    ns, c = x.shape
    nq, k = idx.shape
    out = torch.empty((nq, c), dtype=torch.float32, device=x.device)
    L = _lib.lib()
    cnt = _STREAM_SLOTS
    rng = _zero_slots(cnt, x.device)
    if order is not None and (order.dtype != torch.int32 or order.numel() != nq or not order.is_contiguous()):
        raise ValueError("maxpool: order must be a contiguous int32 permutation of the query rows")
    _lib.check(L.spr_maxpool_gather(_ptr(x), ns, c, _ptr(idx), nq, int(stride), k, _ptr(order), _ptr(out),
                                    _ptr(rng), cnt, _stream(x)), "spr_maxpool_gather")
    _set_range(out, rng, cnt)
    return out


def linear(x, weight, bias=None, residual=None, act: int = ACT_NONE) -> torch.Tensor:
    if _wants_grad(x, weight, bias, residual):
        from .autograd import LinearFn
        return LinearFn.apply(_dev(x, "x", torch.float32), weight, bias, residual, int(act))
    return linear_raw(x, weight, bias, residual, act)


def linear_raw(x, weight, bias=None, residual=None, act: int = ACT_NONE) -> torch.Tensor:
    x = _dev(x, "x", torch.float32)
    weight = _dev(weight, "weight", torch.float32)
    m, k = x.shape
    n = weight.shape[0]
    assert weight.shape[1] == k
    if bias is not None:
        bias = _dev(bias, "bias", torch.float32)
    if residual is not None:
        residual = _dev(residual, "residual", torch.float32)
        assert residual.shape == (m, n)
    out = torch.empty((m, n), dtype=torch.float32, device=x.device)
    L = _lib.lib()
    ws = _workspace(L.spr_linear_workspace_bytes(), x.device)
    xr, xr_n = _get_range(x)
    wr, wr_n = _static_range(weight)
    orng = torch.empty((_RANGE_CAP,), dtype=torch.float32, device=x.device) if residual is None else None
    on = ctypes.c_int(0)
    _lib.check(L.spr_linear(_ptr(x), m, k, _ptr(weight), n, _ptr(bias), _ptr(residual), int(act), _ptr(out),
                            _ptr(xr), int(xr_n), _ptr(wr), int(wr_n), _ptr(orng),
                            _RANGE_CAP if orng is not None else 0, ctypes.byref(on),
                            _ptr(ws), ws.numel(), _stream(x)), "spr_linear")
    if orng is not None:
        _set_range(out, orng, on.value)
    return out


DEFAULT_ATTN_MODE = 4

_modes = {"gemm": 1, "attn": DEFAULT_ATTN_MODE}


def set_gemm_mode(mode: int) -> None:
# ... 807 lines not shown
```

Before: 1288 pairs/s.

## Fuse ResNet block head unary+instnorm and emit KPConv row-flag records

Adds a block_head path that runs the bottleneck block's first unary linear through a per-cloud tiled GEMM whose epilogue writes per-column sum and sum-of-squares partials. Instance norm and leaky ReLU are then applied from those partials. The same head also writes the KPConv row-flag/sxf records, so the following KPConv skips its own rowflag kernel launch. The aim is to cut separate GEMM, norm and rowflag passes and their memory round-trips. In exchange it adds a new launch path, statistics computed in double, and a cached per-stream records blob.

New measurement: 1299 pairs/s, median of 6. No clear change (+0.9%).

```diff
diff --git a/include/spr.h b/include/spr.h
--- a/include/spr.h
+++ b/include/spr.h
@@ -119,6 +119,7 @@
                             const float* rot, const int* dir_cols_host, int n_dir, float* out, void* stream);
 
 size_t spr_kpconv_workspace_bytes(int nq, int ns, int cin, int cout);
+size_t spr_kpconv_records_size(int ns);
 size_t spr_kpconv_plan_bytes(int nq);
 int spr_kpconv_plan(const int* nbr, int nq, int ns, int nbr_stride, int kmax, int rows_sorted,
                     const int* order, void* plan, size_t plan_bytes, void* stream);
@@ -130,7 +131,7 @@
                    const float* weights, int cout, const float* kernel_points, int n_kp,
                    float kp_extent, float* out, int impl, const float* x_range, int x_range_n,
                    const float* w_range, int w_range_n, const void* plan, const void* wplanes,
-                   void* ws, size_t ws_bytes, void* stream);
+                   void* ws, size_t ws_bytes, void* stream, const void* records);
 
 #define SPR_KP_CONSTANT 0
 #define SPR_KP_LINEAR 1
@@ -214,6 +215,14 @@
                    int wa_range_n, const float* xb_range, int xb_range_n, const float* wb_range,
                    int wb_range_n, float* out_range, int out_range_n, const float* xa_mean,
                    const float* xa_rstd, float xa_slope, void* ws, size_t ws_bytes, void* stream);
+
+int spr_block_head_supported(int k, int n_out);
+int spr_block_head_tile_rows(void);
+size_t spr_block_head_workspace_size(int n, int nb, int n_out);
+int spr_block_head(const float* x, int k, const float* w, const int* cu, const int* tiles, int n, int nb, int n_out,
+                   float eps, int norm, float slope, float* out, float* stats_out, const float* x_range,
+                   int x_range_n, const float* w_range, int w_range_n, float* out_range, int out_range_n,
+                   const float* s_xyz, void* records, size_t records_bytes, void* ws, size_t ws_bytes, void* stream);
 
 int spr_maxpool_gather(const float* x, int ns, int c, const int* idx, int nq, int idx_stride, int k,
                        const int* order, float* out, float* out_range, int out_range_n, void* stream);
diff --git a/superpoints_registration_amd/_lib.py b/superpoints_registration_amd/_lib.py
--- a/superpoints_registration_amd/_lib.py
+++ b/superpoints_registration_amd/_lib.py
@@ -61,7 +61,8 @@
     "spr_feats_gather_rotate": (_i, [_vp, _i, _i, _vp, _i, _vp, _i, _vp, _vp, _i, _vp, _vp]),
     "spr_kpconv_workspace_bytes": (_sz, [_i, _i, _i, _i]),
     "spr_kpconv_fwd": (_i, [_vp, _i, _vp, _i, _vp, _i, _i, _i, _vp, _i, _vp, _i, _vp, _i, _f, _vp, _i, _vp, _i, _vp,
-                            _i, _vp, _vp, _vp, _sz, _vp]),
+                            _i, _vp, _vp, _vp, _sz, _vp, _vp]),
+    "spr_kpconv_records_size": (_sz, [_i]),
     "spr_kpconv_modes_workspace_size": (_sz, [_i, _i, _i, _i]),
     "spr_kpconv_modes_fwd": (_i, [_vp, _i, _vp, _i, _vp, _i, _i, _vp, _i, _vp, _i, _vp, _i, _f, _i, _i, _vp, _i, _vp,
                                   _i, _vp, _i, _vp, _vp, _sz, _vp]),
@@ -105,6 +106,11 @@
     "spr_block_tail_workspace_bytes": (_sz, [_i, _i, _i, _i, _i]),
     "spr_block_tail": (_i, [_vp, _i, _vp, _vp, _i, _vp, _vp, _vp, _vp, _i, _i, _i, _f, _f, _vp, _vp, _i, _vp, _i,
                             _vp, _i, _vp, _i, _vp, _i, _vp, _vp, _f, _vp, _sz, _vp]),
+    "spr_block_head_supported": (_i, [_i, _i]),
+    "spr_block_head_tile_rows": (_i, []),
+    "spr_block_head_workspace_size": (_sz, [_i, _i, _i]),
+    "spr_block_head": (_i, [_vp, _i, _vp, _vp, _vp, _i, _i, _i, _f, _i, _f, _vp, _vp, _vp, _i, _vp, _i, _vp, _i, _vp,
+                            _vp, _sz, _vp, _sz, _vp]),
     "spr_instnorm_stats": (_i, [_vp, _vp, _i, _i, _i, _i, _f, _vp, _vp, _vp, _sz, _vp]),
     "spr_cell_order_workspace_bytes": (_sz, [_i]),
     "spr_cell_order": (_i, [_vp, _vp, _i, _i, _f, _vp, _vp, _sz, _vp]),
diff --git a/superpoints_registration_amd/csrc/block_tail.hip b/superpoints_registration_amd/csrc/block_tail.hip
--- a/superpoints_registration_amd/csrc/block_tail.hip
+++ b/superpoints_registration_amd/csrc/block_tail.hip
@@ -410,13 +410,19 @@
 }
 
 }
+
+void launch_tail_final(const double* part, const int* cu, const int* tile_cu, int nb, int nbr, int n_total, float eps,
+                       float* stats, hipStream_t stream) {
+  hipLaunchKernelGGL(k_tail_final, dim3(cdiv((long)nb * nbr * n_total, 256)), dim3(256), 0, stream, part, cu, tile_cu, nb,
+                     nbr, n_total, eps, stats);
+}
 }
 
 using namespace spr;
 
 extern "C" int spr_block_tail_tile_rows(int ka, int kb, int n_out) { return tail_shape(ka, kb, n_out).tr; }
 
-static size_t tiles_desc_offset(int nb) { return align_up((size_t)(nb > 0 ? nb : 0) + 1, 4); }
+static size_t tiles_desc_offset(int nb) { return tail_tiles_desc_offset(nb); }
 extern "C" size_t spr_block_tail_tiles_len(int n, int nb, int tile_rows) {
   return tiles_desc_offset(nb) + 4 * ((size_t)cdiv(n > 0 ? n : 1, tile_rows > 0 ? tile_rows : 64) + (size_t)(nb > 0 ? nb : 1));
 }
diff --git a/superpoints_registration_amd/csrc/kp_records.h b/superpoints_registration_amd/csrc/kp_records.h
--- /dev/null
+++ b/superpoints_registration_amd/csrc/kp_records.h
@@ -0,0 +1,58 @@
+#pragma once
+#include "spr_common.h"
+
+namespace spr {
+
+struct KpRecords {
+  unsigned char* flag;
+  float4* sxf;
+  int* tile_ctr;
+};
+static inline KpRecords records_view(Workspace& w, int ns) {
+  const size_t n = (size_t)(ns > 0 ? ns : 1);
+  KpRecords r;
+  r.flag = w.take<unsigned char>(n);
+  r.sxf = w.take<float4>(n + 1);
+  r.tile_ctr = w.take<int>(64);
+  return r;
+}
+
+__host__ __device__ static inline bool rowflag_wide(int cin) {
+  const int c4 = cin >> 2;
+  return cin >= 4 && (cin & 3) == 0 && c4 <= 64 && (c4 & (c4 - 1)) == 0;
+}
+
+#ifdef __HIPCC__
+__device__ __forceinline__ float rowflag_wide_sum(const float4 v, int c4, int lane) {
+  float c[4] = {v.x, v.y, v.z, v.w};
+#pragma unroll
+  for (int e = 0; e < 4; ++e) {
+    float t = c[e];
+    if (c4 == 64) {
+      const int b = lane & 15;
+      const float a0 = __shfl(t, b, 64), a1 = __shfl(t, b | 16, 64), a2 = __shfl(t, b | 32, 64),
+                  a3 = __shfl(t, b | 48, 64);
+      t = ((a0 + a1) + a2) + a3;
+    } else if (c4 == 32) {
+      t += __shfl_xor(t, 16, 64);
+    }
+    for (int o = (c4 < 16 ? c4 : 16) >> 1; o > 0; o >>= 1) t += __shfl_xor(t, o, 64);
+    c[e] = t;
+  }
+  return (c[0] + c[2]) + (c[1] + c[3]);
+}
+
+__device__ __forceinline__ void rowflag_write(float sum, int row, const float* __restrict__ s_xyz,
+                                              unsigned char* __restrict__ flag, float4* __restrict__ sxf) {
+  const int f = sum > 0.f ? 1 : 0;
+  flag[row] = (unsigned char)f;
+  sxf[row] = make_float4(s_xyz[3 * (size_t)row], s_xyz[3 * (size_t)row + 1], s_xyz[3 * (size_t)row + 2],
+                         __int_as_float(f));
+}
+__device__ __forceinline__ void rowflag_shadow(int ns, float4* __restrict__ sxf, int* __restrict__ tile_ctr) {
+  sxf[ns] = make_float4(-1.0e17f, -1.0e17f, -1.0e17f, __int_as_float(0));
+  tile_ctr[0] = 0;
+}
+#endif
+
+}
diff --git a/superpoints_registration_amd/csrc/kpconv.hip b/superpoints_registration_amd/csrc/kpconv.hip
--- a/superpoints_registration_amd/csrc/kpconv.hip
+++ b/superpoints_registration_amd/csrc/kpconv.hip
@@ -1,3 +1,4 @@
+#include "kp_records.h"
 #include "lds_dma.h"
 #include "spr_common.h"
 #include "split_mma.h"
@@ -13,11 +14,8 @@
   const int wid = (blockIdx.x * blockDim.x + threadIdx.x) >> 6;
   const int lane = threadIdx.x & 63;
   const int c4 = cin >> 2;
-  if (blockIdx.x == 0 && threadIdx.x == 0) {
-    sxf[ns] = make_float4(-1.0e17f, -1.0e17f, -1.0e17f, __int_as_float(0));
-    tile_ctr[0] = 0;
-  }
-  if ((cin & 3) == 0 && c4 <= 64 && (c4 & (c4 - 1)) == 0) {
+  if (blockIdx.x == 0 && threadIdx.x == 0) rowflag_shadow(ns, sxf, tile_ctr);
+  if (rowflag_wide(cin)) {
     constexpr int kRfSteps = 4;
     const int rpl = 64 / c4;
     const int sub = lane / c4, chunk = lane % c4;
@@ -32,28 +30,8 @@
 #pragma unroll
     for (int r = 0; r < kRfSteps; ++r) {
       const int row = row0 + r * rpl;
-      float c[4] = {v[r].x, v[r].y, v[r].z, v[r].w};
-#pragma unroll
-      for (int e = 0; e < 4; ++e) {
-        float t = c[e];
-        if (c4 == 64) {
-          const int b = lane & 15;
-          const float a0 = __shfl(t, b, 64), a1 = __shfl(t, b | 16, 64), a2 = __shfl(t, b | 32, 64),
-                      a3 = __shfl(t, b | 48, 64);
-          t = ((a0 + a1) + a2) + a3;
-        } else if (c4 == 32) {
-          t += __shfl_xor(t, 16, 64);
-        }
-        for (int o = (c4 < 16 ? c4 : 16) >> 1; o > 0; o >>= 1) t += __shfl_xor(t, o, 64);
-        c[e] = t;
-      }
-      const float t = (c[0] + c[2]) + (c[1] + c[3]);
-      if (chunk == 0 && row < ns) {
-        const int f = t > 0.f ? 1 : 0;
-        flag[row] = (unsigned char)f;
-        sxf[row] = make_float4(s_xyz[3 * (size_t)row], s_xyz[3 * (size_t)row + 1],
-                               s_xyz[3 * (size_t)row + 2], __int_as_float(f));
-      }
+      const float t = rowflag_wide_sum(v[r], c4, lane);
+      if (chunk == 0 && row < ns) rowflag_write(t, row, s_xyz, flag, sxf);
     }
     return;
   }
@@ -62,12 +40,7 @@
   float s = 0.f;
   for (int c = lane; c < cin; c += 64) s += x[(size_t)row * cin + c];
   s = wave_sum(s);
-  if (lane == 0) {
-    const int f = s > 0.f ? 1 : 0;
-    flag[row] = (unsigned char)f;
-    sxf[row] = make_float4(s_xyz[3 * (size_t)row], s_xyz[3 * (size_t)row + 1],
-                           s_xyz[3 * (size_t)row + 2], __int_as_float(f));
-  }
+  if (lane == 0) rowflag_write(s, row, s_xyz, flag, sxf);
 }
 
 __global__ void k_kpconv_simple(const float* __restrict__ q_xyz, int nq,
@@ -1266,7 +1239,7 @@
 void launch_rowflag(const float* x, const float* s_xyz, int ns, int cin, unsigned char* flag, float4* sxf,
                     int* tile_ctr, hipStream_t stream) {
   const int c4 = cin >> 2;
-  const bool wide = (cin & 3) == 0 && c4 <= 64 && (c4 & (c4 - 1)) == 0;
+  const bool wide = rowflag_wide(cin);
   const long waves = wide ? cdiv(ns, (64 / c4) * 4) : (long)ns;
   hipLaunchKernelGGL(k_rowflag, dim3(cdiv(waves * 64, 256)), dim3(256), 0, stream, x, s_xyz, ns, cin, flag, sxf, tile_ctr);
 }
@@ -1301,6 +1274,9 @@
   p.hi = w.take<_Float16>(n);
   p.lo = w.take<_Float16>(n);
   return p;
+}
+extern "C" size_t spr_kpconv_records_size(int ns) {
+  return measure(records_view, ns);
 }
 struct KpWs {
   unsigned char* flag;
@@ -1451,17 +1427,23 @@
                               const float* kernel_points, int n_kp, float kp_extent,
                               float* out, int impl, const float* x_range, int x_range_n, const float* w_range,
                               int w_range_n, const void* plan, const void* wplanes, void* ws, size_t ws_bytes,
-                              void* stream_) {
+                              void* stream_, const void* records) {
   hipStream_t stream = (hipStream_t)stream_;
   SPR_REQUIRE((x_range == nullptr || x_range_n >= 1) && (w_range == nullptr || w_range_n >= 1),
               "kpconv: a range needs a count");
+  SPR_REQUIRE(records == nullptr || ((uintptr_t)records & 15) == 0, "kpconv: the records blob must be 16-byte aligned");
   SPR_REQUIRE(nq > 0 && ns > 0, "kpconv: empty input");
   SPR_REQUIRE(kmax >= 1 && kmax <= nbr_stride, "kpconv: bad kmax=%d stride=%d", kmax, nbr_stride);
   SPR_REQUIRE(cin >= 1 && cout >= 1 && n_kp >= 1 && n_kp <= 32, "kpconv: bad dims");
   SPR_REQUIRE(kp_extent > 0.f, "kpconv: KP_extent must be > 0");
   Workspace w(ws, ws_bytes);
-  const auto [flag, sxf, own_wplanes, x_parts, w_parts, own_plan, tile_ctr, few_rec] = kpconv_layout(w, nq, ns, cin, cout);
+  const auto [own_flag, own_sxf, own_wplanes, x_parts, w_parts, own_plan, own_ctr, few_rec] = kpconv_layout(w, nq, ns, cin, cout);
   SPR_REQUIRE(ws != nullptr && w.ok(), "kpconv: workspace too small");
+  Workspace given_r(const_cast<void*>(records), SIZE_MAX);
+  const KpRecords rec = records != nullptr ? records_view(given_r, ns) : KpRecords{own_flag, own_sxf, own_ctr};
+  unsigned char* const flag = rec.flag;
+  float4* const sxf = rec.sxf;
+  int* const tile_ctr = rec.tile_ctr;
   SPR_REQUIRE(wplanes == nullptr || w_range != nullptr, "kpconv: prepared weight planes come with the range they were scaled by");
   Workspace given_w(const_cast<void*>(wplanes), SIZE_MAX), given_p(const_cast<void*>(plan), SIZE_MAX);
   const auto [wh, wl] = wplanes != nullptr ? wplanes_view(given_w, cin, cout) : own_wplanes;
@@ -1492,7 +1474,7 @@
     return 0;
   }
 
-  launch_rowflag(x, s_xyz, ns, cin, flag, sxf, tile_ctr, stream);
+  if (records == nullptr) launch_rowflag(x, s_xyz, ns, cin, flag, sxf, tile_ctr, stream);
   SPR_LAUNCH_CHECK();
 
   const bool tile_fits = cin % 64 == 0 ? mfma_lds_bytes(64, kTile64TQ, kTileWaves, kmax) <= kMfmaLdsMax
diff --git a/superpoints_registration_amd/csrc/linear.hip b/superpoints_registration_amd/csrc/linear.hip
--- a/superpoints_registration_amd/csrc/linear.hip
+++ b/superpoints_registration_amd/csrc/linear.hip
@@ -143,13 +143,19 @@
   store_tile<ACT, RES>(acc, m0 + wm * 32, col, M, N, bv, residual, out, lh);
 }
 
-template <int BM, int BN, int WM, int WN, int ACT, bool RES, bool PLANES = false>
+struct HeadTiles {
+  const int* tile_cu;
+  const int4* desc;
+  int nb;
+  double* part;
+};
+template <int BM, int BN, int WM, int WN, int ACT, bool RES, bool PLANES = false, bool HEAD = false>
 __global__ __launch_bounds__(WM* WN * 64) void k_gemm_nt_h3(
     const float* __restrict__ Xp, int Mp, int K, const float* __restrict__ Wp, int Np,
     const float* __restrict__ bias, const float* __restrict__ residual,
     float* __restrict__ outp, AttnPlanes pl, int f0, const float* __restrict__ a_parts, int n_aparts,
     const float* __restrict__ w_parts, float* __restrict__ out_parts,
-    const GemmGroup* __restrict__ groups, int n_wparts) {
+    const GemmGroup* __restrict__ groups, int n_wparts, HeadTiles head) {
   constexpr int NT = WM * WN * 64;
   const float* __restrict__ X = Xp;
   const float* __restrict__ Wt = Wp;
@@ -176,7 +182,14 @@
   const int wm = wave / WN, wn = wave % WN;
   const int gx = (N + BN - 1) / BN;
   const int lid = groups != nullptr ? bid : xcd_swizzle(bid, nblk);
-  const int m0 = (lid / gx) * BM, n0 = (lid % gx) * BN;
+  int mt0 = (lid / gx) * BM;
+  if constexpr (HEAD) {
+    if (lid / gx >= head.tile_cu[head.nb]) return;
+    const int4 d = head.desc[lid / gx];
+    mt0 = d.x;
+    M = d.x + d.y;
+  }
+  const int m0 = mt0, n0 = (lid % gx) * BN;
   const int l31 = lane & 31, lh = lane >> 5;
 
   float sa, sb, unscale;
@@ -293,6 +306,41 @@
     for (int i = 0; i < TM; ++i)
       omax = fmaxf(omax, store_tile<ACT, RES>(acc[i][j], m0 + (wm * TM + i) * 32, col, M, N, bv, residual, out, lh,
                                               unscale, ACT >= kEpiScale ? bias : nullptr));
+  }
+  if constexpr (HEAD) {
+    static_assert(!HEAD || (WN == 1 && TM == 1 && ACT == SPR_ACT_NONE && !RES && !PLANES), "head epilogue shape");
+    double* shd = reinterpret_cast<double*>(gemm_smem);
+#pragma unroll
+    for (int j = 0; j < TN; ++j) {
+      const int col = n0 + j * 32 + l31;
+      double s = 0.0, ss = 0.0;
+      if (col < N) {
+#pragma unroll
+        for (int r = 0; r < 16; ++r) {
+          const int row = m0 + wm * 32 + acc_row32(r, lh);
+          const double v = (double)(acc[0][j][r] * unscale + 0.f);
+          if (row < M) {
+            s += v;
+            ss += v * v;
+          }
+        }
+      }
+      shd[((wm * 2 + lh) * 2 + 0) * BN + j * 32 + l31] = s;
+      shd[((wm * 2 + lh) * 2 + 1) * BN + j * 32 + l31] = ss;
+    }
+    __syncthreads();
+    if (tid < BN && n0 + tid < N) {
+      double s = 0.0, ss = 0.0;
+#pragma unroll
+      for (int h = 0; h < WM * 2; ++h) {
+        s += shd[(h * 2 + 0) * BN + tid];
+        ss += shd[(h * 2 + 1) * BN + tid];
+      }
+      double* p = head.part + (size_t)(lid / gx) * 2 * N + n0 + tid;
+      p[0] = s;
+      p[N] = ss;
+    }
+    return;
   }
   if (out_parts != nullptr) {
     float* shf = reinterpret_cast<float*>(gemm_smem);
@@ -705,18 +753,18 @@
       float* op = (out_parts && grid <= out_cap) ? out_parts : nullptr;
       if (op && out_n) *out_n = grid;
       hipLaunchKernelGGL(kern, dim3(grid), dim3(512), lds(256, 256), stream, x, m, k,
-                         w, n, bias, residual, out, spr::AttnPlanes(), 0, a_parts, n_aparts, w_parts, op, (const spr::GemmGroup*)nullptr, n_wparts);
+                         w, n, bias, residual, out, spr::AttnPlanes(), 0, a_parts, n_aparts, w_parts, op, (const spr::GemmGroup*)nullptr, n_wparts, spr::HeadTiles());
     } else if (n > 32) {
       const int grid = cdiv(n, 64) * cdiv(m, 128);
       float* op = (out_parts && grid <= out_cap) ? out_parts : nullptr;
       if (op && out_n) *out_n = grid;
       hipLaunchKernelGGL((spr::k_gemm_nt_h3<128, 64, 4, 1, ACT, RES>), dim3(grid),
                          dim3(256), lds(128, 64), stream, x, m, k, w, n, bias, residual, out, spr::AttnPlanes(), 0,
-                         a_parts, n_aparts, w_parts, op, (const spr::GemmGroup*)nullptr, n_wparts);
+                         a_parts, n_aparts, w_parts, op, (const spr::GemmGroup*)nullptr, n_wparts, spr::HeadTiles());
     } else {
       hipLaunchKernelGGL((spr::k_gemm_nt_h3<128, 32, 4, 1, ACT, RES>), dim3(cdiv(n, 32) * cdiv(m, 128)),
                          dim3(256), lds(128, 32), stream, x, m, k, w, n, bias, residual, out, spr::AttnPlanes(), 0,
-                         a_parts, n_aparts, w_parts, (float*)nullptr, (const spr::GemmGroup*)nullptr, n_wparts);
+                         a_parts, n_aparts, w_parts, (float*)nullptr, (const spr::GemmGroup*)nullptr, n_wparts, spr::HeadTiles());
     }
   } else if (n % 64 == 0) {
     hipLaunchKernelGGL((spr::k_gemm_nt<2, 2, ACT, RES>), dim3((n / 64) * cdiv(m, 64)), dim3(256), 0, stream,
@@ -743,7 +791,7 @@
   if (int rc = ensure_dyn_lds((const void*)kern, (int)lds)) return rc;
   hipLaunchKernelGGL(kern, dim3(cdiv(n, 256) * cdiv(m, 256)), dim3(512), lds, stream, x, m, k, w, n, bias,
                      (const float*)nullptr, (float*)nullptr, planes, f0, a_parts, n_aparts, w_parts, (float*)nullptr,
-                     (const spr::GemmGroup*)nullptr, kAmaxParts);
+                     (const spr::GemmGroup*)nullptr, kAmaxParts, spr::HeadTiles());
   SPR_LAUNCH_CHECK();
   return 0;
 }
@@ -752,6 +800,30 @@
                               float* out, const float* a_parts, const float* w_parts, hipStream_t stream) {
   return launch_gemm<SPR_ACT_NONE, false>(x, m, k, w, n, bias, nullptr, out, a_parts, kAmaxParts, w_parts, kAmaxParts,
                                           nullptr, 0, nullptr, stream);
+}
+
+int spr::launch_gemm_head(const float* x, int k, const float* w, int n_out, float* out, const int* tiles, int nb,
+                          int max_tiles, const float* a_parts, int n_aparts, const float* w_parts, int n_wparts,
+                          double* part, hipStream_t stream) {
+  SPR_REQUIRE(spr::gemm_mode() == 1 && k >= BK && k % BK == 0 && n_out >= 16 && max_tiles >= 1 && nb >= 1,
+              "block head gemm: bad arguments (k=%d n_out=%d)", k, n_out);
+  SPR_REQUIRE(x && w && out && tiles && a_parts && w_parts && part, "block head gemm: null operand");
+  auto lds = [](int bm, int bn) { return (size_t)(bm + bn) * spr::kPlaneStride * 2 * sizeof(_Float16); };
+  const spr::HeadTiles head{tiles, reinterpret_cast<const int4*>(tiles + tail_tiles_desc_offset(nb)), nb, part};
+  static_assert(kHeadTileRows == 128, "the head kernels below have 128-row tiles");
+  if (n_out > 32) {
+    hipLaunchKernelGGL((spr::k_gemm_nt_h3<128, 64, 4, 1, SPR_ACT_NONE, false, false, true>),
+                       dim3(cdiv(n_out, 64) * max_tiles), dim3(256), lds(128, 64), stream, x, 0, k, w, n_out,
+                       (const float*)nullptr, (const float*)nullptr, out, spr::AttnPlanes(), 0, a_parts, n_aparts,
+                       w_parts, (float*)nullptr, (const spr::GemmGroup*)nullptr, n_wparts, head);
+  } else {
+    hipLaunchKernelGGL((spr::k_gemm_nt_h3<128, 32, 4, 1, SPR_ACT_NONE, false, false, true>),
+                       dim3(cdiv(n_out, 32) * max_tiles), dim3(256), lds(128, 32), stream, x, 0, k, w, n_out,
+                       (const float*)nullptr, (const float*)nullptr, out, spr::AttnPlanes(), 0, a_parts, n_aparts,
+                       w_parts, (float*)nullptr, (const spr::GemmGroup*)nullptr, n_wparts, head);
+  }
+  SPR_LAUNCH_CHECK();
+  return 0;
 }
 
 void spr::gemm_group_tile(int max_n, int* bm, int* bn) {
@@ -773,15 +845,15 @@
     if (int rc = ensure_dyn_lds((const void*)kern, (int)lds(256, 256))) return rc;
     hipLaunchKernelGGL(kern, dim3(total_tiles), dim3(512), lds(256, 256), stream, a, 0, k, b, 0, epi,
                        (const float*)nullptr, c, spr::AttnPlanes(), 0, a_parts, kAmaxParts, w_parts,
-                       (float*)nullptr, groups_dev, kAmaxParts);
+                       (float*)nullptr, groups_dev, kAmaxParts, spr::HeadTiles());
   } else if (bn == 64) {
     hipLaunchKernelGGL((spr::k_gemm_nt_h3<128, 64, 4, 1, ACT, false>), dim3(total_tiles), dim3(256),
                        lds(128, 64), stream, a, 0, k, b, 0, epi, (const float*)nullptr, c, spr::AttnPlanes(), 0,
-                       a_parts, kAmaxParts, w_parts, (float*)nullptr, groups_dev, kAmaxParts);
+                       a_parts, kAmaxParts, w_parts, (float*)nullptr, groups_dev, kAmaxParts, spr::HeadTiles());
   } else {
     hipLaunchKernelGGL((spr::k_gemm_nt_h3<128, 32, 4, 1, ACT, false>), dim3(total_tiles), dim3(256),
                        lds(128, 32), stream, a, 0, k, b, 0, epi, (const float*)nullptr, c, spr::AttnPlanes(), 0,
-                       a_parts, kAmaxParts, w_parts, (float*)nullptr, groups_dev, kAmaxParts);
+                       a_parts, kAmaxParts, w_parts, (float*)nullptr, groups_dev, kAmaxParts, spr::HeadTiles());
   }
   SPR_LAUNCH_CHECK();
   return 0;
diff --git a/superpoints_registration_amd/csrc/norm_pool.hip b/superpoints_registration_amd/csrc/norm_pool.hip
--- a/superpoints_registration_amd/csrc/norm_pool.hip
+++ b/superpoints_registration_amd/csrc/norm_pool.hip
@@ -1,6 +1,8 @@
+#include "kp_records.h"
 #include "spr_common.h"
 
 namespace spr {
+int gemm_mode();
 namespace {
 
 constexpr int kSliceRows = 512;
@@ -91,52 +93,70 @@
 }
 
 constexpr int kInApplyUnroll = 4;
+struct ApplyRecords {
+  const float* s_xyz;
+  unsigned char* flag;
+  float4* sxf;
+  int* tile_ctr;
+};
+template <bool HEAD>
 __global__ __launch_bounds__(256) void k_in_apply(const float* __restrict__ x, const int* __restrict__ cu, int n,
                                                   int nb, int c, int norm, const float* __restrict__ mean,
                                                   const float* __restrict__ rstd, const float* __restrict__ add,
                                                   float slope, float* __restrict__ out,
-                                                  float* __restrict__ out_range, int nslots) {
+                                                  float* __restrict__ out_range, int nslots, int sstride,
+                                                  ApplyRecords rec) {
   const int c4 = c >> 2;
   const long total = (long)n * c4;
   const long stride = (long)gridDim.x * blockDim.x;
   const long g0 = (long)blockIdx.x * blockDim.x + threadIdx.x;
+  const float4* src = HEAD ? reinterpret_cast<const float4*>(out) : reinterpret_cast<const float4*>(x);
   float4 v[kInApplyUnroll], a[kInApplyUnroll];
 #pragma unroll
   for (int u = 0; u < kInApplyUnroll; ++u) {
     const long gid = g0 + u * stride;
     if (gid < total) {
-      v[u] = reinterpret_cast<const float4*>(x)[gid];
+      v[u] = src[gid];
       if (add) a[u] = reinterpret_cast<const float4*>(add)[gid];
     }
   }
+  const bool records = HEAD && rec.sxf != nullptr;
+  if (records && blockIdx.x == 0 && threadIdx.x == 0) rowflag_shadow(n, rec.sxf, rec.tile_ctr);
   float mx = 0.f;
 #pragma unroll
   for (int u = 0; u < kInApplyUnroll; ++u) {
     const long gid = g0 + u * stride;
-    if (gid >= total) continue;
-    float4 w = v[u];
-    if (norm) {
-      const int row = (int)(gid / c4), q = (int)(gid % c4);
-      const int cloud = find_segment(cu, nb, row);
-      const float4 m = reinterpret_cast<const float4*>(mean + (size_t)cloud * c)[q];
-      const float4 r = reinterpret_cast<const float4*>(rstd + (size_t)cloud * c)[q];
-      w.x = (w.x - m.x) * r.x;
-      w.y = (w.y - m.y) * r.y;
-      w.z = (w.z - m.z) * r.z;
-      w.w = (w.w - m.w) * r.w;
-    }
-    if (add) {
-      w.x += a[u].x;
-      w.y += a[u].y;
-      w.z += a[u].z;
-      w.w += a[u].w;
-    }
-    w.x = w.x >= 0.f ? w.x : w.x * slope;
-    w.y = w.y >= 0.f ? w.y : w.y * slope;
-    w.z = w.z >= 0.f ? w.z : w.z * slope;
-    w.w = w.w >= 0.f ? w.w : w.w * slope;
-    reinterpret_cast<float4*>(out)[gid] = w;
-    mx = fmaxf(mx, fmaxf(fmaxf(fabsf(w.x), fabsf(w.y)), fmaxf(fabsf(w.z), fabsf(w.w))));
+    const bool live = gid < total;
+    float4 w = make_float4(0.f, 0.f, 0.f, 0.f);
+    if (live) {
+      w = v[u];
+      if (norm) {
+        const int row = (int)(gid / c4), q = (int)(gid % c4);
+        const int cloud = find_segment(cu, nb, row);
+        const float4 m = reinterpret_cast<const float4*>(mean + (size_t)cloud * sstride)[q];
+        const float4 r = reinterpret_cast<const float4*>(rstd + (size_t)cloud * sstride)[q];
+        w.x = (w.x - m.x) * r.x;
+        w.y = (w.y - m.y) * r.y;
+        w.z = (w.z - m.z) * r.z;
+        w.w = (w.w - m.w) * r.w;
+      }
+      if (add) {
+        w.x += a[u].x;
+        w.y += a[u].y;
+        w.z += a[u].z;
+        w.w += a[u].w;
+      }
+      w.x = w.x >= 0.f ? w.x : w.x * slope;
+      w.y = w.y >= 0.f ? w.y : w.y * slope;
+      w.z = w.z >= 0.f ? w.z : w.z * slope;
+      w.w = w.w >= 0.f ? w.w : w.w * slope;
+      reinterpret_cast<float4*>(out)[gid] = w;
+      mx = fmaxf(mx, fmaxf(fmaxf(fabsf(w.x), fabsf(w.y)), fmaxf(fabsf(w.z), fabsf(w.w))));
+    }
+    if (records) {
+      const float t = rowflag_wide_sum(w, c4, (int)(threadIdx.x & 63));
+      if (live && gid % c4 == 0) rowflag_write(t, (int)(gid / c4), rec.s_xyz, rec.flag, rec.sxf);
+    }
   }
   if (out_range != nullptr) publish_range(mx, out_range, nslots);
 }
@@ -378,8 +398,88 @@
     SPR_LAUNCH_CHECK();
   }
   const long total = (long)n * (c / 4);
-  hipLaunchKernelGGL(k_in_apply, dim3(cdiv(total, 256 * kInApplyUnroll)), dim3(256), 0, stream, x, cu, n, nb, c,
-                     norm, mean, rstd, add, slope, out, out_range, out_range_n);
+  hipLaunchKernelGGL(k_in_apply<false>, dim3(cdiv(total, 256 * kInApplyUnroll)), dim3(256), 0, stream, x, cu, n, nb, c,
+                     norm, mean, rstd, add, slope, out, out_range, out_range_n, c, ApplyRecords{});
+  SPR_LAUNCH_CHECK();
+  return 0;
+}
+
+namespace {
+struct HeadWs {
+  double* part;
+  float* stats;
+  float *ap, *wp;
+};
+HeadWs head_layout(Workspace& w, int n, int nb, int n_out) {
+  const size_t B = (size_t)(nb > 0 ? nb : 1), no = (size_t)(n_out > 0 ? n_out : 0);
+  const size_t tiles = (size_t)cdiv(n > 0 ? n : 1, kHeadTileRows) + B;
+  HeadWs l;
+  l.part = w.take<double>(tiles * 2 * no);
+  l.stats = w.take<float>(B * 2 * no);
+  l.ap = w.take<float>(kAmaxParts);
+  l.wp = w.take<float>(kAmaxParts);
+  return l;
+}
+}
+
+extern "C" int spr_block_head_supported(int k, int n_out) {
+  return k >= 32 && k % 32 == 0 && n_out >= 16 && rowflag_wide(n_out);
+}
+
+extern "C" int spr_block_head_tile_rows(void) { return kHeadTileRows; }
+
+extern "C" size_t spr_block_head_workspace_size(int n, int nb, int n_out) {
+  return measure(head_layout, n, nb, n_out);
+}
+
+extern "C" int spr_block_head(const float* x, int k, const float* w, const int* cu, const int* tiles, int n, int nb,
+                              int n_out, float eps, int norm, float slope, float* out, float* stats_out,
+                              const float* x_range, int x_range_n, const float* w_range, int w_range_n,
+                              float* out_range, int out_range_n,
+                              const float* s_xyz, void* records, size_t records_bytes, void* ws, size_t ws_bytes,
+                              void* stream_) {
+  hipStream_t stream = (hipStream_t)stream_;
+  SPR_REQUIRE(spr::gemm_mode() == 1, "block_head: only in the split-fp16 product mode (spr_set_gemm_mode(1))");
+  SPR_REQUIRE(spr_block_head_supported(k, n_out), "block_head: unsupported shape k=%d n_out=%d (spr_block_head_supported)",
+              k, n_out);
+  SPR_REQUIRE(x && w && cu && tiles && out && n > 0 && nb >= 1, "block_head: null operand or empty input");
+  SPR_REQUIRE(((uintptr_t)tiles & 15) == 0 && ((uintptr_t)out & 15) == 0 && ((uintptr_t)stats_out & 15) == 0,
+              "block_head: tiles, out and stats_out must be 16-byte aligned");
+  SPR_REQUIRE((x_range == nullptr || x_range_n >= 1) && (w_range == nullptr || w_range_n >= 1),
+              "block_head: a range needs a count");
+  SPR_REQUIRE(out_range == nullptr || (out_range_n >= 1 && (out_range_n & (out_range_n - 1)) == 0),
+              "block_head: out_range_n must be a power of two");
+  SPR_REQUIRE((s_xyz == nullptr) == (records == nullptr), "block_head: s_xyz and records come together");
+  ApplyRecords rec{};
+  if (records != nullptr) {
+    SPR_REQUIRE(((uintptr_t)records & 15) == 0, "block_head: the records blob must be 16-byte aligned");
+    Workspace rw(records, records_bytes);
+    const KpRecords r = records_view(rw, n);
+    SPR_REQUIRE(rw.ok(), "block_head: records blob too small (spr_kpconv_records_size)");
+    rec = ApplyRecords{s_xyz, r.flag, r.sxf, r.tile_ctr};
+  }
+  Workspace wk(ws, ws_bytes);
+  const HeadWs l = head_layout(wk, n, nb, n_out);
+  SPR_REQUIRE(ws != nullptr && wk.ok(), "block_head: workspace too small");
+  const float* a_parts = x_range != nullptr ? x_range : l.ap;
+  const float* w_parts = w_range != nullptr ? w_range : l.wp;
+  const int n_ap = x_range != nullptr ? x_range_n : kAmaxParts, n_wp = w_range != nullptr ? w_range_n : kAmaxParts;
+  if (x_range == nullptr && w_range == nullptr) {
+    if (int rc = launch_absmax2(x, n, k, k, l.ap, w, n_out, k, k, l.wp, stream)) return rc;
+  } else if (x_range == nullptr) {
+    if (int rc = launch_absmax(x, n, k, k, l.ap, stream)) return rc;
+  } else if (w_range == nullptr) {
+    if (int rc = launch_absmax(w, n_out, k, k, l.wp, stream)) return rc;
+  }
+  const int max_tiles = cdiv(n, kHeadTileRows) + nb;
+  if (int rc = launch_gemm_head(x, k, w, n_out, out, tiles, nb, max_tiles, a_parts, n_ap, w_parts, n_wp, l.part, stream))
+    return rc;
+  float* const stats = stats_out != nullptr ? stats_out : l.stats;
+  launch_tail_final(l.part, cu, tiles, nb, 1, n_out, eps, stats, stream);
+  const long total = (long)n * (n_out / 4);
+  hipLaunchKernelGGL(k_in_apply<true>, dim3(cdiv(total, 256 * kInApplyUnroll)), dim3(256), 0, stream, (const float*)nullptr,
+                     cu, n, nb, n_out, norm, stats, stats + n_out, (const float*)nullptr, slope, out, out_range,
+                     out_range_n, 2 * n_out, rec);
   SPR_LAUNCH_CHECK();
   return 0;
 }
diff --git a/superpoints_registration_amd/csrc/spr_common.h b/superpoints_registration_amd/csrc/spr_common.h
--- a/superpoints_registration_amd/csrc/spr_common.h
+++ b/superpoints_registration_amd/csrc/spr_common.h
@@ -114,6 +114,15 @@
 void launch_in_final(const double* part, const int* cu, int nb, int c, int nsplit, float eps, float* mean,
                      float* rstd, hipStream_t stream);
 
+static inline size_t tail_tiles_desc_offset(int nb) { return align_up((size_t)(nb > 0 ? nb : 0) + 1, 4); }
+void launch_tail_final(const double* part, const int* cu, const int* tile_cu, int nb, int nbr, int n_total, float eps,
+                       float* stats, hipStream_t stream);
+
+constexpr int kHeadTileRows = 128;
+int launch_gemm_head(const float* x, int k, const float* w, int n_out, float* out, const int* tiles, int nb,
+                     int max_tiles, const float* a_parts, int n_aparts, const float* w_parts, int n_wparts,
+                     double* part, hipStream_t stream);
+
 #ifdef __HIPCC__
 typedef float f32x2 __attribute__((ext_vector_type(2)));
 typedef float f32x4 __attribute__((ext_vector_type(4)));
diff --git a/superpoints_registration_amd/kpconv_blocks.py b/superpoints_registration_amd/kpconv_blocks.py
--- a/superpoints_registration_amd/kpconv_blocks.py
+++ b/superpoints_registration_amd/kpconv_blocks.py
@@ -89,11 +89,14 @@
                                       fixed=self.fixed_kernel_points)
         return Parameter(torch.tensor(K_points_numpy, dtype=torch.float32), requires_grad=False)
 
-    def forward(self, q_pts, s_pts, neighb_inds, x):
+    def takes_records(self) -> bool:
+        return kpconv_modes.is_default_mode(self.KP_influence, self.aggregation_mode)
+
+    def forward(self, q_pts, s_pts, neighb_inds, x, records=None):
         if kpconv_modes.is_default_mode(self.KP_influence, self.aggregation_mode):
             return ops.kpconv(q_pts, s_pts, neighb_inds, x, self.weights,
                               self.kernel_points.detach(), self.KP_extent,
-                              rows_sorted=self.rows_sorted, impl=self.impl)
+                              rows_sorted=self.rows_sorted, impl=self.impl, records=records)
         return kpconv_modes.kpconv(q_pts, s_pts, neighb_inds, x, self.weights, self.kernel_points.detach(),
                                    self.KP_extent, self.KP_influence, self.aggregation_mode)
 
@@ -294,10 +297,20 @@
                 joined.record(branch)
             features.record_stream(branch)
 
-        x = self.unary1(features, stack_lengths_pre, cu=cu_pre, max_len=ml_pre) \
-            if isinstance(self.unary1, UnaryBlock) else features
+        records = None
+        if (isinstance(self.unary1, UnaryBlock) and features.is_cuda and not torch.is_grad_enabled() and self.use_bn
+                and ops.block_head_supported(self.unary1.in_dim, self.unary1.out_dim)):
+            if isinstance(self.KPConv, KPConv) and self.KPConv.takes_records():
+                x, records = ops.block_head(features, self.unary1.mlp.weight, cu_pre, eps=self.unary1.batch_norm.eps,
+                                            slope=0.1, s_pts=s_pts)
+            else:
+                x = ops.block_head(features, self.unary1.mlp.weight, cu_pre, eps=self.unary1.batch_norm.eps, slope=0.1)
+        else:
+            x = self.unary1(features, stack_lengths_pre, cu=cu_pre, max_len=ml_pre) \
+                if isinstance(self.unary1, UnaryBlock) else features
         self.KPConv.rows_sorted = bool(batch.get('_rows_sorted', False))
-        x = self.KPConv(q_pts, s_pts, neighb_inds, x)
+        x = self.KPConv(q_pts, s_pts, neighb_inds, x, records=records) if records is not None \
+            else self.KPConv(q_pts, s_pts, neighb_inds, x)
         fold = fused and self.use_bn
         conv_stats = None
         if fold:
diff --git a/superpoints_registration_amd/ops.py b/superpoints_registration_amd/ops.py
--- a/superpoints_registration_amd/ops.py
+++ b/superpoints_registration_amd/ops.py
@@ -541,17 +541,18 @@
 
 
 def kpconv(q_pts, s_pts, nbr, x, weights, kernel_points, kp_extent: float, rows_sorted: bool = False,
-           impl: int = 0) -> torch.Tensor:
+           impl: int = 0, records: Optional[torch.Tensor] = None) -> torch.Tensor:
     if _wants_grad(x, weights):
         from .autograd import KPConvFn
         return KPConvFn.apply(_dev(q_pts, "q_pts", torch.float32), _dev(s_pts, "s_pts", torch.float32), nbr,
                               _dev(x, "x", torch.float32), weights, kernel_points, float(kp_extent),
                               bool(rows_sorted), int(impl))
-    return kpconv_raw(q_pts, s_pts, nbr, x, weights, kernel_points, kp_extent, rows_sorted, impl)
+    return kpconv_raw(q_pts, s_pts, nbr, x, weights, kernel_points, kp_extent, rows_sorted, impl, records=records)
 
 
 def kpconv_raw(q_pts, s_pts, nbr, x, weights, kernel_points, kp_extent: float, rows_sorted: bool = False,
-               impl: int = 0, order: Optional[torch.Tensor] = None) -> torch.Tensor:
+               impl: int = 0, order: Optional[torch.Tensor] = None,
+               records: Optional[torch.Tensor] = None) -> torch.Tensor:
     q_pts = _dev(q_pts, "q_pts", torch.float32)
     s_pts = _dev(s_pts, "s_pts", torch.float32)
     x = _dev(x, "x", torch.float32)
@@ -569,6 +570,9 @@
     n_kp, cin, cout = weights.shape
     assert x.shape == (ns, cin), (x.shape, ns, cin)
     L = _lib.lib()
+    if records is not None and not (records.is_cuda and records.dtype == torch.uint8 and records.is_contiguous()
+                                    and records.numel() >= L.spr_kpconv_records_size(ns)):
+        raise ValueError("kpconv: records must be a device blob of spr_kpconv_records_size(ns) bytes")
     ws = _workspace(L.spr_kpconv_workspace_bytes(nq, ns, cin, cout), x.device)
     out = torch.empty((nq, cout), dtype=torch.float32, device=x.device)
     xr, xr_n = _get_range(x)
@@ -583,7 +587,7 @@
                                 int(bool(rows_sorted)), _ptr(x), cin, _ptr(weights), cout,
                                 _ptr(kernel_points), n_kp, float(kp_extent), _ptr(out), int(impl),
                                 _ptr(xr), int(xr_n), _ptr(wr), int(wr_n), _ptr(plan), _ptr(wplanes),
-                                _ptr(ws), ws.numel(), _stream(x)), "spr_kpconv_fwd")
+                                _ptr(ws), ws.numel(), _stream(x), _ptr(records)), "spr_kpconv_fwd")
     return out
 
 
@@ -744,6 +748,59 @@
                                 _stream(xa)), "spr_block_tail")
     _set_range(out, rng, cnt)
     return out
+
+
+def block_head_supported(k: int, n_out: int) -> bool:
+    return _modes["gemm"] == 1 and bool(_lib.lib().spr_block_head_supported(int(k), int(n_out)))
+
+
+def _head_records(cu: torch.Tensor, n: int) -> torch.Tensor:
+    def build():
+        blob = torch.empty((_lib.lib().spr_kpconv_records_size(n),), dtype=torch.uint8, device=cu.device)
+        return blob, blob
+    return _derived(cu, '_spr_head_records', (n, torch.cuda.current_stream(cu.device).cuda_stream), build)
+
+
+def block_head(x, w, cu, eps: float = 1e-5, slope: float = 0.1, s_pts=None, out=None, records=None,
+               norm: bool = True, stats=None):
+    x = _dev(x, "x", torch.float32)
+    w = _dev(w, "w", torch.float32)
+    cu = _dev(cu, "cu", torch.int32)
+    n, k = x.shape
+    n_out = w.shape[0]
+    assert w.shape[1] == k
+    nb = cu.numel() - 1
+    L = _lib.lib()
+    if not L.spr_block_head_supported(k, n_out):
+        raise RuntimeError(f"block_head: no kernel for k={k} n_out={n_out}")
+    tiles = _tail_tiles(cu, n, L.spr_block_head_tile_rows())
+    if out is None:
+        out = torch.empty((n, n_out), dtype=torch.float32, device=x.device)
+    else:
+        assert out.shape == (n, n_out) and out.dtype == torch.float32 and out.is_contiguous() and out.is_cuda
+    rbytes = 0
+    if s_pts is not None:
+        s_pts = _dev(s_pts, "s_pts", torch.float32)
+        assert s_pts.shape == (n, 3)
+        if records is None:
+            records = _head_records(cu, n)
+        assert records.dtype == torch.uint8 and records.is_cuda and records.is_contiguous()
+        rbytes = records.numel()
+    else:
+        records = None
+    ws = _workspace(L.spr_block_head_workspace_size(n, nb, n_out), x.device)
+    xr, xr_n = _get_range(x)
+    wr, wr_n = _static_range(w)
+    cnt = _STREAM_SLOTS
+    rng = _zero_slots(cnt, x.device)
+    if stats is not None:
+        assert stats.shape == (nb, 2, n_out) and stats.dtype == torch.float32 and stats.is_cuda and stats.is_contiguous()
+    _lib.check(L.spr_block_head(_ptr(x), k, _ptr(w), _ptr(cu), _ptr(tiles), n, nb, n_out, float(eps), int(bool(norm)),
+                                float(slope), _ptr(out), _ptr(stats), _ptr(xr), int(xr_n), _ptr(wr), int(wr_n),
+                                _ptr(rng), cnt, _ptr(s_pts),
+                                _ptr(records), rbytes, _ptr(ws), ws.numel(), _stream(x)), "spr_block_head")
+    _set_range(out, rng, cnt)
+    return (out, records) if s_pts is not None else out
 
 
 def cell_order(points: torch.Tensor, cu: torch.Tensor, cell: float) -> torch.Tensor:
```
